# SomeUserName1/UNet-bSSFP

Measured on AMD Instinct MI355X. Metric: train-step volumes/sec (128^3 bSSFP->6ch DTI), higher is better.
Workload: dtype bf16; 1 GPU; gan_step: full GAN training step (G fwd x2, G bwd, D fwd x3, D bwd x3, 2x AdamW); volume=1x24x128^3 -> 6ch per GPU, global_batch=1, perceptual_term=absent (needs remote weights), parallelism=dp1, input_feed=one batch resident in HBM

## Files before the change

### include/mi355_unet.h

```cpp
#ifndef MI355_UNET_H
#define MI355_UNET_H

#include <stddef.h>
#include <stdint.h>

#ifdef __cplusplus
extern "C" {
#endif

#define MI355_DT_F32 0
#define MI355_DT_BF16 1
#define MI355_DT_F64 2
#define MI355_DT_FP8 3

#define MI355_OK 0
#define MI355_ERR_ARG (-1)
#define MI355_ERR_UNSUPPORTED (-2)
#define MI355_ERR_HIP (-3)

int mi355_version(void);
const char* mi355_last_error(void);

int mi355_pack_ncdhw(const float* src, void* dst, int32_t n, int32_t c, int64_t v,
                     int32_t ld, int32_t coff, int32_t zero_to, int32_t dtype, void* stream);
int mi355_unpack_ncdhw(const void* src, float* dst, int32_t n, int32_t c, int64_t v,
                       int32_t ld, int32_t coff, int32_t dtype, void* stream);
int mi355_pack_ncdhw_s2d(const float* src, void* dst, int32_t n, int32_t c, int32_t d, int32_t h, int32_t w,
                         int32_t cblk, int32_t ld, int32_t coff, int32_t zero_to, int32_t dtype, void* stream);
int mi355_pack2_ncdhw(const float* src0, int32_t c0, const float* src1, int32_t c1, void* dst, int32_t n, int64_t v,
                      int32_t ld, int32_t coff, int32_t zero_to, int32_t dtype, void* stream);
int mi355_pack2_ncdhw_s2d(const float* src0, int32_t c0, const float* src1, int32_t c1, void* dst, int32_t n, int32_t d,
                          int32_t h, int32_t w, int32_t cblk, int32_t ld, int32_t coff, int32_t zero_to, int32_t dtype,
                          void* stream);
int mi355_unpack_ncdhw_s2d(const void* src, float* dst, int32_t n, int32_t c, int32_t d, int32_t h, int32_t w,
                           int32_t cblk, int32_t ld, int32_t coff, int32_t dtype, void* stream);

typedef struct mi355_wpack_desc {
  const float* src;
  void* dst;
  int32_t cout, cin;
  int32_t coutp, cinp;
  int32_t ks;
  int64_t s_co, s_ci;
  int64_t s_k[3];
  int32_t tbase[3], tstep[3];
  int32_t dtype;
  int32_t s2d_mode, s2d_cp;
  const float* q_amax;
} mi355_wpack_desc;
int mi355_weight_pack(const mi355_wpack_desc* d, void* stream);
int mi355_weight_pack_multi(const mi355_wpack_desc* descs, int32_t n, void* stream);

typedef struct mi355_conv_desc {
  const void* x0; int32_t c0; int32_t ld0;
  const void* x1; int32_t c1; int32_t ld1;
  int32_t n, di, hi, wi;
  int32_t do_, ho, wo;
  int32_t ks, stride;
  int32_t pad[3];
  const void* wp;
  int32_t coutp;
  const float* bias;
  void* y; int32_t ldy; int32_t cstore;
  int32_t dy, hy, wy;
  int32_t os; int32_t ooff[3];
  float* stats_part;
  int32_t dtype;
  void* workspace; int64_t workspace_bytes;
  int32_t cls_cout;
  int32_t nbias;
  const float* q_amax_x; const float* q_amax_w;
  const float* addend; int32_t ld_add; int32_t y_f32;
  int32_t add_n;
  int32_t d2s; const float* delta; int32_t add_bf16;
} mi355_conv_desc;
int mi355_conv_fwd(const mi355_conv_desc* d, void* stream);
int64_t mi355_conv_workspace_bytes(const mi355_conv_desc* d);
int mi355_conv_plan_id(const mi355_conv_desc* d);
int mi355_conv_num_tiles(const mi355_conv_desc* d, int32_t* tiles, int32_t* tiles_per_sample);

int mi355_upcat_compose(const float* wd, const float* wc, const float* bd, const float* bc, int32_t cl, int32_t cu, int32_t ce,
                        int32_t co, float* k4, void* wp_d2s, float* biasp, float* delta, void* stream);
int mi355_upcat_chain(const float* dk4, const float* wd, const float* wc, const float* bd, const float* esum, int32_t cl, int32_t cu,
                      int32_t ce, int32_t co, float* dwd, float* dwc, float* dbd, int32_t accumulate, void* stream);
int64_t mi355_border_sums_workspace(int32_t n, int32_t d, int32_t c);
int mi355_border_sums(const void* g, int32_t ld, int32_t n, int32_t d, int32_t h, int32_t w, int32_t c, int32_t dtype, float* workspace,
                      float* e, void* stream);
int mi355_s2d_repack(const void* src, int32_t ld_src, void* dst, int32_t ld_dst, int32_t n, int32_t d, int32_t h, int32_t w,
                     int32_t c, int32_t dtype, void* stream);
int mi355_seam_grad(const float* g_ncdhw, const void* g_s2d, int32_t ld_s, int32_t cblk, void* dz, int32_t ld_dz, int32_t cpad,
                    int32_t n, int32_t c, int32_t d, int32_t h, int32_t w, int32_t dtype, void* stream);

typedef struct mi355_wgrad_desc {
  const void* x0; int32_t c0; int32_t ld0;
  const void* x1; int32_t c1; int32_t ld1;
  int32_t n, di, hi, wi;
  const void* g; int32_t cg; int32_t ldg;
  int32_t do_, ho, wo;
  int32_t gd, gh, gw;
  int32_t gs; int32_t goff[3];
  int32_t ks, stride;
  int32_t pad[3];
  float* workspace; int64_t workspace_bytes;
  float* dw; int32_t cout, cin;
  int64_t s_co, s_ci; int64_t s_k[3];
  int32_t tbase[3], tstep[3];
  int32_t accumulate;
  int32_t dtype;
  int32_t s2d_cp;
  int32_t g_cls_cout;
  int32_t xn;
} mi355_wgrad_desc;
int64_t mi355_conv_wgrad_workspace(const mi355_wgrad_desc* d);
int mi355_conv_wgrad(const mi355_wgrad_desc* d, void* stream);
int mi355_conv_wgrad_plan_kind(const mi355_wgrad_desc* d);
typedef struct mi355_wreduce_job { int64_t opaque[20]; } mi355_wreduce_job;
int mi355_conv_wgrad_partial(const mi355_wgrad_desc* d, mi355_wreduce_job* job, void* stream);
int mi355_wgrad_reduce_multi(const mi355_wreduce_job* jobs, int32_t n, void* stream);

int mi355_channel_stats(const void* x, int32_t ld, int32_t c, int64_t rows_per_group, int32_t groups,
                        float* part, int32_t blocks_per_group, int32_t dtype, void* stream);
int32_t mi355_channel_stats_blocks(int64_t rows_per_group);

int mi355_norm_finalize(const float* part, int32_t parts_per_group, int32_t groups, int32_t c,
                        int64_t count_per_group, const float* shift, int32_t n_real, float eps,
                        float* mean, float* rstd,
                        float* running_mean, float* running_var, float momentum, int64_t* batches_tracked, void* stream);

typedef struct mi355_normact_desc {
  const void* z; int32_t ldz;
  void* a; int32_t lda;
  int32_t c; int64_t rows_per_group; int32_t groups;
  const float* mean; const float* rstd;
  const float* gamma; const float* beta;
  float slope;
  float drop_p; uint64_t seed;
  int32_t dtype;
  const void* da; int32_t ldda;
  void* dz; int32_t lddz;
  float* part;
  int32_t blocks_per_group;
  const float* sums;
  int32_t batch_stats;
  int32_t s2d_a, s2d_da;
  int32_t sd, sh, sw;
  const uint64_t* seed_ptr;
  int32_t n_affine;
  void* q8; int32_t ld8; const float* q_use; float* q_next;
  const void* gz; int32_t ldgz; const float* gw; int32_t gw_ld; int32_t gk;
  void* fy; int32_t ldfy; int32_t fcp; const float* fbias; int32_t skip_a;
  const void* pool_idx; const void* pool_dy; int32_t ldpdy;
  void* pool_y; int32_t ldpy; uint8_t* pool_widx;
} mi355_normact_desc;
int mi355_normact_fwd(const mi355_normact_desc* d, void* stream);
int mi355_normact_bwd_reduce(const mi355_normact_desc* d, void* stream);
int mi355_normact_bwd_finalize(const float* part, int32_t blocks_per_group, int32_t groups, int32_t c,
                               float* sums, float* dgamma, float* dbeta, void* stream);
int mi355_normact_bwd_finalize_into(const float* part, int32_t blocks_per_group, int32_t groups, int32_t c,
                                    float* sums, float* dgamma, float* dbeta, int32_t n_affine, int32_t accumulate,
                                    void* stream);
int mi355_normact_bwd_apply(const mi355_normact_desc* d, void* stream);

typedef struct mi355_normact_small_desc {
  mi355_normact_desc base;
  float eps, momentum;
  float* mean_out; float* rstd_out;
  float* running_mean; float* running_var; int64_t* batches_tracked; int32_t n_real;
  float* dgamma; float* dbeta; int32_t accumulate;
} mi355_normact_small_desc;
int mi355_normact_small_fwd(const mi355_normact_small_desc* d, void* stream);
int mi355_normact_small_bwd(const mi355_normact_small_desc* d, void* stream);

int mi355_colsum_finalize(const float* part, int32_t parts, int32_t c, float* out, void* stream);
int mi355_colsum_finalize_into(const float* part, int32_t parts, int32_t c, float* out, int32_t n_out, int32_t accumulate,
                               void* stream);
int mi355_colsum_finalize_from(const float* part, int32_t parts, int32_t c, int32_t offset, float* out, int32_t n_out,
                               int32_t accumulate, void* stream);

int mi355_maxpool2_fwd(const void* x, int32_t ldx, void* y, int32_t ldy, int32_t n, int32_t c,
                       int32_t d, int32_t h, int32_t w, int32_t dtype, void* stream);
int mi355_maxpool2_fwd_idx(const void* x, int32_t ldx, void* y, int32_t ldy, uint8_t* idx, int32_t n, int32_t c,
                           int32_t d, int32_t h, int32_t w, int32_t dtype, void* stream);
int mi355_maxpool2_bwd(const void* x, int32_t ldx, const void* y, int32_t ldy,
                       const void* dy, int32_t lddy, void* dx, int32_t lddx,
                       int32_t n, int32_t c, int32_t d, int32_t h, int32_t w,
                       int32_t dtype, void* stream);
int mi355_maxpool2_bwd_add(const void* x, int32_t ldx, const void* y, int32_t ldy, const void* dy, int32_t lddy,
                           void* dx, int32_t lddx, const void* add, int32_t ldadd,
                           int32_t n, int32_t c, int32_t d, int32_t h, int32_t w,
                           int32_t dtype, void* stream);

int32_t mi355_l1_blocks(int64_t count);
int mi355_l1_fwd(const float* a, const float* b, int64_t count, float* partials, float* out, void* stream);
int mi355_l1_bwd(const float* a, const float* b, int64_t count, const float* gscale, float* da, void* stream);
int mi355_l1_partials(const float* a, const float* b, int64_t count, float* partials, void* stream);

int mi355_gan_gen_loss_fwd(const float* logits, int32_t n, const float* l1_partials, int32_t n_partials, int64_t count,
                           float recon_divisor, float recon_factor, float* out4, void* stream);
int mi355_gan_gen_loss_bwd(const float* logits, int32_t n, const float* upstream, float recon_divisor, float recon_factor,
                           float* dlogits, float* l1_gscale, void* stream);
int mi355_gan_discr_loss_fwd(const float* logits_fake, int32_t n_fake, const float* logits_real, int32_t n_real, float* out1,
                             void* stream);
int mi355_gan_discr_loss_bwd(const float* logits_fake, int32_t n_fake, const float* logits_real, int32_t n_real,
                             const float* upstream, float* dfake, float* dreal, void* stream);

int mi355_adamw_multi(const void* const* ptrs, const int64_t* sizes, int32_t ntensors,
                      float lr, float beta1, float beta2, float eps, float weight_decay,
                      const int64_t* step_dev, int64_t step, void* stream);

int mi355_dti_scalar_maps(const void* tensor, int32_t dtype, int64_t nvox, int64_t comp_stride,
                          int64_t vox_stride, double scale, double offset, void* fa, void* md, void* ad,
                          void* rd, void* azimuth, void* inclination, void* rgb, void* stream);

int64_t mi355_dti_errors_workspace_bytes(int64_t nvox, int32_t nroi);
int mi355_dti_errors(const void* pred, const void* target, int32_t dtype, int64_t comp_stride, int64_t vox_stride,
                     const uint8_t* mask, const void* probseg, int32_t probseg_dtype, int64_t roi_stride,
                     int64_t probseg_vox_stride, int64_t nvox, int32_t nroi, double scale, double offset,
                     void* workspace, int64_t workspace_bytes, double* table_out, void* const* maps, void* stream);

#define MI355_MAX_PATCHES 48
#define MI355_AGG_CROP 0
#define MI355_AGG_AVERAGE 1
int mi355_patch_gather(const float* vol, int32_t c, int32_t d, int32_t h, int32_t w, const int32_t* origins,
                       int32_t npatches, int32_t pd, int32_t ph, int32_t pw, float* out, void* stream);
int mi355_patch_aggregate(const float* patches, const int32_t* locs9, int32_t npatches, int32_t pd, int32_t ph,
                          int32_t pw, int32_t mode, float* vol, float* count, int32_t c, int32_t d, int32_t h,
                          int32_t w, void* stream);
int mi355_patch_average_finalize(float* vol, const float* count, int32_t c, int64_t voxels, void* stream);

int32_t mi355_err_blocks(int64_t per_item);
int mi355_err_sums(const float* a, const float* b, int64_t per_item, int32_t items, double* partials,
                   double* out, void* stream);
int64_t mi355_ssim3d_workspace_bytes(int32_t items, int32_t c, int32_t d, int32_t h, int32_t w, int32_t win);
int mi355_ssim3d(const float* x, const float* y, int32_t items, int32_t c, int32_t d, int32_t h, int32_t w,
                 int32_t win, const float* window, float c1, float c2, void* workspace,
                 int64_t workspace_bytes, double* out, void* stream);

int mi355_aug_bias_field(const float* x, float* out, int32_t c, int32_t d, int32_t h, int32_t w,
                         const float* coefficients, int32_t order, void* stream);
int mi355_aug_gamma(const float* x, float* out, int64_t count, float gamma, void* stream);
int mi355_aug_noise(const float* x, float* out, int64_t count, float mean, float std, uint64_t seed, void* stream);

#define MI355_QUEUE_MAX_LOADS 4
#define MI355_QUEUE_MAX_IMAGES 4
#define MI355_QUEUE_MAX_STAGES 3
#define MI355_STAGE_BIAS_FIELD 1
#define MI355_STAGE_NOISE 2
#define MI355_STAGE_GAMMA 3

typedef struct mi355_queue_load {
  int32_t nstages;
  int32_t stage[MI355_QUEUE_MAX_STAGES];
  int32_t bias_order;
  float bias_coef[35];
  float noise_mean, noise_std;
  uint64_t noise_seed;
  float gamma;
} mi355_queue_load;

typedef struct mi355_queue_source {
  const float* src;
  int32_t d, h, w;
} mi355_queue_source;

int mi355_patch_queue_gather(const mi355_queue_load* loads, int32_t nloads, const mi355_queue_source* sources,
                             const int32_t* channels, const int32_t* augmented, float* const* outs, int32_t nimages,
                             const int32_t* patches, int32_t npatches, int32_t td, int32_t th, int32_t tw,
                             int32_t pd, int32_t ph, int32_t pw, float padding_value, void* stream);

#define MI355_AXIS_MAX_N 128
#define MI355_KSPACE_SUM_BLOCKS 128
int mi355_axis_apply(const float* x, const float* m, float* out, int32_t c, int32_t d, int32_t h, int32_t w,
                     int32_t axis, void* stream);
int mi355_axis_apply_complex(const float* xr, const float* xi, const float* mr, const float* mi, float* outr, float* outi,
                             int32_t c, int32_t d, int32_t h, int32_t w, int32_t axis, void* stream);
int64_t mi355_kspace_workspace_bytes(int32_t c, int32_t d, int32_t h, int32_t w);
int mi355_axis_apply_complex_max(const float* xr, const float* xi, const float* mr, const float* mi, int32_t c, int32_t d,
                                 int32_t h, int32_t w, void* workspace, int64_t workspace_bytes, double* out, void* stream);
int mi355_channel_sum_min(const float* x, int32_t c, int64_t vol, void* workspace, int64_t workspace_bytes, double* out,
                          void* stream);
int mi355_aug_spike_add(const float* x, float* out, int32_t c, int32_t d, int32_t h, int32_t w, int32_t f0, int32_t f1,
                        int32_t f2, const double* m, int32_t dc, float intensity, void* stream);

int mi355_mfma_selftest(float* out_f32_1024, float* out_bf16_1024, void* stream);

int mi355_amax_f32(const float* x, int64_t n, float* amax, void* stream);
int mi355_amax_act(const void* x, int32_t ld, int32_t c, int64_t rows, int32_t dtype, float* amax, void* stream);
int mi355_cast_fp8(const void* src, int32_t ld_src, int32_t c, int64_t rows, int32_t src_dtype, const float* amax,
                   void* dst, int32_t ld_dst, void* stream);
int mi355_cast_fp8_delayed(const void* src, int32_t ld_src, int32_t c, int64_t rows, int32_t src_dtype, const float* amax,
                           float* amax_next, void* dst, int32_t ld_dst, void* stream);
int mi355_fp8_scale_roll(float* table, int32_t n, int32_t* sat, void* stream);
int mi355_fp8_selftest(float* out_1024, void* stream);

#ifdef __cplusplus
}
#endif
#endif
```

### unet_bssfp_amd/_lib.py

```python
from __future__ import annotations

import ctypes as C
import os
import threading

_HERE = os.path.dirname(os.path.abspath(__file__))
LIB_PATH = os.path.join(_HERE, "libmi355_unet.so")

DT_F32 = 0
DT_BF16 = 1
DT_FP8 = 3

_i32, _i64, _f32, _u64, _vp = C.c_int32, C.c_int64, C.c_float, C.c_uint64, C.c_void_p


class WpackDesc(C.Structure):
    _fields_ = [("src", _vp), ("dst", _vp), ("cout", _i32), ("cin", _i32), ("coutp", _i32), ("cinp", _i32),
                ("ks", _i32), ("s_co", _i64), ("s_ci", _i64), ("s_k", _i64 * 3),
                ("tbase", _i32 * 3), ("tstep", _i32 * 3), ("dtype", _i32), ("s2d_mode", _i32), ("s2d_cp", _i32),
                ("q_amax", _vp)]


class ConvDesc(C.Structure):
    _fields_ = [("x0", _vp), ("c0", _i32), ("ld0", _i32), ("x1", _vp), ("c1", _i32), ("ld1", _i32),
                ("n", _i32), ("di", _i32), ("hi", _i32), ("wi", _i32),
                ("do_", _i32), ("ho", _i32), ("wo", _i32), ("ks", _i32), ("stride", _i32),
                ("pad", _i32 * 3), ("wp", _vp), ("coutp", _i32), ("bias", _vp),
                ("y", _vp), ("ldy", _i32), ("cstore", _i32), ("dy", _i32), ("hy", _i32), ("wy", _i32),
                ("os", _i32), ("ooff", _i32 * 3), ("stats_part", _vp), ("dtype", _i32),
                ("workspace", _vp), ("workspace_bytes", _i64), ("cls_cout", _i32), ("nbias", _i32),
                ("q_amax_x", _vp), ("q_amax_w", _vp), ("addend", _vp), ("ld_add", _i32), ("y_f32", _i32), ("add_n", _i32),
                ("d2s", _i32), ("delta", _vp), ("add_bf16", _i32)]


class WgradDesc(C.Structure):
    _fields_ = [("x0", _vp), ("c0", _i32), ("ld0", _i32), ("x1", _vp), ("c1", _i32), ("ld1", _i32),
                ("n", _i32), ("di", _i32), ("hi", _i32), ("wi", _i32),
                ("g", _vp), ("cg", _i32), ("ldg", _i32),
                ("do_", _i32), ("ho", _i32), ("wo", _i32), ("gd", _i32), ("gh", _i32), ("gw", _i32),
                ("gs", _i32), ("goff", _i32 * 3), ("ks", _i32), ("stride", _i32), ("pad", _i32 * 3),
                ("workspace", _vp), ("workspace_bytes", _i64),
                ("dw", _vp), ("cout", _i32), ("cin", _i32), ("s_co", _i64), ("s_ci", _i64), ("s_k", _i64 * 3),
                ("tbase", _i32 * 3), ("tstep", _i32 * 3), ("accumulate", _i32), ("dtype", _i32), ("s2d_cp", _i32),
                ("g_cls_cout", _i32), ("xn", _i32)]


class WreduceJob(C.Structure):
    _fields_ = [("opaque", _i64 * 20)]


class NormActDesc(C.Structure):
    _fields_ = [("z", _vp), ("ldz", _i32), ("a", _vp), ("lda", _i32), ("c", _i32),
                ("rows_per_group", _i64), ("groups", _i32),
                ("mean", _vp), ("rstd", _vp), ("gamma", _vp), ("beta", _vp),
                ("slope", _f32), ("drop_p", _f32), ("seed", _u64), ("dtype", _i32),
                ("da", _vp), ("ldda", _i32), ("dz", _vp), ("lddz", _i32),
                ("part", _vp), ("blocks_per_group", _i32), ("sums", _vp), ("batch_stats", _i32),
                ("s2d_a", _i32), ("s2d_da", _i32), ("sd", _i32), ("sh", _i32), ("sw", _i32), ("seed_ptr", _vp),
                ("n_affine", _i32), ("q8", _vp), ("ld8", _i32), ("q_use", _vp), ("q_next", _vp),
                ("gz", _vp), ("ldgz", _i32), ("gw", _vp), ("gw_ld", _i32), ("gk", _i32),
                ("fy", _vp), ("ldfy", _i32), ("fcp", _i32), ("fbias", _vp), ("skip_a", _i32),
                ("pool_idx", _vp), ("pool_dy", _vp), ("ldpdy", _i32),
                ("pool_y", _vp), ("ldpy", _i32), ("pool_widx", _vp)]


class QueueLoad(C.Structure):
    _fields_ = [("nstages", _i32), ("stage", _i32 * 3), ("bias_order", _i32), ("bias_coef", _f32 * 35),
                ("noise_mean", _f32), ("noise_std", _f32), ("noise_seed", _u64), ("gamma", _f32)]


class QueueSource(C.Structure):
    _fields_ = [("src", _vp), ("d", _i32), ("h", _i32), ("w", _i32)]


class NormSmallDesc(C.Structure):
    _fields_ = [("base", NormActDesc), ("eps", _f32), ("momentum", _f32), ("mean_out", _vp), ("rstd_out", _vp),
                ("running_mean", _vp), ("running_var", _vp), ("batches_tracked", _vp), ("n_real", _i32),
                ("dgamma", _vp), ("dbeta", _vp), ("accumulate", _i32)]


_SIGNATURES = {
    "mi355_version": (C.c_int, []),
    "mi355_last_error": (C.c_char_p, []),
    "mi355_pack_ncdhw": (C.c_int, [_vp, _vp, _i32, _i32, _i64, _i32, _i32, _i32, _i32, _vp]),
    "mi355_unpack_ncdhw": (C.c_int, [_vp, _vp, _i32, _i32, _i64, _i32, _i32, _i32, _vp]),
    "mi355_pack_ncdhw_s2d": (C.c_int, [_vp, _vp, _i32, _i32, _i32, _i32, _i32, _i32, _i32, _i32, _i32, _i32, _vp]),
    "mi355_unpack_ncdhw_s2d": (C.c_int, [_vp, _vp, _i32, _i32, _i32, _i32, _i32, _i32, _i32, _i32, _i32, _vp]),
    "mi355_pack2_ncdhw": (C.c_int, [_vp, _i32, _vp, _i32, _vp, _i32, _i64, _i32, _i32, _i32, _i32, _vp]),
    "mi355_pack2_ncdhw_s2d": (C.c_int, [_vp, _i32, _vp, _i32, _vp, _i32, _i32, _i32, _i32, _i32, _i32, _i32, _i32, _i32, _vp]),
    "mi355_upcat_compose": (C.c_int, [_vp, _vp, _vp, _vp, _i32, _i32, _i32, _i32, _vp, _vp, _vp, _vp, _vp]),
    "mi355_upcat_chain": (C.c_int, [_vp, _vp, _vp, _vp, _vp, _i32, _i32, _i32, _i32, _vp, _vp, _vp, _i32, _vp]),
    "mi355_border_sums_workspace": (_i64, [_i32, _i32, _i32]),
    "mi355_border_sums": (C.c_int, [_vp, _i32, _i32, _i32, _i32, _i32, _i32, _i32, _vp, _vp, _vp]),
    "mi355_s2d_repack": (C.c_int, [_vp, _i32, _vp, _i32, _i32, _i32, _i32, _i32, _i32, _i32, _vp]),
    "mi355_seam_grad": (C.c_int, [_vp, _vp, _i32, _i32, _vp, _i32, _i32, _i32, _i32, _i32, _i32, _i32, _i32, _vp]),
    "mi355_weight_pack": (C.c_int, [C.POINTER(WpackDesc), _vp]),
    "mi355_weight_pack_multi": (C.c_int, [C.POINTER(WpackDesc), _i32, _vp]),
    "mi355_conv_fwd": (C.c_int, [C.POINTER(ConvDesc), _vp]),
    "mi355_conv_workspace_bytes": (_i64, [C.POINTER(ConvDesc)]),
    "mi355_conv_plan_id": (C.c_int, [C.POINTER(ConvDesc)]),
    "mi355_conv_num_tiles": (C.c_int, [C.POINTER(ConvDesc), C.POINTER(_i32), C.POINTER(_i32)]),
    "mi355_conv_wgrad_workspace": (_i64, [C.POINTER(WgradDesc)]),
    "mi355_conv_wgrad_plan_kind": (C.c_int, [C.POINTER(WgradDesc)]),
    "mi355_conv_wgrad": (C.c_int, [C.POINTER(WgradDesc), _vp]),
    "mi355_conv_wgrad_partial": (C.c_int, [C.POINTER(WgradDesc), C.POINTER(WreduceJob), _vp]),
    "mi355_wgrad_reduce_multi": (C.c_int, [C.POINTER(WreduceJob), _i32, _vp]),
    "mi355_channel_stats": (C.c_int, [_vp, _i32, _i32, _i64, _i32, _vp, _i32, _i32, _vp]),
    "mi355_channel_stats_blocks": (_i32, [_i64]),
    "mi355_norm_finalize": (C.c_int, [_vp, _i32, _i32, _i32, _i64, _vp, _i32, _f32, _vp, _vp, _vp, _vp, _f32, _vp, _vp]),
    "mi355_normact_fwd": (C.c_int, [C.POINTER(NormActDesc), _vp]),
    "mi355_normact_bwd_reduce": (C.c_int, [C.POINTER(NormActDesc), _vp]),
    "mi355_normact_bwd_finalize": (C.c_int, [_vp, _i32, _i32, _i32, _vp, _vp, _vp, _vp]),
    "mi355_normact_bwd_finalize_into": (C.c_int, [_vp, _i32, _i32, _i32, _vp, _vp, _vp, _i32, _i32, _vp]),
    "mi355_normact_bwd_apply": (C.c_int, [C.POINTER(NormActDesc), _vp]),
    "mi355_normact_small_fwd": (C.c_int, [C.POINTER(NormSmallDesc), _vp]),
    "mi355_normact_small_bwd": (C.c_int, [C.POINTER(NormSmallDesc), _vp]),
    "mi355_colsum_finalize": (C.c_int, [_vp, _i32, _i32, _vp, _vp]),
    "mi355_colsum_finalize_into": (C.c_int, [_vp, _i32, _i32, _vp, _i32, _i32, _vp]),
    "mi355_colsum_finalize_from": (C.c_int, [_vp, _i32, _i32, _i32, _vp, _i32, _i32, _vp]),
    "mi355_maxpool2_fwd": (C.c_int, [_vp, _i32, _vp, _i32, _i32, _i32, _i32, _i32, _i32, _i32, _vp]),
    "mi355_maxpool2_fwd_idx": (C.c_int, [_vp, _i32, _vp, _i32, _vp, _i32, _i32, _i32, _i32, _i32, _i32, _vp]),
    "mi355_maxpool2_bwd": (C.c_int, [_vp, _i32, _vp, _i32, _vp, _i32, _vp, _i32, _i32, _i32, _i32, _i32, _i32, _i32, _vp]),
    "mi355_maxpool2_bwd_add": (C.c_int, [_vp, _i32, _vp, _i32, _vp, _i32, _vp, _i32, _vp, _i32, _i32, _i32, _i32, _i32, _i32, _i32, _vp]),
    "mi355_l1_blocks": (_i32, [_i64]),
    "mi355_l1_fwd": (C.c_int, [_vp, _vp, _i64, _vp, _vp, _vp]),
    "mi355_l1_bwd": (C.c_int, [_vp, _vp, _i64, _vp, _vp, _vp]),
    "mi355_l1_partials": (C.c_int, [_vp, _vp, _i64, _vp, _vp]),
    "mi355_gan_gen_loss_fwd": (C.c_int, [_vp, _i32, _vp, _i32, _i64, _f32, _f32, _vp, _vp]),
    "mi355_gan_gen_loss_bwd": (C.c_int, [_vp, _i32, _vp, _f32, _f32, _vp, _vp, _vp]),
    "mi355_gan_discr_loss_fwd": (C.c_int, [_vp, _i32, _vp, _i32, _vp, _vp]),
    "mi355_gan_discr_loss_bwd": (C.c_int, [_vp, _i32, _vp, _i32, _vp, _vp, _vp, _vp]),
    "mi355_adamw_multi": (C.c_int, [_vp, _vp, _i32, _f32, _f32, _f32, _f32, _f32, _vp, _i64, _vp]),
    "mi355_dti_scalar_maps": (C.c_int, [_vp, _i32, _i64, _i64, _i64, C.c_double, C.c_double,
                                        _vp, _vp, _vp, _vp, _vp, _vp, _vp, _vp]),
    "mi355_dti_errors_workspace_bytes": (_i64, [_i64, _i32]),
    "mi355_dti_errors": (C.c_int, [_vp, _vp, _i32, _i64, _i64, _vp, _vp, _i32, _i64, _i64, _i64, _i32,
                                   C.c_double, C.c_double, _vp, _i64, _vp, _vp, _vp]),
    "mi355_patch_gather": (C.c_int, [_vp, _i32, _i32, _i32, _i32, _vp, _i32, _i32, _i32, _i32, _vp, _vp]),
    "mi355_patch_aggregate": (C.c_int, [_vp, _vp, _i32, _i32, _i32, _i32, _i32, _vp, _vp, _i32, _i32, _i32, _i32, _vp]),
    "mi355_patch_average_finalize": (C.c_int, [_vp, _vp, _i32, _i64, _vp]),
    "mi355_err_blocks": (_i32, [_i64]),
    "mi355_err_sums": (C.c_int, [_vp, _vp, _i64, _i32, _vp, _vp, _vp]),
    "mi355_ssim3d_workspace_bytes": (_i64, [_i32, _i32, _i32, _i32, _i32, _i32]),
    "mi355_ssim3d": (C.c_int, [_vp, _vp, _i32, _i32, _i32, _i32, _i32, _i32, _vp, _f32, _f32, _vp, _i64, _vp, _vp]),
    "mi355_aug_bias_field": (C.c_int, [_vp, _vp, _i32, _i32, _i32, _i32, _vp, _i32, _vp]),
    "mi355_aug_gamma": (C.c_int, [_vp, _vp, _i64, _f32, _vp]),
    "mi355_aug_noise": (C.c_int, [_vp, _vp, _i64, _f32, _f32, C.c_uint64, _vp]),
    "mi355_patch_queue_gather": (C.c_int, [C.POINTER(QueueLoad), _i32, C.POINTER(QueueSource), _vp, _vp, _vp, _i32,
                                           _vp, _i32, _i32, _i32, _i32, _i32, _i32, _i32, _f32, _vp]),
    "mi355_axis_apply": (C.c_int, [_vp, _vp, _vp, _i32, _i32, _i32, _i32, _i32, _vp]),
    "mi355_axis_apply_complex": (C.c_int, [_vp, _vp, _vp, _vp, _vp, _vp, _i32, _i32, _i32, _i32, _i32, _vp]),
    "mi355_kspace_workspace_bytes": (_i64, [_i32, _i32, _i32, _i32]),
    "mi355_axis_apply_complex_max": (C.c_int, [_vp, _vp, _vp, _vp, _i32, _i32, _i32, _i32, _vp, _i64, _vp, _vp]),
    "mi355_channel_sum_min": (C.c_int, [_vp, _i32, _i64, _vp, _i64, _vp, _vp]),
    "mi355_aug_spike_add": (C.c_int, [_vp, _vp, _i32, _i32, _i32, _i32, _i32, _i32, _i32, _vp, _i32, _f32, _vp]),
    "mi355_mfma_selftest": (C.c_int, [_vp, _vp, _vp]),
    "mi355_amax_f32": (C.c_int, [_vp, _i64, _vp, _vp]),
    "mi355_amax_act": (C.c_int, [_vp, _i32, _i32, _i64, _i32, _vp, _vp]),
    "mi355_cast_fp8": (C.c_int, [_vp, _i32, _i32, _i64, _i32, _vp, _vp, _i32, _vp]),
    "mi355_cast_fp8_delayed": (C.c_int, [_vp, _i32, _i32, _i64, _i32, _vp, _vp, _vp, _i32, _vp]),
    "mi355_fp8_scale_roll": (C.c_int, [_vp, _i32, _vp, _vp]),
    "mi355_fp8_selftest": (C.c_int, [_vp, _vp]),
}

EXPORTED_SYMBOLS = tuple(_SIGNATURES)

_lock = threading.Lock()
_lib = None


class Mi355Error(RuntimeError):
    pass


def load():
    global _lib
    if _lib is not None:
        return _lib
    with _lock:
        if _lib is None:
            if not os.path.exists(LIB_PATH):
                raise Mi355Error(
                    f"{LIB_PATH} not found: build it with `python -c 'import __graft_entry__ as g; g.build()'` "
                    "(hipcc --offload-arch=gfx950).  There is no CPU fallback.")
            lib = C.CDLL(LIB_PATH)
            for name, (res, args) in _SIGNATURES.items():
                fn = getattr(lib, name)
                fn.restype = res
                fn.argtypes = args
            _lib = lib
    return _lib


def check(rc: int, what: str = ""):
    if rc != 0:
        msg = load().mi355_last_error().decode("utf-8", "replace")
        raise Mi355Error(f"{what or 'mi355 call'} failed ({rc}): {msg}")
```

### unet_bssfp_amd/csrc/elementwise.hip

```cpp
#include <stdlib.h>
#include "common.h"

namespace {

constexpr int kRowsPerStatBlock = 2048;

struct S2D { int d, h, w, cblk; };
__device__ __forceinline__ void s2d_cell(const S2D& q, long long row , long long& srow, int& blk, int& border) {
  const int w = (int)(row % q.w); long long t = row / q.w;
  const int h = (int)(t % q.h); t /= q.h;
  const int d = (int)(t % q.d); const long long n = t / q.d;
  srow = ((n * (q.d / 2 + 1) + ((d + 1) >> 1)) * (q.h / 2 + 1) + ((h + 1) >> 1)) * (q.w / 2 + 1) + ((w + 1) >> 1);
  blk = ((d + 1) & 1) * 4 + ((h + 1) & 1) * 2 + ((w + 1) & 1);
  border = ((d == 0 || d == q.d - 1) ? 4 : 0) | ((h == 0 || h == q.h - 1) ? 2 : 0) | ((w == 0 || w == q.w - 1) ? 1 : 0);
}
__device__ __forceinline__ long long s2d_offset(const S2D& q, long long row, int ld) {
  long long srow; int blk, border;
  s2d_cell(q, row, srow, blk, border);
  return srow * ld + (long long)blk * q.cblk;
}
template <typename T>
__device__ __forceinline__ void s2d_zero_siblings(T* base, const S2D& q, long long srow, int blk, int border, int ld, int e0) {
  if (!border) return;
  Vec16<T> z;
// ... 222 lines not shown
                                                             long long rows_per_group, float* __restrict__ part,
                                                             int blocks_per_group) {
  const int g = blockIdx.y, b = blockIdx.x;
  const long long rb = (rows_per_group + blocks_per_group - 1) / blocks_per_group;
  const long long r0 = (long long)b * rb;
  long long r1 = r0 + rb;
  if (r1 > rows_per_group) r1 = rows_per_group;
  const T* base = x + (long long)g * rows_per_group * ld;
  float* out = part + ((long long)g * blocks_per_group + b) * 2 * c;
  block_channel_sums<T>(c, r0, r1,
      [&](long long row, int ch0, float* s0, float* s1) {
        Vec16<T> v;
        v.load(base + row * ld + ch0);
#pragma unroll
        for (int j = 0; j < Vec16<T>::N; ++j) { s0[j] += v.f[j]; s1[j] += v.f[j] * v.f[j]; }
      },
      out, out + c);
}

__device__ __forceinline__ void block_sum_parts(const float* __restrict__ part, int nparts, int c, int ch0,
                                                double& t0, double& t1) {
  __shared__ double red[16][8][2];
  const int cl = threadIdx.x & 7, pl = threadIdx.x >> 3;
  const int ch = ch0 + cl;
  double s0 = 0.0, s1 = 0.0;
  if (ch < c) {
    int k = pl;
    for (; k + 384 < nparts; k += 512) {
      const float a0 = part[(long long)k * 2 * c + ch], b0 = part[(long long)k * 2 * c + c + ch];
      const float a1 = part[(long long)(k + 128) * 2 * c + ch], b1 = part[(long long)(k + 128) * 2 * c + c + ch];
      const float a2 = part[(long long)(k + 256) * 2 * c + ch], b2 = part[(long long)(k + 256) * 2 * c + c + ch];
      const float a3 = part[(long long)(k + 384) * 2 * c + ch], b3 = part[(long long)(k + 384) * 2 * c + c + ch];
      s0 += ((double)a0 + (double)a1) + ((double)a2 + (double)a3);
      s1 += ((double)b0 + (double)b1) + ((double)b2 + (double)b3);
    }
    for (; k < nparts; k += 128) {
      s0 += (double)part[(long long)k * 2 * c + ch];
      s1 += (double)part[(long long)k * 2 * c + c + ch];
    }
  }
#pragma unroll
  for (int o = 8; o < 64; o <<= 1) {
    s0 += __shfl_xor(s0, o, 64);
    s1 += __shfl_xor(s1, o, 64);
  }
  const int wave = threadIdx.x >> 6;
  if ((threadIdx.x & 63) < 8) { red[wave][cl][0] = s0; red[wave][cl][1] = s1; }
  __syncthreads();
  double a0 = 0.0, a1 = 0.0;
#pragma unroll
  for (int w = 0; w < 16; ++w) { a0 += red[w][cl][0]; a1 += red[w][cl][1]; }
  t0 = a0;
  t1 = a1;
  __syncthreads();
}

__global__ __launch_bounds__(1024) void norm_finalize_kernel(const float* __restrict__ part, int ppg, int c,
                                                             long long count, const float* __restrict__ shift,
                                                             int n_real, float eps, float* __restrict__ mean,
                                                             float* __restrict__ rstd, float* running_mean,
                                                             float* running_var, float momentum,
                                                             long long* batches_tracked, int groups_here) {
  const int ch0 = blockIdx.x * 8;
  if (batches_tracked && blockIdx.x == 0 && blockIdx.y == 0 && threadIdx.x == 0) batches_tracked[0] += groups_here;
  for (int gi = 0; gi < groups_here; ++gi) {
    const int g = groups_here > 1 ? gi : blockIdx.y;
    double s1, s2;
    block_sum_parts(part + (long long)g * ppg * 2 * c, ppg, c, ch0, s1, s2);
    const int ch = ch0 + (int)threadIdx.x;
    if (threadIdx.x >= 8 || ch >= c) continue;
    const double m = s1 / (double)count;
    double var = s2 / (double)count - m * m;
    if (var < 0.0) var = 0.0;
    const double mu = m + ((shift && ch < n_real) ? (double)shift[ch] : 0.0);
    mean[(long long)g * c + ch] = (float)mu;
    rstd[(long long)g * c + ch] = (float)(1.0 / sqrt(var + (double)eps));
    if (running_mean && ch < n_real) {
      const double unb = count > 1 ? var * (double)count / (double)(count - 1) : var;
      running_mean[ch] = (float)((1.0 - momentum) * running_mean[ch] + momentum * mu);
      running_var[ch] = (float)((1.0 - momentum) * running_var[ch] + momentum * unb);
    }
  }
}

__global__ __launch_bounds__(1024) void colsum_finalize_kernel(const float* __restrict__ part, int parts, int c, int offset,
                                                               float* __restrict__ out, int n_out, int accumulate) {
  const int ch0 = offset + blockIdx.x * 8;
  double s0, s1;
  block_sum_parts(part, parts, c, ch0, s0, s1);
  const int j = blockIdx.x * 8 + (int)threadIdx.x;
  if (threadIdx.x < 8 && j < n_out) out[j] = accumulate ? out[j] + (float)s0 : (float)s0;
}

__device__ __forceinline__ unsigned long long eff_seed(unsigned long long salt, const unsigned long long* p) {
  return p ? p[0] * 0x9E3779B97F4A7C15ull + salt * 0xD1B54A32D192ED03ull + 1ull : salt;
}
__device__ __forceinline__ unsigned long long drop_group_bits(unsigned long long seed, unsigned long long group) {
  unsigned long long x = group * 0x9E3779B97F4A7C15ull + seed;
  x ^= x >> 32; x *= 0xD6E8FEB86659FD93ull; x ^= x >> 32;
  return x;
}
template <int EPV>
__device__ __forceinline__ unsigned drop_keep_mask(unsigned long long seed, unsigned long long e0, unsigned thr16) {
  unsigned m = 0;
#pragma unroll
  for (int g4 = 0; g4 < EPV / 4; ++g4) {
    const unsigned long long x = drop_group_bits(seed, (e0 >> 2) + g4);
#pragma unroll
    for (int k = 0; k < 4; ++k) m |= ((((unsigned)(x >> (16 * k))) & 0xffffu) >= thr16 ? 1u : 0u) << (4 * g4 + k);
  }
  return m;
}

__device__ __forceinline__ void amax_commit(float m, float* out) {
  __shared__ float red[4];
#pragma unroll
  for (int o = 32; o > 0; o >>= 1) m = fmaxf(m, __shfl_xor(m, o, 64));
  if ((threadIdx.x & 63) == 0) red[threadIdx.x >> 6] = m;
  __syncthreads();
  if (threadIdx.x == 0) {
    m = fmaxf(fmaxf(red[0], red[1]), fmaxf(red[2], red[3]));
    const unsigned cur = __hip_atomic_load(reinterpret_cast<unsigned int*>(out), __ATOMIC_RELAXED, __HIP_MEMORY_SCOPE_AGENT);
    if (__float_as_uint(m) > cur) atomicMax(reinterpret_cast<unsigned int*>(out), __float_as_uint(m));
  }
}
__device__ __forceinline__ float e4m3_piece(const float (&f)[8], float sc, uint8_t* dst) {
  float m = 0.f, r[8];
#pragma unroll
  for (int j = 0; j < 8; ++j) {
    const float b = __uint_as_float((uint32_t)f32_to_bf16_bits(f[j]) << 16);
    m = fmaxf(m, fabsf(b));
    r[j] = b * sc;
  }
  uint32_t w0 = cvt_pk_fp8(r[0], r[1], 0u, false), w1 = cvt_pk_fp8(r[4], r[5], 0u, false);
  w0 = cvt_pk_fp8(r[2], r[3], w0, true);
  w1 = cvt_pk_fp8(r[6], r[7], w1, true);
  *reinterpret_cast<uint2*>(dst) = make_uint2(w0, w1);
  return m;
}

struct NormActArgs {
  const char* z; int ldz; char* a; int lda;
  int c; long long rows_per_group; int groups;
  const float* mean; const float* rstd; const float* gamma; const float* beta;
  float slope; float drop_scale; unsigned thr16; unsigned long long seed; const unsigned long long* seed_ptr;
  const char* da; int ldda; char* dz; int lddz;
  float* part; int blocks_per_group; const float* sums; int batch_stats;
  int n_affine;
  S2D s2d_a;
  S2D s2d_da;
  uint8_t* q8; int ld8; const float* q_use; float* q_next;
  const char* gz; int ldgz; const float* gw; int gw_ld; int gk;
  char* fy; int ldfy; int fcp; const float* fbias; int skip_a;
  const uint8_t* pool_idx; const char* pool_dy; int ldpdy; int pd, ph, pw;
  char* pool_y; int ldpy; uint8_t* pool_widx;
};

#ifndef MI355_DIAG_NO_NT
#define FP8_NT_A 1
#endif
__device__ __forceinline__ void st_nt_b128(void* p, const uint4 v) {
  typedef unsigned u4 __attribute__((ext_vector_type(4)));
  const u4 x = {v.x, v.y, v.z, v.w};
  __builtin_nontemporal_store(x, reinterpret_cast<u4*>(p));
}
__device__ __forceinline__ void store16_nt(const Vec16<float>& v, void* p) {
  st_nt_b128(p, make_uint4(__float_as_uint(v.f[0]), __float_as_uint(v.f[1]), __float_as_uint(v.f[2]), __float_as_uint(v.f[3])));
}
__device__ __forceinline__ void store16_nt(const Vec16<bf16_t>& v, void* p) {
  uint32_t w[4];
#pragma unroll
  for (int i = 0; i < 4; ++i) w[i] = (uint32_t)f32_to_bf16_bits(v.f[2 * i]) | ((uint32_t)f32_to_bf16_bits(v.f[2 * i + 1]) << 16);
  st_nt_b128(p, make_uint4(w[0], w[1], w[2], w[3]));
}

template <typename T, bool DROP>
__global__ __launch_bounds__(256) void normact_fwd_kernel(const NormActArgs q) {
  constexpr int EPV = Elem<T>::kPer16B;
  const int g = blockIdx.y;
  const int lpr = q.c / EPV, rpp = 256 / lpr;
  const int piece = threadIdx.x % lpr, rsub = threadIdx.x / lpr;
  if (rsub >= rpp) return;
  const int ch0 = piece * EPV;
  const unsigned long long seed = DROP ? eff_seed(q.seed, q.seed_ptr) : 0ull;
  float sc[EPV], sh[EPV];
#pragma unroll
  for (int j = 0; j < EPV; ++j) {
    const int ch = ch0 + j;
    const float ga = q.gamma ? (ch < q.n_affine ? q.gamma[ch] : 0.f) : 1.f, be = (q.beta && ch < q.n_affine) ? q.beta[ch] : 0.f;
    if (q.mean) {
      const float rs = q.rstd[(long long)g * q.c + ch], mu = q.mean[(long long)g * q.c + ch];
      sc[j] = ga * rs;
      sh[j] = be - mu * ga * rs;
    } else { sc[j] = ga; sh[j] = be; }
  }
  const T* zb = reinterpret_cast<const T*>(q.z) + (long long)g * q.rows_per_group * q.ldz;
  T* ab = reinterpret_cast<T*>(q.a) + (long long)g * q.rows_per_group * q.lda;
  const long long stride = (long long)gridDim.x * rpp;
  const float sc8 = q.q8 ? fp8_scale_of(q.q_use) : 1.f;
  float m8 = 0.f;
  for (long long row = (long long)blockIdx.x * rpp + rsub; row < q.rows_per_group; row += stride) {
    Vec16<T> v;
#ifdef NORM_NT_FWD
    v.load_nt(zb + row * q.ldz + ch0);
#else
    v.load(zb + row * q.ldz + ch0);
#endif
    const unsigned long long e0 = ((unsigned long long)g * q.rows_per_group + row) * q.c + ch0;
    unsigned keep = 0;
    if constexpr (DROP) keep = drop_keep_mask<EPV>(seed, e0, q.thr16);
#pragma unroll
    for (int j = 0; j < EPV; ++j) {
      float t = v.f[j] * sc[j] + sh[j];
      if constexpr (DROP) t = (keep >> j) & 1u ? t * q.drop_scale : 0.f;
      v.f[j] = t > 0.f ? t : t * q.slope;
    }
    if (q.s2d_a.d) {
      long long srow; int blk, border;
      s2d_cell(q.s2d_a, (long long)g * q.rows_per_group + row, srow, blk, border);
      v.store(reinterpret_cast<T*>(q.a) + srow * q.lda + (long long)blk * q.s2d_a.cblk + ch0);
      s2d_zero_siblings<T>(reinterpret_cast<T*>(q.a), q.s2d_a, srow, blk, border, q.lda, ch0);
    }
#ifdef FP8_NT_A
    else if (q.q8) store16_nt(v, ab + row * q.lda + ch0);
#endif
    else v.store(ab + row * q.lda + ch0);
    if constexpr (sizeof(T) == 2) {
      if (q.q8) m8 = fmaxf(m8, e4m3_piece(v.f, sc8, q.q8 + ((long long)g * q.rows_per_group + row) * q.ld8 + ch0));
    }
  }
  if constexpr (sizeof(T) == 2) {
    if (q.q8) amax_commit(m8, q.q_next);
  }
}

template <typename T, bool DROP>
__global__ __launch_bounds__(256) void normact_pool_fwd_kernel(const NormActArgs q) {
  constexpr int EPV = Elem<T>::kPer16B;
  const int lpr = q.c / EPV, vpp = 256 / lpr;
  const int piece = threadIdx.x % lpr, vsub = threadIdx.x / lpr;
  if (vsub >= vpp) return;
  const int ch0 = piece * EPV;
  const int n_ = blockIdx.y;
  const long long dhw = (long long)q.pd * q.ph * q.pw;
  const int g = (int)(((long long)n_ * dhw) / q.rows_per_group);
  const unsigned long long seed = DROP ? eff_seed(q.seed, q.seed_ptr) : 0ull;
  float sc[EPV], sh[EPV];
#pragma unroll
  for (int j = 0; j < EPV; ++j) {
    const int ch = ch0 + j;
    const float ga = q.gamma ? (ch < q.n_affine ? q.gamma[ch] : 0.f) : 1.f, be = (q.beta && ch < q.n_affine) ? q.beta[ch] : 0.f;
    if (q.mean) {
      const float rs = q.rstd[(long long)g * q.c + ch], mu = q.mean[(long long)g * q.c + ch];
      sc[j] = ga * rs;
      sh[j] = be - mu * ga * rs;
    } else { sc[j] = ga; sh[j] = be; }
  }
  const int od_ = q.pd / 2, oh_ = q.ph / 2, ow_ = q.pw / 2;
  const int pooled = od_ * oh_ * ow_;
  const T* zb = reinterpret_cast<const T*>(q.z);
  T* ab = reinterpret_cast<T*>(q.a);
  for (int o = blockIdx.x * vpp + vsub; o < pooled; o += gridDim.x * vpp) {
    const int ow = o % ow_, t = o / ow_, oh = t % oh_, od = t / oh_;
    Vec16<T> m;
    unsigned long long where = 0;
    unsigned nan_seen = 0;
#pragma unroll
    for (int kd = 0; kd < 2; ++kd)
#pragma unroll
      for (int kh = 0; kh < 2; ++kh)
#pragma unroll
        for (int kw = 0; kw < 2; ++kw) {
          const long long vox = (((long long)n_ * q.pd + 2 * od + kd) * q.ph + 2 * oh + kh) * q.pw + 2 * ow + kw;
          const unsigned long long kk = (unsigned long long)(kd * 4 + kh * 2 + kw);
          Vec16<T> v;
#ifdef NORM_NT_FWD
          v.load_nt(zb + vox * q.ldz + ch0);
#else
          v.load(zb + vox * q.ldz + ch0);
#endif
          unsigned keep = 0;
          if constexpr (DROP) keep = drop_keep_mask<EPV>(seed, (unsigned long long)vox * q.c + ch0, q.thr16);
#pragma unroll
          for (int j = 0; j < EPV; ++j) {
            float t2 = v.f[j] * sc[j] + sh[j];
            if constexpr (DROP) t2 = (keep >> j) & 1u ? t2 * q.drop_scale : 0.f;
            t2 = t2 > 0.f ? t2 : t2 * q.slope;
            if constexpr (sizeof(T) == 2) t2 = bf16_bits_to_f32(f32_to_bf16_bits(t2));
            v.f[j] = t2;
          }
          v.store(ab + vox * q.lda + ch0);
          if (kk == 0) {
            m = v;
#pragma unroll
            for (int j = 0; j < EPV; ++j) nan_seen |= (v.f[j] != v.f[j] ? 1u : 0u) << j;
          } else {
#pragma unroll
            for (int j = 0; j < EPV; ++j) {
              const bool isnan_ = v.f[j] != v.f[j];
              const bool take = v.f[j] > m.f[j] || isnan_;
              m.f[j] = take ? v.f[j] : m.f[j];
              const bool mark = ((nan_seen >> j) & 1u) ? false : take;
              where = mark ? ((where & ~(0xffull << (8 * j))) | (kk << (8 * j))) : where;
              nan_seen |= (isnan_ ? 1u : 0u) << j;
            }
          }
        }
    const long long orow = (long long)n_ * pooled + o;
    m.store(reinterpret_cast<T*>(q.pool_y) + orow * q.ldpy + ch0);
    if constexpr (EPV == 8) *reinterpret_cast<unsigned long long*>(q.pool_widx + orow * q.c + ch0) = where;
    else *reinterpret_cast<unsigned*>(q.pool_widx + orow * q.c + ch0) = (unsigned)where;
  }
}

typedef float f32x4v __attribute__((ext_vector_type(4)));
template <bool DROP>
__global__ __launch_bounds__(256) void normact_fwd_final32_kernel(const NormActArgs q) {
  const int lane = threadIdx.x & 63, wave = threadIdx.x >> 6, n = lane & 15, p = lane >> 4;
  const int g = blockIdx.y, ch0 = 8 * p;
  const unsigned long long seed = DROP ? eff_seed(q.seed, q.seed_ptr) : 0ull;
  float sc[8], sh[8];
#pragma unroll
  for (int j = 0; j < 8; ++j) {
    const int ch = ch0 + j;
    const float ga = q.gamma ? (ch < q.n_affine ? q.gamma[ch] : 0.f) : 1.f, be = (q.beta && ch < q.n_affine) ? q.beta[ch] : 0.f;
    if (q.mean) {
      const float rs = q.rstd[(long long)g * 32 + ch], mu = q.mean[(long long)g * 32 + ch];
      sc[j] = ga * rs;
      sh[j] = be - mu * ga * rs;
    } else { sc[j] = ga; sh[j] = be; }
  }
  uint4 wf;
  {
    unsigned w[4];
#pragma unroll
    for (int i = 0; i < 4; ++i) {
      const int ch = ch0 + 2 * i;
      const float lo = (n < q.gk && ch < q.gw_ld) ? q.gw[(long long)n * q.gw_ld + ch] : 0.f;
      const float hi = (n < q.gk && ch + 1 < q.gw_ld) ? q.gw[(long long)n * q.gw_ld + ch + 1] : 0.f;
      w[i] = (unsigned)f32_to_bf16_bits(lo) | ((unsigned)f32_to_bf16_bits(hi) << 16);
    }
    wf = make_uint4(w[0], w[1], w[2], w[3]);
  }
  float fb[4];
#pragma unroll
  for (int j = 0; j < 4; ++j) fb[j] = (q.fbias && 4 * p + j < q.gk) ? q.fbias[4 * p + j] : 0.f;
  const bf16_t* zb = reinterpret_cast<const bf16_t*>(q.z) + (long long)g * q.rows_per_group * q.ldz;
  bf16_t* ab = reinterpret_cast<bf16_t*>(q.a) + (long long)g * q.rows_per_group * q.lda;
  bf16_t* yb = reinterpret_cast<bf16_t*>(q.fy) + (long long)g * q.rows_per_group * q.ldfy;
  const long long stride = (long long)gridDim.x * 64;
  const long long first = (long long)blockIdx.x * 64 + wave * 16;
  uint4 zn = make_uint4(0u, 0u, 0u, 0u);
  if (first < q.rows_per_group) {
    const long long rc = first + n < q.rows_per_group ? first + n : q.rows_per_group - 1;
    zn = *reinterpret_cast<const uint4*>(zb + rc * q.ldz + ch0);
  }
  for (long long row0 = first; row0 < q.rows_per_group; row0 += stride) {
    const long long row = row0 + n;
    const bool ok = row < q.rows_per_group;
    const long long rowc = ok ? row : q.rows_per_group - 1;
    const uint4 zc = zn;
    if (row0 + stride < q.rows_per_group) {
      const long long rc = row + stride < q.rows_per_group ? row + stride : q.rows_per_group - 1;
      zn = *reinterpret_cast<const uint4*>(zb + rc * q.ldz + ch0);
    }
    Vec16<bf16_t> v;
    v.from_bits(zc);
    unsigned keep = 0;
    if constexpr (DROP) keep = drop_keep_mask<8>(seed, ((unsigned long long)g * q.rows_per_group + rowc) * 32 + ch0, q.thr16);
#pragma unroll
    for (int j = 0; j < 8; ++j) {
      float x = v.f[j] * sc[j] + sh[j];
      if constexpr (DROP) x = (keep >> j) & 1u ? x * q.drop_scale : 0.f;
      v.f[j] = x > 0.f ? x : x * q.slope;
    }
    unsigned w[4];
#pragma unroll
    for (int i = 0; i < 4; ++i) w[i] = (unsigned)f32_to_bf16_bits(v.f[2 * i]) | ((unsigned)f32_to_bf16_bits(v.f[2 * i + 1]) << 16);
    const uint4 aw = make_uint4(w[0], w[1], w[2], w[3]);
    if (ok && !q.skip_a) *reinterpret_cast<uint4*>(ab + row * q.lda + ch0) = aw;
    f32x4v acc = {0.f, 0.f, 0.f, 0.f};
    acc = __builtin_amdgcn_mfma_f32_16x16x32_bf16(__builtin_bit_cast(bf16x8, wf), __builtin_bit_cast(bf16x8, aw), acc, 0, 0, 0);
    if (ok && 4 * p < q.fcp) {
      const uint2 yv = make_uint2((uint32_t)f32_to_bf16_bits(acc[0] + fb[0]) | ((uint32_t)f32_to_bf16_bits(acc[1] + fb[1]) << 16),
                                  (uint32_t)f32_to_bf16_bits(acc[2] + fb[2]) | ((uint32_t)f32_to_bf16_bits(acc[3] + fb[3]) << 16));
      *reinterpret_cast<uint2*>(yb + row * q.ldfy + 4 * p) = yv;
    }
  }
}

template <int EPV> struct BwdConst { float mu[EPV], rs[EPV], ga[EPV], be[EPV]; };
template <int EPV>
__device__ __forceinline__ void load_bwd_const(const NormActArgs& q, int g, int ch0, BwdConst<EPV>& k) {
#pragma unroll
  for (int j = 0; j < EPV; ++j) {
    const int ch = ch0 + j;
    k.mu[j] = q.mean ? q.mean[(long long)g * q.c + ch] : 0.f;
    k.rs[j] = q.mean ? q.rstd[(long long)g * q.c + ch] : 1.f;
    k.ga[j] = q.gamma ? (ch < q.n_affine ? q.gamma[ch] : 0.f) : 1.f;
    k.be[j] = (q.beta && ch < q.n_affine) ? q.beta[ch] : 0.f;
  }
}
constexpr int kImplicitMaxC = 64;
__device__ __forceinline__ void fill_implicit_w(const NormActArgs& q, uint4* wtab) {
  const int ch = threadIdx.x;
  if (ch < q.c && ch < kImplicitMaxC) {
    unsigned w[4];
#pragma unroll
    for (int i = 0; i < 4; ++i) {
      const bool okc = ch < q.gw_ld;
      const float lo = (okc && 2 * i < q.gk) ? q.gw[(long long)(2 * i) * q.gw_ld + ch] : 0.f;
      const float hi = (okc && 2 * i + 1 < q.gk) ? q.gw[(long long)(2 * i + 1) * q.gw_ld + ch] : 0.f;
      w[i] = (unsigned)f32_to_bf16_bits(lo) | ((unsigned)f32_to_bf16_bits(hi) << 16);
    }
    wtab[ch] = make_uint4(w[0], w[1], w[2], w[3]);
  }
  __syncthreads();
}
template <typename T, int EPV>
__device__ __forceinline__ void implicit_da(const NormActArgs& q, long long grow, const uint4* wtab, int ch0, Vec16<T>& dv) {
  if constexpr (sizeof(T) == 2) {
    typedef __bf16 bf16x2 __attribute__((ext_vector_type(2)));
    const uint4 gv = *reinterpret_cast<const uint4*>(reinterpret_cast<const T*>(q.gz) + grow * q.ldgz);
    asm volatile("" : "+v"(ch0));
#pragma unroll
    for (int j = 0; j < EPV; ++j) {
      const uint4 wv = wtab[ch0 + j];
      float t = __builtin_amdgcn_fdot2_f32_bf16(__builtin_bit_cast(bf16x2, gv.x), __builtin_bit_cast(bf16x2, wv.x), 0.f, false);
      t = __builtin_amdgcn_fdot2_f32_bf16(__builtin_bit_cast(bf16x2, gv.y), __builtin_bit_cast(bf16x2, wv.y), t, false);
      t = __builtin_amdgcn_fdot2_f32_bf16(__builtin_bit_cast(bf16x2, gv.z), __builtin_bit_cast(bf16x2, wv.z), t, false);
      t = __builtin_amdgcn_fdot2_f32_bf16(__builtin_bit_cast(bf16x2, gv.w), __builtin_bit_cast(bf16x2, wv.w), t, false);
      dv.f[j] = bf16_bits_to_f32(f32_to_bf16_bits(t));
    }
  }
}
template <typename T, int EPV>
__device__ __forceinline__ void pooled_da(const NormActArgs& q, long long grow, int ch0, Vec16<T>& dv) {
  const unsigned v = (unsigned)grow, W = (unsigned)q.pw, H = (unsigned)q.ph, D = (unsigned)q.pd;
  const unsigned w_ = v % W, t1 = v / W, h_ = t1 % H, t2 = t1 / H, d_ = t2 % D, n_ = t2 / D;
  const long long o = (((long long)n_ * (D >> 1) + (d_ >> 1)) * (H >> 1) + (h_ >> 1)) * (W >> 1) + (w_ >> 1);
  const unsigned k = ((d_ & 1u) << 2) | ((h_ & 1u) << 1) | (w_ & 1u);
  Vec16<T> gy;
  gy.load(reinterpret_cast<const T*>(q.pool_dy) + o * q.ldpdy + ch0);
  unsigned long long ib;
  if constexpr (EPV == 8) ib = *reinterpret_cast<const unsigned long long*>(q.pool_idx + o * q.c + ch0);
  else ib = *reinterpret_cast<const unsigned*>(q.pool_idx + o * q.c + ch0);
  if (q.da) dv.load(reinterpret_cast<const T*>(q.da) + grow * q.ldda + ch0);
#pragma unroll
  for (int j = 0; j < EPV; ++j) {
    float t = ((unsigned)(ib >> (8 * j)) & 0xffu) == k ? gy.f[j] : 0.f;
    if (q.da) t += dv.f[j];
    if constexpr (sizeof(T) == 2) t = bf16_bits_to_f32(f32_to_bf16_bits(t));
    dv.f[j] = t;
  }
}
template <bool DROP>
__device__ __forceinline__ void bwd_elem(const NormActArgs& q, bool keep, float mu, float rs, float ga,
                                         float be, float zv, float dav, float& gout, float& xhat) {
  xhat = (zv - mu) * rs;
  float pre = xhat * ga + be;
  float gv = dav;
  if constexpr (DROP) {
    pre = keep ? pre : 0.f;
    gv = keep ? gv * q.drop_scale : 0.f;
  }
  gout = pre > 0.f ? gv : gv * q.slope;
}

template <typename T, bool DROP, int IMPL = 0>
__global__ __launch_bounds__(256) void normact_bwd_reduce_kernel(const NormActArgs q) {
  constexpr int EPV = Elem<T>::kPer16B;
  const int g = blockIdx.y, b = blockIdx.x;
  const long long rb = (q.rows_per_group + q.blocks_per_group - 1) / q.blocks_per_group;
  const long long r0 = (long long)b * rb;
  long long r1 = r0 + rb;
  if (r1 > q.rows_per_group) r1 = q.rows_per_group;
  const T* zb = reinterpret_cast<const T*>(q.z) + (long long)g * q.rows_per_group * q.ldz;
  const T* db = reinterpret_cast<const T*>(q.da) + (long long)g * q.rows_per_group * q.ldda;
  float* out = q.part + ((long long)g * q.blocks_per_group + b) * 2 * q.c;
  BwdConst<EPV> k;
  load_bwd_const<EPV>(q, g, (int)(threadIdx.x % (q.c / EPV)) * EPV, k);
  const unsigned long long seed = DROP ? eff_seed(q.seed, q.seed_ptr) : 0ull;
  __shared__ uint4 wtab[IMPL == 1 ? kImplicitMaxC : 1];
  if constexpr (IMPL == 1) fill_implicit_w(q, wtab);
  block_channel_sums<T>(q.c, r0, r1,
      [&](long long row, int ch0, float* s0, float* s1) {
        Vec16<T> zv, dv;
        zv.load(zb + row * q.ldz + ch0);
        if constexpr (IMPL == 1) implicit_da<T, EPV>(q, (long long)g * q.rows_per_group + row, wtab, ch0, dv);
        else if constexpr (IMPL == 2) pooled_da<T, EPV>(q, (long long)g * q.rows_per_group + row, ch0, dv);
        else if (q.s2d_da.d) dv.load(reinterpret_cast<const T*>(q.da) + s2d_offset(q.s2d_da, (long long)g * q.rows_per_group + row, q.ldda) + ch0);
        else dv.load(db + row * q.ldda + ch0);
        unsigned keep = 0;
        if constexpr (DROP) keep = drop_keep_mask<EPV>(seed, ((unsigned long long)g * q.rows_per_group + row) * q.c + ch0, q.thr16);
#pragma unroll
        for (int j = 0; j < EPV; ++j) {
          float gv, xh;
          bwd_elem<DROP>(q, (keep >> j) & 1u, k.mu[j], k.rs[j], k.ga[j], k.be[j], zv.f[j], dv.f[j], gv, xh);
          s0[j] += gv;
          s1[j] += gv * xh;
        }
      },
      out, out + q.c);
}

__global__ __launch_bounds__(1024) void normact_bwd_finalize_kernel(const float* __restrict__ part, int bpg,
                                                                    int groups, int c, float* __restrict__ sums,
                                                                    float* dgamma, float* dbeta, int n_affine, int accumulate) {
  const int ch0 = blockIdx.x * 8;
  const int ch = ch0 + (int)threadIdx.x;
  const bool owner = threadIdx.x < 8 && ch < c;
  double tg = 0.0, tb = 0.0;
  for (int g = 0; g < groups; ++g) {
    double s0, s1;
    block_sum_parts(part + (long long)g * bpg * 2 * c, bpg, c, ch0, s0, s1);
    if (owner) {
      sums[((long long)g * 2 + 0) * c + ch] = (float)s0;
      sums[((long long)g * 2 + 1) * c + ch] = (float)s1;
      tb += s0;
      tg += s1;
    }
  }
  if (owner && ch < n_affine) {
    if (dgamma) dgamma[ch] = accumulate ? dgamma[ch] + (float)tg : (float)tg;
    if (dbeta) dbeta[ch] = accumulate ? dbeta[ch] + (float)tb : (float)tb;
  }
}

template <typename T, bool DROP, int IMPL = 0>
__global__ __launch_bounds__(256, IMPL == 1 ? 5 : 1) void normact_bwd_apply_kernel(const NormActArgs q) {
  constexpr int EPV = Elem<T>::kPer16B;
  __shared__ uint4 wtab[IMPL == 1 ? kImplicitMaxC : 1];
  if constexpr (IMPL == 1) fill_implicit_w(q, wtab);
  const int g = blockIdx.y;
  const int lpr = q.c / EPV, rpp = 256 / lpr;
  const int piece = threadIdx.x % lpr, rsub = threadIdx.x / lpr;
  if (rsub >= rpp) return;
  const int ch0 = piece * EPV;
  const float inv = 1.f / (float)q.rows_per_group;
// ... 1070 lines not shown
                "weight_pack: bad extents");
  MI355_REQUIRE(d->s2d_mode >= 0 && d->s2d_mode <= 2 && (d->s2d_mode == 0 || (d->s2d_cp > 0 && d->s2d_cp % 8 == 0)),
                "weight_pack: bad space-to-depth mode");
  a->src = d->src; a->dst = d->dst; a->cout = d->cout; a->cin = d->cin; a->coutp = d->coutp; a->cinp = d->cinp; a->ks = d->ks;
  a->s_co = d->s_co; a->s_ci = d->s_ci; a->s_k0 = d->s_k[0]; a->s_k1 = d->s_k[1]; a->s_k2 = d->s_k[2];
  a->tb0 = d->tbase[0]; a->tb1 = d->tbase[1]; a->tb2 = d->tbase[2];
  a->ts0 = d->tstep[0]; a->ts1 = d->tstep[1]; a->ts2 = d->tstep[2];
  a->s2d_mode = d->s2d_mode; a->s2d_cp = d->s2d_cp;
  a->q_amax = d->q_amax;
  return MI355_OK;
}

int mi355_weight_pack_multi(const mi355_wpack_desc* descs, int32_t n, void* stream) {
  MI355_REQUIRE(descs && n > 0, "weight_pack_multi: bad argument");
  const int dtype = descs[0].dtype;
  MI355_REQUIRE(dtype == MI355_DT_F32 || dtype == MI355_DT_BF16 || dtype == MI355_DT_FP8, "weight_pack_multi: bad dtype");
  for (int pass = 0; pass < 3; ++pass) {
    const bool want_dense = pass == 0, want_s2d = pass == 1;
    int i0 = 0;
    while (i0 < n) {
      WpackMulti m;
      int cnt = 0;
      long long mx = 0, patches = 0;
      const mi355_wpack_desc* firstd = nullptr;
      for (; i0 < n && cnt < kWpackChunk; ++i0) {
        const mi355_wpack_desc* d = &descs[i0];
        MI355_REQUIRE(d->dtype == dtype, "weight_pack_multi: mixed dtypes");
        const int klass = wpack_is_dense3(d) ? 0 : (wpack_is_s2d_dense(d) ? 1 : 2);
        if (klass != pass) continue;
        int rc = fill_wpack(d, &m.a[cnt]);
        if (rc) return rc;
        if (!firstd) firstd = d;
        const long long total = (long long)d->cinp * d->ks * d->ks * d->ks * d->coutp;
        const long long np = want_s2d ? (d->s2d_mode == 1 ? (long long)(d->coutp / 8) * (d->s2d_cp / 16) : (long long)(d->cinp / 16) * (d->s2d_cp / 8))
                                      : (long long)(d->cinp / 16) * (d->coutp / 16);
        if (total > mx) mx = total;
        if (np > patches) patches = np;
        ++cnt;
      }
      if (cnt == 0) break;
      for (int i = cnt; i < kWpackChunk; ++i) m.a[i] = m.a[0];
      if (want_dense) {
        MI355_REQUIRE(patches < (1ll << 31), "weight_pack_multi: too many patches");
        dim3 grid((unsigned)patches, cnt);
        if (dtype == MI355_DT_F32) wpack_dense3_multi_kernel<float><<<grid, dim3(256), 0, (hipStream_t)stream>>>(m);
        else if (dtype == MI355_DT_FP8) wpack_dense3_multi_kernel<fp8_t><<<grid, dim3(256), 0, (hipStream_t)stream>>>(m);
        else wpack_dense3_multi_kernel<bf16_t><<<grid, dim3(256), 0, (hipStream_t)stream>>>(m);
      } else if (want_s2d) {
        MI355_REQUIRE(patches < (1ll << 31), "weight_pack_multi: too many patches");
        dim3 grid((unsigned)patches, cnt);
        MI355_REQUIRE(dtype != MI355_DT_FP8, "weight_pack_multi: no fp8 space-to-depth packing");
        if (dtype == MI355_DT_F32) wpack_s2d_multi_kernel<float><<<grid, dim3(256), 0, (hipStream_t)stream>>>(m);
        else wpack_s2d_multi_kernel<bf16_t><<<grid, dim3(256), 0, (hipStream_t)stream>>>(m);
      } else {
        long long nb = (mx + 256 * 8 - 1) / (256 * 8);
        if (nb > 512) nb = 512;
        dim3 grid((unsigned)nb, cnt);
        if (dtype == MI355_DT_F32) hipLaunchKernelGGL(wpack_multi_kernel<float>, grid, dim3(256), 0, (hipStream_t)stream, m);
        else if (dtype == MI355_DT_FP8) hipLaunchKernelGGL(wpack_multi_kernel<fp8_t>, grid, dim3(256), 0, (hipStream_t)stream, m);
        else hipLaunchKernelGGL(wpack_multi_kernel<bf16_t>, grid, dim3(256), 0, (hipStream_t)stream, m);
      }
    }
  }
  return mi355_check_launch("weight_pack_multi");
}

int32_t mi355_channel_stats_blocks(int64_t rows_per_group) {
  long long b = rows_per_group / 128;
  if (b > 1024) b = (rows_per_group + kRowsPerStatBlock - 1) / kRowsPerStatBlock;
  if (b < 1024 && rows_per_group / 128 > 1024) b = 1024;
  const long long fine = rows_per_group / 16 < 256 ? rows_per_group / 16 : 256;
  if (b < fine) b = fine;
  if (b < 1) b = 1;
  if (b > 2048) b = 2048;
  return (int32_t)b;
}

int mi355_channel_stats(const void* x, int32_t ld, int32_t c, int64_t rows_per_group, int32_t groups, float* part,
                        int32_t blocks_per_group, int32_t dtype, void* stream) {
  MI355_REQUIRE(x && part && rows_per_group > 0 && groups > 0 && blocks_per_group > 0, "channel_stats: bad argument");
  int rc = check_rows(c, ld, dtype, "channel_stats");
  if (rc) return rc;
  dim3 grid(blocks_per_group, groups);
  if (dtype == MI355_DT_F32)
    hipLaunchKernelGGL(channel_stats_kernel<float>, grid, dim3(256), 0, (hipStream_t)stream, (const float*)x, ld, c, (long long)rows_per_group, part, blocks_per_group);
  else
    hipLaunchKernelGGL(channel_stats_kernel<bf16_t>, grid, dim3(256), 0, (hipStream_t)stream, (const bf16_t*)x, ld, c, (long long)rows_per_group, part, blocks_per_group);
  return mi355_check_launch("channel_stats");
}

int mi355_norm_finalize(const float* part, int32_t parts_per_group, int32_t groups, int32_t c, int64_t count_per_group,
                        const float* shift, int32_t n_real, float eps, float* mean, float* rstd, float* running_mean,
                        float* running_var, float momentum, int64_t* batches_tracked, void* stream) {
  MI355_REQUIRE(part && mean && rstd && parts_per_group > 0 && groups > 0 && c > 0 && count_per_group > 0, "norm_finalize: bad argument");
  MI355_REQUIRE(!running_mean || running_var, "norm_finalize: running_mean without running_var");
  const bool serial = running_mean && groups > 1;
  hipLaunchKernelGGL(norm_finalize_kernel, dim3((c + 7) / 8, serial ? 1 : groups), dim3(1024), 0, (hipStream_t)stream, part,
                     parts_per_group, c, (long long)count_per_group, shift, n_real > 0 ? n_real : c, eps, mean, rstd, running_mean, running_var, momentum,
                     (long long*)batches_tracked, serial ? groups : 1);
  return mi355_check_launch("norm_finalize");
}

int mi355_colsum_finalize(const float* part, int32_t parts, int32_t c, float* out, void* stream) {
  return mi355_colsum_finalize_into(part, parts, c, out, c, 0, stream);
}

int mi355_colsum_finalize_into(const float* part, int32_t parts, int32_t c, float* out, int32_t n_out, int32_t accumulate,
                               void* stream) {
  return mi355_colsum_finalize_from(part, parts, c, 0, out, n_out, accumulate, stream);
}

int mi355_colsum_finalize_from(const float* part, int32_t parts, int32_t c, int32_t offset, float* out, int32_t n_out,
                               int32_t accumulate, void* stream) {
  MI355_REQUIRE(part && out && parts > 0 && c > 0 && n_out > 0 && offset >= 0 && offset + n_out <= c, "colsum_finalize: bad argument");
  hipLaunchKernelGGL(colsum_finalize_kernel, dim3((n_out + 7) / 8), dim3(1024), 0, (hipStream_t)stream, part, parts, c, offset, out, n_out,
                     accumulate);
  return mi355_check_launch("colsum_finalize");
}

static int fill_normact(const mi355_normact_desc* d, NormActArgs* q, const char* who) {
  MI355_REQUIRE(d && d->z, "%s: null pointer", who);
  int rc = check_rows(d->c, d->ldz, d->dtype, who);
  if (rc) return rc;
  MI355_REQUIRE(d->rows_per_group > 0 && d->groups > 0, "%s: empty", who);
  MI355_REQUIRE(!d->mean || d->rstd, "%s: mean without rstd", who);
  MI355_REQUIRE(d->drop_p >= 0.f && d->drop_p < 1.f, "%s: dropout p out of range", who);
  q->z = (const char*)d->z; q->ldz = d->ldz; q->a = (char*)d->a; q->lda = d->lda;
  q->c = d->c; q->rows_per_group = d->rows_per_group; q->groups = d->groups;
  q->mean = d->mean; q->rstd = d->rstd; q->gamma = d->gamma; q->beta = d->beta;
  q->slope = d->slope;
  q->thr16 = d->drop_p > 0.f ? (unsigned)(d->drop_p * 65536.f + 0.5f) : 0u;
  q->drop_scale = d->drop_p > 0.f ? 1.f / (1.f - d->drop_p) : 1.f;
  q->seed = d->seed;
  q->seed_ptr = (const unsigned long long*)d->seed_ptr;
  q->n_affine = d->n_affine > 0 ? d->n_affine : d->c;
  q->da = (const char*)d->da; q->ldda = d->ldda; q->dz = (char*)d->dz; q->lddz = d->lddz;
  q->part = d->part; q->blocks_per_group = d->blocks_per_group; q->sums = d->sums; q->batch_stats = d->batch_stats;
  q->s2d_a = S2D{0, 0, 0, 0};
  q->s2d_da = S2D{0, 0, 0, 0};
  MI355_REQUIRE(!d->q8 || (d->dtype == MI355_DT_BF16 && d->c == 32 && d->ld8 >= d->c && d->ld8 % 8 == 0 && d->q_use && d->q_next &&
                           !d->s2d_a && !d->s2d_da),
                "%s: the e4m3 copy is written for plain bf16 tensors of 32 channels (q8, q_use, q_next)", who);
  q->q8 = (uint8_t*)d->q8; q->ld8 = d->ld8; q->q_use = d->q_use; q->q_next = d->q_next;
  MI355_REQUIRE(!d->gz || (d->dtype == MI355_DT_BF16 && !d->da && !d->s2d_da && d->gw && d->gk > 0 && d->gk <= 8 && d->ldgz >= 8 &&
                           d->ldgz % 8 == 0 && d->gw_ld > 0 && d->c <= kImplicitMaxC),
                "%s: the implicit 1x1x1 data gradient needs bf16, gz rows of >= 8 channels, gk <= 8 and no da", who);
  q->gz = (const char*)d->gz; q->ldgz = d->ldgz; q->gw = d->gw; q->gw_ld = d->gw_ld; q->gk = d->gk;
  MI355_REQUIRE(!d->fy || (d->dtype == MI355_DT_BF16 && d->gw && d->gk > 0 && d->gk <= 8 && d->gw_ld > 0 && d->c == 32 &&
                           d->fcp >= 8 && d->fcp % 8 == 0 && d->fcp <= d->c && d->ldfy >= d->fcp && d->ldfy % 8 == 0 && !d->s2d_a &&
                           !d->q8 && d->ldz % 8 == 0 && (d->skip_a || d->lda % 8 == 0)),
                "%s: the fused 1x1x1 convolution needs bf16, 32 channels, gk <= 8 outputs in rows of fcp (8 .. 32) channels", who);
  MI355_REQUIRE(!d->skip_a || d->fy, "%s: skip_a without the fused convolution", who);
  q->fy = (char*)d->fy; q->ldfy = d->ldfy; q->fcp = d->fcp; q->fbias = d->fbias; q->skip_a = d->skip_a;
  MI355_REQUIRE(!d->pool_idx || (d->pool_dy && !d->gz && !d->s2d_da && !d->s2d_a && d->sd >= 2 && d->sh >= 2 && d->sw >= 2 &&
                                 !((d->sd | d->sh | d->sw) & 1) && d->ldpdy >= d->c && d->ldpdy % (d->dtype == MI355_DT_F32 ? 4 : 8) == 0 &&
                                 ((long long)d->rows_per_group * d->groups) % ((long long)d->sd * d->sh * d->sw) == 0 &&
                                 (long long)d->rows_per_group * d->groups < (1ll << 31) && (!d->da || d->ldda >= d->c)),
                "%s: the implicit max-pool gradient needs pool_dy, even extents sd/sh/sw that divide the row count, and plain layouts", who);
  q->pool_idx = (const uint8_t*)d->pool_idx; q->pool_dy = (const char*)d->pool_dy; q->ldpdy = d->ldpdy;
  q->pd = d->sd; q->ph = d->sh; q->pw = d->sw;
  MI355_REQUIRE(!d->pool_y || (d->pool_widx && !d->pool_idx && !d->s2d_a && !d->s2d_da && !d->q8 && !d->fy && d->a && d->sd >= 2 &&
                               d->sh >= 2 && d->sw >= 2 && !((d->sd | d->sh | d->sw) & 1) && d->ldpy >= d->c &&
                               d->ldpy % (d->dtype == MI355_DT_F32 ? 4 : 8) == 0 &&
                               d->rows_per_group % ((long long)d->sd * d->sh * d->sw) == 0),
                "%s: the fused max-pool needs pool_widx, even extents sd/sh/sw that divide the row count, and plain layouts", who);
  q->pool_y = (char*)d->pool_y; q->ldpy = d->ldpy; q->pool_widx = (uint8_t*)d->pool_widx;
  if (d->s2d_a || d->s2d_da) {
    MI355_REQUIRE((long long)d->sd * d->sh * d->sw * (d->groups == 1 ? 1 : 1) > 0 &&
                  ((long long)d->rows_per_group * d->groups) % ((long long)d->sd * d->sh * d->sw) == 0,
                  "%s: space-to-depth extents do not match the row count", who);
    if (d->s2d_a) { int rc2 = check_s2d(d->sd, d->sh, d->sw, d->c, d->lda, who); if (rc2) return rc2; q->s2d_a = S2D{d->sd, d->sh, d->sw, d->c}; }
    if (d->s2d_da) { int rc2 = check_s2d(d->sd, d->sh, d->sw, d->c, d->ldda, who); if (rc2) return rc2; q->s2d_da = S2D{d->sd, d->sh, d->sw, d->c}; }
  }
  return MI355_OK;
}

static unsigned stream_blocks(long long rows, int c, int dtype) {
  const int epv = dtype == MI355_DT_F32 ? 4 : 8;
  const int rpp = 256 / (c / epv);
  long long b = (rows + (long long)rpp * 8 - 1) / ((long long)rpp * 8);
  if (b < 1) b = 1;
  if (b > 1024) b = 1024;
  return (unsigned)b;
}

int mi355_normact_fwd(const mi355_normact_desc* d, void* stream) {
  NormActArgs q;
  int rc = fill_normact(d, &q, "normact_fwd");
  if (rc) return rc;
  MI355_REQUIRE((d->a && d->lda >= d->c) || d->skip_a, "normact_fwd: bad output");
  dim3 grid(stream_blocks(d->rows_per_group, d->c, d->dtype), d->groups);
  if (q.pool_y) {
    const long long dhw = (long long)d->sd * d->sh * d->sw, samples = (long long)d->rows_per_group * d->groups / dhw;
    const int epv = d->dtype == MI355_DT_F32 ? 4 : 8, vpp = 256 / (d->c / epv);
    long long b = (dhw / 8 + vpp - 1) / vpp;
    const long long cap = std::max(1ll, 2048 / samples);
    if (b > cap) b = cap;
    const dim3 gridp((unsigned)b, (unsigned)samples);
    if (d->dtype == MI355_DT_F32) {
      if (q.thr16) normact_pool_fwd_kernel<float, true><<<gridp, dim3(256), 0, (hipStream_t)stream>>>(q);
      else normact_pool_fwd_kernel<float, false><<<gridp, dim3(256), 0, (hipStream_t)stream>>>(q);
    } else {
      if (q.thr16) normact_pool_fwd_kernel<bf16_t, true><<<gridp, dim3(256), 0, (hipStream_t)stream>>>(q);
      else normact_pool_fwd_kernel<bf16_t, false><<<gridp, dim3(256), 0, (hipStream_t)stream>>>(q);
    }
    return mi355_check_launch("normact_pool_fwd");
  }
  if (d->dtype == MI355_DT_F32) {
    if (q.thr16) normact_fwd_kernel<float, true><<<grid, dim3(256), 0, (hipStream_t)stream>>>(q);
    else normact_fwd_kernel<float, false><<<grid, dim3(256), 0, (hipStream_t)stream>>>(q);
  } else if (q.fy) {
    MI355_REQUIRE(d->fcp == 16, "normact_fwd: the fused convolution writes 16-channel rows");
    long long b = (d->rows_per_group + 64 * 8 - 1) / (64 * 8);
    const dim3 grid32((unsigned)(b < 1 ? 1 : (b > 2048 ? 2048 : b)), d->groups);
    if (q.thr16) normact_fwd_final32_kernel<true><<<grid32, dim3(256), 0, (hipStream_t)stream>>>(q);
    else normact_fwd_final32_kernel<false><<<grid32, dim3(256), 0, (hipStream_t)stream>>>(q);
  } else {
    if (q.thr16) normact_fwd_kernel<bf16_t, true><<<grid, dim3(256), 0, (hipStream_t)stream>>>(q);
    else normact_fwd_kernel<bf16_t, false><<<grid, dim3(256), 0, (hipStream_t)stream>>>(q);
  }
  return mi355_check_launch("normact_fwd");
}

int mi355_normact_bwd_reduce(const mi355_normact_desc* d, void* stream) {
  NormActArgs q;
  int rc = fill_normact(d, &q, "normact_bwd_reduce");
  if (rc) return rc;
  MI355_REQUIRE((d->gz || d->pool_idx || (d->da && d->ldda >= d->c)) && d->part && d->blocks_per_group > 0, "normact_bwd_reduce: bad argument");
  dim3 grid(d->blocks_per_group, d->groups);
  if (q.pool_idx) {
    if (d->dtype == MI355_DT_F32) {
      if (q.thr16) normact_bwd_reduce_kernel<float, true, 2><<<grid, dim3(256), 0, (hipStream_t)stream>>>(q);
      else normact_bwd_reduce_kernel<float, false, 2><<<grid, dim3(256), 0, (hipStream_t)stream>>>(q);
    } else {
      if (q.thr16) normact_bwd_reduce_kernel<bf16_t, true, 2><<<grid, dim3(256), 0, (hipStream_t)stream>>>(q);
      else normact_bwd_reduce_kernel<bf16_t, false, 2><<<grid, dim3(256), 0, (hipStream_t)stream>>>(q);
    }
  } else if (d->dtype == MI355_DT_F32) {
    if (q.thr16) normact_bwd_reduce_kernel<float, true><<<grid, dim3(256), 0, (hipStream_t)stream>>>(q);
    else normact_bwd_reduce_kernel<float, false><<<grid, dim3(256), 0, (hipStream_t)stream>>>(q);
  } else if (q.gz) {
    if (q.thr16) normact_bwd_reduce_kernel<bf16_t, true, 1><<<grid, dim3(256), 0, (hipStream_t)stream>>>(q);
    else normact_bwd_reduce_kernel<bf16_t, false, 1><<<grid, dim3(256), 0, (hipStream_t)stream>>>(q);
  } else {
    if (q.thr16) normact_bwd_reduce_kernel<bf16_t, true><<<grid, dim3(256), 0, (hipStream_t)stream>>>(q);
    else normact_bwd_reduce_kernel<bf16_t, false><<<grid, dim3(256), 0, (hipStream_t)stream>>>(q);
  }
  return mi355_check_launch("normact_bwd_reduce");
}

int mi355_normact_bwd_finalize(const float* part, int32_t blocks_per_group, int32_t groups, int32_t c, float* sums,
                               float* dgamma, float* dbeta, void* stream) {
  return mi355_normact_bwd_finalize_into(part, blocks_per_group, groups, c, sums, dgamma, dbeta, c, 0, stream);
}

int mi355_normact_bwd_finalize_into(const float* part, int32_t blocks_per_group, int32_t groups, int32_t c, float* sums,
                                    float* dgamma, float* dbeta, int32_t n_affine, int32_t accumulate, void* stream) {
  MI355_REQUIRE(part && sums && blocks_per_group > 0 && groups > 0 && c > 0 && n_affine > 0 && n_affine <= c,
                "normact_bwd_finalize: bad argument");
  hipLaunchKernelGGL(normact_bwd_finalize_kernel, dim3((c + 7) / 8), dim3(1024), 0, (hipStream_t)stream, part,
                     blocks_per_group, groups, c, sums, dgamma, dbeta, n_affine, accumulate);
  return mi355_check_launch("normact_bwd_finalize");
}

int mi355_normact_bwd_apply(const mi355_normact_desc* d, void* stream) {
  NormActArgs q;
  int rc = fill_normact(d, &q, "normact_bwd_apply");
  if (rc) return rc;
  MI355_REQUIRE((d->gz || d->pool_idx || (d->da && d->ldda >= d->c)) && d->dz && d->lddz >= d->c, "normact_bwd_apply: bad argument");
  MI355_REQUIRE(!(d->mean && d->batch_stats) || d->sums, "normact_bwd_apply: sums required");
  dim3 grid(stream_blocks(d->rows_per_group, d->c, d->dtype), d->groups);
  if (q.pool_idx) {
    if (d->dtype == MI355_DT_F32) {
      if (q.thr16) normact_bwd_apply_kernel<float, true, 2><<<grid, dim3(256), 0, (hipStream_t)stream>>>(q);
      else normact_bwd_apply_kernel<float, false, 2><<<grid, dim3(256), 0, (hipStream_t)stream>>>(q);
    } else {
      if (q.thr16) normact_bwd_apply_kernel<bf16_t, true, 2><<<grid, dim3(256), 0, (hipStream_t)stream>>>(q);
      else normact_bwd_apply_kernel<bf16_t, false, 2><<<grid, dim3(256), 0, (hipStream_t)stream>>>(q);
    }
  } else if (d->dtype == MI355_DT_F32) {
    if (q.thr16) normact_bwd_apply_kernel<float, true><<<grid, dim3(256), 0, (hipStream_t)stream>>>(q);
    else normact_bwd_apply_kernel<float, false><<<grid, dim3(256), 0, (hipStream_t)stream>>>(q);
  } else if (q.gz) {
    if (q.thr16) normact_bwd_apply_kernel<bf16_t, true, 1><<<grid, dim3(256), 0, (hipStream_t)stream>>>(q);
    else normact_bwd_apply_kernel<bf16_t, false, 1><<<grid, dim3(256), 0, (hipStream_t)stream>>>(q);
  } else {
    if (q.thr16) normact_bwd_apply_kernel<bf16_t, true><<<grid, dim3(256), 0, (hipStream_t)stream>>>(q);
    else normact_bwd_apply_kernel<bf16_t, false><<<grid, dim3(256), 0, (hipStream_t)stream>>>(q);
  }
  return mi355_check_launch("normact_bwd_apply");
}

int mi355_normact_small_fwd(const mi355_normact_small_desc* d, void* stream) {
  NormSmallArgs p;
  MI355_REQUIRE(d, "normact_small_fwd: null pointer");
  int rc = fill_normact(&d->base, &p.q, "normact_small_fwd");
  if (rc) return rc;
  MI355_REQUIRE(d->base.a && d->base.lda >= d->base.c && d->mean_out && d->rstd_out, "normact_small_fwd: bad output");
  MI355_REQUIRE(!d->running_mean || d->running_var, "normact_small_fwd: running_mean without running_var");
  p.eps = d->eps; p.momentum = d->momentum; p.mean_out = d->mean_out; p.rstd_out = d->rstd_out;
  p.running_mean = d->running_mean; p.running_var = d->running_var; p.batches_tracked = (long long*)d->batches_tracked;
  p.n_real = d->n_real > 0 ? d->n_real : d->base.c;
  p.dgamma = p.dbeta = nullptr; p.accumulate = 0;
  const int epv = d->base.dtype == MI355_DT_F32 ? 4 : 8;
  dim3 grid(d->base.c / epv);
  if (p.q.rows_per_group <= 8ll * kSmallThreads && p.q.groups <= kSmallResMaxGroups) {
    const int s_slots = p.q.rows_per_group <= kSmallThreads ? 1 : 8, chunk = p.q.groups % 2 == 0 ? 2 : 1;
    if (!p.running_mean) grid.y = (unsigned)(p.q.groups / chunk);
    if (d->base.dtype == MI355_DT_F32) {
      if (p.q.thr16) MI355_SMALL_RES_LAUNCH(normact_small_res_fwd_kernel, float, true, 2);
      else MI355_SMALL_RES_LAUNCH(normact_small_res_fwd_kernel, float, false, 2);
    } else {
      if (p.q.thr16) MI355_SMALL_RES_LAUNCH(normact_small_res_fwd_kernel, bf16_t, true, 2);
      else MI355_SMALL_RES_LAUNCH(normact_small_res_fwd_kernel, bf16_t, false, 2);
    }
    return mi355_check_launch("normact_small_fwd");
  }
  if (d->base.dtype == MI355_DT_F32) {
    if (p.q.thr16) normact_small_fwd_kernel<float, true><<<grid, dim3(kSmallThreads), 0, (hipStream_t)stream>>>(p);
    else normact_small_fwd_kernel<float, false><<<grid, dim3(kSmallThreads), 0, (hipStream_t)stream>>>(p);
  } else {
    if (p.q.thr16) normact_small_fwd_kernel<bf16_t, true><<<grid, dim3(kSmallThreads), 0, (hipStream_t)stream>>>(p);
    else normact_small_fwd_kernel<bf16_t, false><<<grid, dim3(kSmallThreads), 0, (hipStream_t)stream>>>(p);
  }
  return mi355_check_launch("normact_small_fwd");
}

int mi355_normact_small_bwd(const mi355_normact_small_desc* d, void* stream) {
  NormSmallArgs p;
  MI355_REQUIRE(d, "normact_small_bwd: null pointer");
  int rc = fill_normact(&d->base, &p.q, "normact_small_bwd");
  if (rc) return rc;
  MI355_REQUIRE(d->base.da && d->base.dz && d->base.mean, "normact_small_bwd: null pointer");
  p.eps = d->eps; p.momentum = 0.f; p.mean_out = p.rstd_out = nullptr;
  p.running_mean = p.running_var = nullptr; p.batches_tracked = nullptr; p.n_real = 0;
  p.dgamma = d->dgamma; p.dbeta = d->dbeta; p.accumulate = d->accumulate;
  const int epv = d->base.dtype == MI355_DT_F32 ? 4 : 8;
  dim3 grid(d->base.c / epv);
  if (p.q.rows_per_group <= 8ll * kSmallThreads && p.q.groups <= kSmallResMaxGroups) {
    const int s_slots = p.q.rows_per_group <= kSmallThreads ? 1 : 8, chunk = p.q.groups % 2 == 0 ? 2 : 1;
    const bool split = d->base.part != nullptr && p.q.groups / chunk > 1;
    if (split) grid.y = (unsigned)(p.q.groups / chunk); else p.q.part = nullptr;
    if (d->base.dtype == MI355_DT_F32) {
      if (p.q.thr16) MI355_SMALL_RES_LAUNCH(normact_small_res_bwd_kernel, float, true, 1);
      else MI355_SMALL_RES_LAUNCH(normact_small_res_bwd_kernel, float, false, 1);
    } else {
      if (p.q.thr16) MI355_SMALL_RES_LAUNCH(normact_small_res_bwd_kernel, bf16_t, true, 1);
      else MI355_SMALL_RES_LAUNCH(normact_small_res_bwd_kernel, bf16_t, false, 1);
    }
    if (split && (p.dgamma || p.dbeta) && p.q.n_affine > 0)
      normact_small_affine_kernel<<<dim3((p.q.n_affine + 255) / 256), dim3(256), 0, (hipStream_t)stream>>>(
          reinterpret_cast<const double*>(d->base.part), p.q.groups, p.q.c, p.q.n_affine, p.dgamma, p.dbeta, p.accumulate);
    return mi355_check_launch("normact_small_bwd");
  }
  if (d->base.dtype == MI355_DT_F32) {
    if (p.q.thr16) normact_small_bwd_kernel<float, true><<<grid, dim3(kSmallThreads), 0, (hipStream_t)stream>>>(p);
    else normact_small_bwd_kernel<float, false><<<grid, dim3(kSmallThreads), 0, (hipStream_t)stream>>>(p);
  } else {
    if (p.q.thr16) normact_small_bwd_kernel<bf16_t, true><<<grid, dim3(kSmallThreads), 0, (hipStream_t)stream>>>(p);
    else normact_small_bwd_kernel<bf16_t, false><<<grid, dim3(kSmallThreads), 0, (hipStream_t)stream>>>(p);
  }
  return mi355_check_launch("normact_small_bwd");
}

int mi355_maxpool2_fwd(const void* x, int32_t ldx, void* y, int32_t ldy, int32_t n, int32_t c, int32_t d, int32_t h,
                       int32_t w, int32_t dtype, void* stream) {
  return mi355_maxpool2_fwd_idx(x, ldx, y, ldy, nullptr, n, c, d, h, w, dtype, stream);
}

// ... 295 lines not shown
```

### unet_bssfp_amd/functional.py

```python
from __future__ import annotations

import os
import weakref
from typing import Optional

import torch
from torch.autograd import Function
from torch.autograd.function import once_differentiable

from . import ops
from .gradsink import sink_grad, sink_of
from .ops import round_up

CLASSES8 = [(a, b, c) for a in (0, 1) for b in (0, 1) for c in (0, 1)]

_WEIGHT_EPOCH = 0


def bump_weight_epoch():
    global _WEIGHT_EPOCH
    _WEIGHT_EPOCH += 1


class LayerCache:
# ... 214 lines not shown
        s = cls.Slot(table[len(slots)], sat[len(slots): len(slots) + 1])
        slots.append(s)
        return s

    @classmethod
    def advance(cls, device):
        for table, slots, sat in cls._chunks.get(device, ()):
            if any(s.touched for s in slots):
                ops.fp8_scale_roll(table, len(slots), sat)
                for s in slots:
                    s.primed, s.touched = s.primed or s.touched, False
        Fp8Side.clear()

    @classmethod
    def primed_slots(cls, device) -> set:
        return {id(s) for _, slots, _ in cls._chunks.get(device, ()) for s in slots if s.primed or s.touched}

    @classmethod
    def check_capture(cls, device, primed_before: set):
        bad = sum(1 for _, slots, _ in cls._chunks.get(device, ()) for s in slots if s.touched and id(s) not in primed_before)
        if bad:
            raise RuntimeError(f"fp8 delayed scaling: {bad} operand slot(s) were used for the first time inside a hipGraph capture; "
                               "run the step eagerly (at least twice) before capturing it")

    @classmethod
    def saturated_steps(cls, device=None) -> int:
        total = 0
        for dev, chunks in cls._chunks.items():
            if device is None or torch.device(dev) == torch.device(device):
                total += sum(int(sat[: len(slots)].sum()) for _, slots, sat in chunks)
        return total


class Fp8Side:
    _by_ptr = {}

    @classmethod
    def put(cls, t: torch.Tensor, t8: torch.Tensor):
        if len(cls._by_ptr) >= 32:
            cls._by_ptr.clear()
        cls._by_ptr[t.data_ptr()] = (t8, tuple(t.shape), t)

    @classmethod
    def take(cls, t: torch.Tensor, keep: bool = False) -> Optional[torch.Tensor]:
        hit = cls._by_ptr.get(t.data_ptr()) if keep else cls._by_ptr.pop(t.data_ptr(), None)
        return hit[0] if hit is not None and hit[1] == tuple(t.shape) else None

    @classmethod
    def clear(cls):
        cls._by_ptr.clear()


class ColSumSide:
    _by_ptr = {}
    enabled = True

    @classmethod
    def put(cls, t: torch.Tensor, part: torch.Tensor, offset: int):
        if len(cls._by_ptr) >= 32:
            cls._by_ptr.clear()
        cls._by_ptr[t.data_ptr()] = (part, offset, tuple(t.shape), t)

    @classmethod
    def take(cls, t: torch.Tensor):
        hit = cls._by_ptr.pop(t.data_ptr(), None)
        return (hit[0], hit[1]) if hit is not None and hit[2] == tuple(t.shape) else None

    @classmethod
    def clear(cls):
        cls._by_ptr.clear()


class LazyDx:
    _by_ptr = {}
    enabled = True

    @classmethod
    def put(cls, placeholder: torch.Tensor, gz: torch.Tensor, gw: torch.Tensor):
        if len(cls._by_ptr) >= 8:
            cls._by_ptr.clear()
        cls._by_ptr[placeholder.data_ptr()] = (gz, gw, tuple(placeholder.shape), placeholder)

    @classmethod
    def take(cls, t: torch.Tensor):
        hit = cls._by_ptr.pop(t.data_ptr(), None)
        return (hit[0], hit[1]) if hit is not None and hit[2] == tuple(t.shape) else None

    @classmethod
    def clear(cls):
        cls._by_ptr.clear()


class LazyPool:
    _by_ptr = {}
    enabled = True

    @classmethod
    def put(cls, placeholder, x, y, idx, d_pool, d_skip):
        if len(cls._by_ptr) >= 8:
            cls._by_ptr.clear()
        cls._by_ptr[placeholder.data_ptr()] = (x, y, idx, d_pool, d_skip, tuple(placeholder.shape), placeholder)

    @classmethod
    def take(cls, t):
        hit = cls._by_ptr.pop(t.data_ptr(), None)
        return hit[:5] if hit is not None and hit[5] == tuple(t.shape) else None

    @classmethod
    def clear(cls):
        cls._by_ptr.clear()


class PoolSide:
    _by_ptr = {}
    enabled = True

    @classmethod
    def put(cls, a, y, idx):
        if len(cls._by_ptr) >= 8:
            cls._by_ptr.clear()
        cls._by_ptr[a.data_ptr()] = (y, idx, tuple(a.shape), a)

    @classmethod
    def take(cls, a):
        hit = cls._by_ptr.pop(a.data_ptr(), None)
        return (hit[0], hit[1]) if hit is not None and hit[2] == tuple(a.shape) else None

    @classmethod
    def clear(cls):
        cls._by_ptr.clear()


class FusedFinal:
    _by_ptr = {}

    @classmethod
    def put(cls, a: torch.Tensor, y: torch.Tensor, w: torch.Tensor):
        if len(cls._by_ptr) >= 8:
            cls._by_ptr.clear()
        cls._by_ptr[a.data_ptr()] = (y, w, w._version, tuple(a.shape), a)

    @classmethod
    def take(cls, a: torch.Tensor, w: torch.Tensor):
        hit = cls._by_ptr.pop(a.data_ptr(), None)
        if hit is None:
            return None
        if hit[3] != tuple(a.shape) or hit[1].data_ptr() != w.data_ptr() or hit[2] != w._version:
            raise RuntimeError("FusedFinal: the convolution that takes the precomputed output is not the one it was computed for")
        return hit[0]

    @classmethod
    def clear(cls):
        cls._by_ptr.clear()


def fp8_operand(x: torch.Tensor, slot: "Fp8Scales.Slot", constant: bool = False) -> torch.Tensor:
    x8 = Fp8Side.take(x, keep=constant)
    if x8 is not None:
        return x8
    if slot.primed:
        x8 = ops.cast_fp8(x, slot.use, slot.next)
    else:
        ops.amax_act(x, out=slot.use)
        torch.maximum(slot.next, slot.use, out=slot.next)
        x8 = ops.cast_fp8(x, slot.use)
    slot.touched = True
    if constant:
        Fp8Side.put(x, x8)
    return x8


class PackMemo:
    _store = {}

    @classmethod
    def get(cls, x, cp, dtype):
        e = cls._store.get((id(x), cp, dtype))
        if e is not None and e[0]() is x and e[1] == x._version:
            return e[2]
        return None

    @classmethod
    def put(cls, x, cp, dtype, act):
        if len(cls._store) >= 8:
            cls._store.clear()
        cls._store[(id(x), cp, dtype)] = (weakref.ref(x), x._version, act)

    @classmethod
    def holds(cls, act) -> bool:
        return any(e[2].data_ptr() == act.data_ptr() for e in cls._store.values())

    @classmethod
    def clear(cls):
        cls._store.clear()


class PackFn(Function):

    @staticmethod
    def forward(ctx, cp, dtype, *srcs):
        s2d = cp < 0
        cp = abs(cp)
        ctx.s2d = s2d
        n, _, d, h, w = srcs[0].shape
        ctx.dims = (d, h, w)
        epv = 4 if dtype == torch.float32 else 8
        ctx.split = None
        if len(srcs) > 1 and any(s.shape[1] % epv for s in srcs[:-1]):
            ctx.split = [s.shape[1] for s in srcs]
            srcs = (torch.cat([s.detach().to(torch.float32) for s in srcs], dim=1),)
        if s2d:
            out = _new_s2d(ops.s2d_shape(n, d, h, w, cp), dtype, srcs[0].device)
        else:
            out = ops.new_act(n, d, h, w, cp, dtype, srcs[0].device)
        offs, off = [], 0
        if len(srcs) == 2:
            s0, s1 = (t.detach().to(torch.float32).contiguous() for t in srcs)
            ops.pack2(s0, s1, out, 0, cp, s2d_cblk=cp if s2d else 0)
            ctx.offs = [(0, s0.shape[1]), (s0.shape[1], s1.shape[1])]
            return out
        for i, s in enumerate(srcs):
            c = s.shape[1]
            last = i == len(srcs) - 1
            s32 = s.detach().to(torch.float32).contiguous()
            if s2d:
                ops.pack_ncdhw_s2d(s32, out, cp, off, cp if last else off + c)
            else:
                ops.pack_ncdhw(s32, out, off, cp if last else off + c)
            offs.append((off, c))
            off += c
        ctx.offs = offs
        return out

    @staticmethod
    @once_differentiable
    def backward(ctx, g):
        g = ops.as_act(g)
        grads = []
        if ctx.s2d:
            cp = g.shape[4] // 8
            if ctx.split is not None:
                full = ops.unpack_ncdhw_s2d(g, sum(ctx.split), ctx.dims, cp, 0)
                pieces = torch.split(full, ctx.split, dim=1)
                return (None, None, *[pc.contiguous() if ctx.needs_input_grad[2 + i] else None for i, pc in enumerate(pieces)])
            for i, (off, c) in enumerate(ctx.offs):
                grads.append(ops.unpack_ncdhw_s2d(g, c, ctx.dims, cp, off) if ctx.needs_input_grad[2 + i] else None)
            return (None, None, *grads)
        if ctx.split is not None:
            full = ops.unpack_ncdhw(g, sum(ctx.split), 0)
            pieces = torch.split(full, ctx.split, dim=1)
            grads = [pc.contiguous() if ctx.needs_input_grad[2 + i] else None for i, pc in enumerate(pieces)]
            return (None, None, *grads)
        for i, (off, c) in enumerate(ctx.offs):
            grads.append(ops.unpack_ncdhw(g, c, off) if ctx.needs_input_grad[2 + i] else None)
        return (None, None, *grads)


class UnpackFn(Function):

    @staticmethod
    def forward(ctx, act, c):
        ctx.meta = (act.shape[4], act.dtype)
        return ops.unpack_ncdhw(act, c, 0)

    @staticmethod
    @once_differentiable
    def backward(ctx, g):
        cp, dtype = ctx.meta
        n, c, d, h, w = g.shape
        out = ops.new_act(n, d, h, w, cp, dtype, g.device)
        ops.pack_ncdhw(g.to(torch.float32).contiguous(), out, 0, cp)
        return out, None


class GenOutFn(Function):

    @staticmethod
    def forward(ctx, act, c, cblk):
        act = ops.as_act(act)
        ctx.meta = (tuple(act.shape), act.dtype, c)
        ctx.set_materialize_grads(False)
        return ops.unpack_ncdhw(act, c, 0), ops.s2d_repack(act, cblk)

    @staticmethod
    @once_differentiable
    def backward(ctx, gy, gs):
        shape, dtype, c = ctx.meta
        if gy is None and gs is None:
            return None, None, None
        out = torch.empty(shape, dtype=dtype, device=(gy if gy is not None else gs).device)
        ops.seam_grad(gy.to(torch.float32).contiguous() if gy is not None else None, ops.as_act(gs) if gs is not None else None, out, c, shape[1:4])
        return out, None, None


class ConvSpec:

    def __init__(self, kind, cin, cout, ks, stride, pad):
        assert kind in ("conv", "deconv2")
        self.kind, self.cin, self.cout, self.ks, self.stride, self.pad = kind, cin, cout, ks, stride, pad
        self.cache = LayerCache()

    def w_fwd(self, w, dtype, cinp):
        k = self.ks
        return self.cache.get(("fwd", dtype, cinp), w, lambda r: ops.weight_pack(
            w.detach(), self.cout, self.cin, k, self.cin * k ** 3, k ** 3, (k * k, k, 1), (0, 0, 0), (1, 1, 1),
            dtype, cinp, reuse=r))

    def w_dgrad_s1(self, w, dtype, cinp, coutp_min):
        k = self.ks
        return self.cache.get(("dgrad", dtype, cinp), w, lambda r: ops.weight_pack(
            w.detach(), self.cin, self.cout, k, k ** 3, self.cin * k ** 3, (k * k, k, 1), (k - 1,) * 3, (-1,) * 3,
            dtype, cinp, reuse=r))

    def fp8_slot(self, role: str, device) -> "Fp8Scales.Slot":
        slots = self.__dict__.setdefault("_fp8_slots", {})
        key = (role, device)
        if key not in slots:
            slots[key] = Fp8Scales.slot(device)
        return slots[key]

    def _fp8(self, key, w, builder):
        def build(reuse):
            amax = ops.amax_f32(w.detach(), out=self._amax.get(key))
            self._amax[key] = amax
            packed, coutp, cinp = builder(reuse, amax)
            return packed, coutp, cinp, amax
        if not hasattr(self, "_amax"):
            self._amax = {}
        return self.cache.get(key, w, build)

    def w_fwd8(self, w, cinp):
        k = self.ks
        return self._fp8(("fwd8", cinp), w, lambda r, amax: ops.weight_pack(
            w.detach(), self.cout, self.cin, k, self.cin * k ** 3, k ** 3, (k * k, k, 1), (0, 0, 0), (1, 1, 1),
            ops.FP8, cinp, reuse=r, q_amax=amax))

    def w_dgrad8(self, w, cinp):
        k = self.ks
        return self._fp8(("dgrad8", cinp), w, lambda r, amax: ops.weight_pack(
            w.detach(), self.cin, self.cout, k, k ** 3, self.cin * k ** 3, (k * k, k, 1), (k - 1,) * 3, (-1,) * 3,
            ops.FP8, cinp, reuse=r, q_amax=amax))

    def w_dgrad_s2(self, w, dtype, cinp, cls):
        k = self.ks
        tb = tuple(3 if p == 0 else 2 for p in cls)
        return self.cache.get(("dgrad2", dtype, cinp, cls), w, lambda r: ops.weight_pack(
            w.detach(), self.cin, self.cout, 2, k ** 3, self.cin * k ** 3, (k * k, k, 1), tb, (-2,) * 3, dtype, cinp, reuse=r))

    def w_deconv_fwd(self, w, dtype, cinp, cls):
        return self.cache.get(("dfwd", dtype, cinp, cls), w, lambda r: ops.weight_pack(
            w.detach(), self.cout, self.cin, 1, 8, self.cout * 8, (4, 2, 1), cls, (0, 0, 0), dtype, cinp, reuse=r))

    def w_deconv_fwd_all(self, w, dtype, cinp):
        return self.cache.get(("dfwd_all", dtype, cinp), w, lambda r: ops.weight_pack(
            w.detach(), self.cout, self.cin, 1, 8, self.cout * 8, (4, 2, 1), (0, 0, 0), (0, 0, 0), dtype, cinp,
            coutp=8 * self.cout, s2d_mode=2, s2d_cp=self.cout, reuse=r))

    def w_deconv_dgrad(self, w, dtype, cinp):
        return self.cache.get(("ddgrad", dtype, cinp), w, lambda r: ops.weight_pack(
            w.detach(), self.cin, self.cout, 2, self.cout * 8, 8, (4, 2, 1), (0, 0, 0), (1, 1, 1), dtype, cinp, reuse=r))

    def w_fwd_s2d(self, w, dtype, cp):
        k = self.ks
        return self.cache.get(("fwd_s2d", dtype, cp), w, lambda r: ops.weight_pack(
            w.detach(), self.cout, self.cin, 2, self.cin * k ** 3, k ** 3, (k * k, k, 1), (0, 0, 0), (2, 2, 2),
            dtype, cinp=8 * cp, s2d_mode=1, s2d_cp=cp, reuse=r))

    def w_dgrad_s2d(self, w, dtype, cinp, cp):
        k = self.ks
        return self.cache.get(("dgrad_s2d", dtype, cinp, cp), w, lambda r: ops.weight_pack(
            w.detach(), self.cin, self.cout, 2, k ** 3, self.cin * k ** 3, (k * k, k, 1), (2, 2, 2), (-2, -2, -2),
            dtype, cinp=cinp, coutp=8 * cp, s2d_mode=2, s2d_cp=cp, reuse=r))

    def w_fwd_part(self, w, dtype, cinp, c_off, c_n):
        k = self.ks
        return self.cache.get(("fwd_part", dtype, cinp, c_off, c_n), w, lambda r: ops.weight_pack(
            w.detach(), self.cout, c_n, k, self.cin * k ** 3, k ** 3, (k * k, k, 1), (0, 0, 0), (1, 1, 1),
            dtype, cinp, reuse=r, src_offset=c_off * k ** 3))

    def w_dgrad_s1_part(self, w, dtype, cinp, c_off, c_n):
        k = self.ks
        return self.cache.get(("dgrad_part", dtype, cinp, c_off, c_n), w, lambda r: ops.weight_pack(
            w.detach(), c_n, self.cout, k, k ** 3, self.cin * k ** 3, (k * k, k, 1), (k - 1,) * 3, (-1,) * 3,
            dtype, cinp, reuse=r, src_offset=c_off * k ** 3))

    def w_fwd_s2d_part(self, w, dtype, cp, c_off, c_n):
        k = self.ks
        return self.cache.get(("fwd_s2d_part", dtype, cp, c_off, c_n), w, lambda r: ops.weight_pack(
            w.detach(), self.cout, c_n, 2, self.cin * k ** 3, k ** 3, (k * k, k, 1), (0, 0, 0), (2, 2, 2),
            dtype, cinp=8 * cp, s2d_mode=1, s2d_cp=cp, reuse=r, src_offset=c_off * k ** 3))

    def w_dgrad_s2d_part(self, w, dtype, cinp, cp, c_off, c_n):
        k = self.ks
        return self.cache.get(("dgrad_s2d_part", dtype, cinp, cp, c_off, c_n), w, lambda r: ops.weight_pack(
            w.detach(), c_n, self.cout, 2, k ** 3, self.cin * k ** 3, (k * k, k, 1), (2, 2, 2), (-2, -2, -2),
            dtype, cinp=cinp, coutp=8 * cp, s2d_mode=2, s2d_cp=cp, reuse=r, src_offset=c_off * k ** 3))

    def out_extent(self, e):
        if self.kind == "deconv2":
            return 2 * e
        return (e + 2 * self.pad - self.ks) // self.stride + 1


class ConvFn(Function):
    wgrad_first = False

    @staticmethod
    def forward(ctx, x0, x1, weight, bias, spec: ConvSpec, want_stats: bool, zero_bias_grad: bool = False,
                s2d_cp: int = 0, fp8: bool = False, lazy_dx: bool = False):
        x0 = ops.as_act(x0)
        x1 = ops.as_act(x1) if x1 is not None else None
        n, di, hi, wi, c0 = x0.shape
        c1 = x1.shape[4] if x1 is not None else 0
        dtype, dev = x0.dtype, x0.device
        cp = round_up(spec.cout, 16)
        ctx.s2d_cp = s2d_cp
        if s2d_cp:
            assert spec.kind == "conv" and spec.ks == 4 and spec.stride == 2 and spec.pad == 1 and x1 is None
            assert c0 == 8 * s2d_cp
            do_, ho, wo = di - 1, hi - 1, wi - 1
        else:
            do_, ho, wo = (spec.out_extent(e) for e in (di, hi, wi))
        out = ops.new_act(n, do_, ho, wo, cp, dtype, dev)
        part = None
        if s2d_cp:
            wp, coutp, _ = spec.w_fwd_s2d(weight, dtype, s2d_cp)
            bp = bias.detach() if bias is not None else None
            if want_stats:
                tiles, _ = ops.conv_num_tiles(x0, None, wp, coutp, 2, 1, (0, 0, 0), out, (do_, ho, wo))
                part = torch.empty((tiles, 2, coutp), dtype=torch.float32, device=dev)
            ops.conv_fwd(x0, None, wp, coutp, bp, 2, 1, (0, 0, 0), out, (do_, ho, wo), stats=part,
                         real=(spec.cin, spec.cout))
        elif (fp8 and spec.kind == "conv" and spec.ks == 3 and spec.stride == 1 and spec.pad == 1 and x1 is None
              and dtype == torch.bfloat16 and ops.conv_fp8_supported(x0, round_up(spec.cout, 32), out, (do_, ho, wo))):
# ... 288 lines not shown
        return None, dsy, dw, db, None, None, None, None


class UpCatTables:

    def __init__(self):
        self.tag = None
        self.bufs = None
        self.wpk = None

    def stale(self, wd, bd, wc, bc) -> bool:
        return self.tag != tuple(LayerCache._tag(t) for t in (wd, wc, bd, bc) if t is not None)

    def get(self, wd, bd, wc, bc, ce, dtype):
        tag = tuple(LayerCache._tag(t) for t in (wd, wc, bd, bc) if t is not None)
        if tag != self.tag:
            self.bufs = ops.upcat_compose(wd.detach(), wc.detach(), bd.detach(), bc.detach() if bc is not None else None, ce, out=self.bufs)
            k4 = self.bufs[0]
            cl, co = k4.shape[:2]
            self.wpk = ops.weight_pack(k4, cl, co, 2, co * 64, 64, (16, 4, 1), (0, 0, 0), (2, 2, 2), dtype, cinp=8 * co, s2d_mode=1,
                                       s2d_cp=co, reuse=self.wpk[0] if self.wpk is not None else None)
            self.tag = tag
            self.args = (wd, bd, wc, bc, ce, dtype)
        return self.bufs, self.wpk

    def refresh(self):
        if self.tag is not None:
            self.get(*self.args)


class UpCatConvFn(Function):

    @staticmethod
    def forward(ctx, x_e, x_low, wd, bd, wc, bc, spec_c: ConvSpec, tables: UpCatTables, want_stats: bool):
        x_e, x_low = ops.as_act(x_e), ops.as_act(x_low)
        n, D, H, W, ce = x_e.shape
        cl = x_low.shape[4]
        co = spec_c.cout
        assert tuple(x_low.shape[1:4]) == (D // 2, H // 2, W // 2) and wc.shape[1] == ce + wd.shape[1] and co % 32 == 0
        dtype, dev = x_e.dtype, x_e.device
        (k4, wp, biasp, delta), _ = tables.get(wd, bd, wc, bc, ce, dtype)
        wps, coutp, _ = spec_c.w_fwd_part(wc, dtype, ce, 0, ce)
        p_skip = ops.new_act(n, D, H, W, co, dtype, dev)
        ops.conv_fwd(x_e, None, wps, coutp, None, 3, 1, (1, 1, 1), p_skip, (D, H, W), real=(ce, co))
        out = ops.new_act(n, D, H, W, co, dtype, dev)
        grid = (D // 2, H // 2, W // 2)
        part = None
        if want_stats:
            tiles, _ = ops.conv_num_tiles(x_low, None, wp, 8 * co, 2, 1, (0, 0, 0), out, grid, addend=p_skip, d2s=True)
            part = torch.empty((tiles, 2, co), dtype=torch.float32, device=dev)
        ops.conv_fwd(x_low, None, wp, 8 * co, biasp, 2, 1, (0, 0, 0), out, grid, stats=part, addend=p_skip, d2s=True, delta=delta,
                     real=(cl, 8 * co))
        ctx.save_for_backward(x_e, x_low, wd, wc, bd)
        ctx.spec_c, ctx.tables = spec_c, tables
        ctx.params = (wd, bd, wc, bc)
        if part is None:
            part = torch.empty((0,), dtype=torch.float32, device=dev)
        ctx.mark_non_differentiable(part)
        ctx.set_materialize_grads(False)
        return out, part

    @staticmethod
    @once_differentiable
    def backward(ctx, dz, _dpart):
        if dz is None:
            return (None,) * 9
        x_e, x_low, wd, wc, bd = ctx.saved_tensors
        spec_c: ConvSpec = ctx.spec_c
        dz = ops.as_act(dz)
        n, D, H, W, ce = x_e.shape
        cl, co = x_low.shape[4], spec_c.cout
        cu = wd.shape[1]
        dtype, dev = x_e.dtype, x_e.device
        grid = (D // 2, H // 2, W // 2)
        (k4, _, _, _), wpk = ctx.tables.get(wd, bd, wc, ctx.params[3], ce, dtype)
        dx_e = dx_low = dwd = dbd = dwc = dbc = None
        if ctx.needs_input_grad[0]:
            wp, coutp, _ = spec_c.w_dgrad_s1_part(wc, dtype, dz.shape[4], 0, ce)
            dx_e = ops.new_act(n, D, H, W, ce, dtype, dev)
            ops.conv_fwd(dz, None, wp, coutp, None, 3, 1, (1, 1, 1), dx_e, (D, H, W), real=(co, ce))
        need_w = ctx.needs_input_grad[2] or ctx.needs_input_grad[4] or ctx.needs_input_grad[3]
        sg = ops.s2d_repack(dz) if (ctx.needs_input_grad[1] or need_w) else None
        if ctx.needs_input_grad[1]:
            dx_low = ops.new_act(n, *grid, cl, dtype, dev)
            ops.conv_fwd(sg, None, wpk[0], wpk[1], None, 2, 1, (0, 0, 0), dx_low, grid, real=(co, cl))
        if need_w:
            wd_p, bd_p, wc_p, bc_p = ctx.params

            def target(p):
                sink = sink_of(p)
                if sink is not None:
                    return sink, sink_grad(p), not sink.fresh(p)
                return None, torch.empty_like(p, dtype=torch.float32), False
            sk_c, dwc_t, acc_c = target(wc_p)
            sk_d, dwd_t, acc_d = target(wd_p)
            sk_b, dbd_t, acc_b = target(bd_p)
            assert acc_c == acc_d == acc_b, "the UpCat block's parameters are used together"
            ops.conv_wgrad(x_e, None, dz, (D, H, W), 1, (0, 0, 0), 3, 1, (1, 1, 1), dwc_t, co, ce, (ce + cu) * 27, 27, (9, 3, 1),
                           (0, 0, 0), (1, 1, 1), accumulate=acc_c)
            dk4 = torch.empty_like(k4)
            ops.conv_wgrad(sg, None, x_low, grid, 1, (0, 0, 0), 2, 1, (0, 0, 0), dk4, cl, co, co * 64, 64, (16, 4, 1), (0, 0, 0), (2, 2, 2),
                           s2d_cp=co)
            esum = ops.border_sums(dz, co)
            ops.upcat_chain(dk4, wd.detach(), wc.detach(), bd.detach(), esum, ce, dwd_t, dwc_t, dbd_t, acc_c)
            for sk, p in ((sk_c, wc_p), (sk_d, wd_p), (sk_b, bd_p)):
                if sk is not None:
                    sk.written(p)
            dwc = None if sk_c is not None else dwc_t
            dwd = None if sk_d is not None else dwd_t
            dbd = None if sk_b is not None else dbd_t
            if bc_p is not None and ctx.needs_input_grad[5]:
                bsink = sink_of(bc_p)
                if bsink is not None:
                    bsink.written(bc_p)
                else:
                    dbc = _cached_zeros(co, dev)
        return dx_e, dx_low, dwd, dbd, dwc, dbc, None, None, None


class NormCfg:
    def __init__(self, kind, channels, eps=1e-5, momentum=0.1, slope=1.0, p=0.0):
        assert kind in ("instance", "batch", "none")
        self.kind, self.channels, self.eps, self.momentum, self.slope, self.p = kind, channels, eps, momentum, slope, p


class DropoutState:
    _base = {}
    _salt = 0

    @classmethod
    def base(cls, device) -> torch.Tensor:
        t = cls._base.get(device)
        if t is None:
            t = torch.randint(0, 2 ** 40, (1,), dtype=torch.int64).to(device)
            cls._base[device] = t
        return t

    @classmethod
    def next_salt(cls) -> int:
        cls._salt += 1
        return cls._salt

    @classmethod
    def advance(cls, device):
        cls.base(device).add_(1)
        cls._salt = 0
        PackMemo.clear()
        StepMemo.clear()
        ColSumSide.clear()
        LazyDx.clear()
        LazyPool.clear()
        PoolSide.clear()
        FusedFinal.clear()
        Fp8Scales.advance(device)

    @classmethod
    def reset(cls):
        cls._base.clear()
        cls._salt = 0


class NormActFn(Function):

    @staticmethod
    def forward(ctx, z, part, gamma, beta, conv_bias, cfg: NormCfg, training, running_mean, running_var,
                s2d_out: bool = False, batches_tracked=None, small: bool = False, bn_groups: int = 1,
                emit8=None, emit8_bwd=None, final=None, pool_after: bool = False):
        z = ops.as_act(z)
        n, d, h, w, c = z.shape
        rows = n * d * h * w
        use_batch = cfg.kind == "instance" or (cfg.kind == "batch" and (training or running_mean is None))
        groups = n if cfg.kind == "instance" else (bn_groups if (cfg.kind == "batch" and use_batch) else 1)
        assert n % groups == 0
        mean = rstd = None
        batch_stats = False
        ctx.small = False
        ctx.emit8_bwd = emit8_bwd if (emit8_bwd is not None and emit8_bwd.primed and not small and not s2d_out) else None
        if emit8 is not None and not (emit8.primed and not small and not s2d_out and z.dtype == torch.bfloat16 and c == 32):
            emit8 = None
        if small and cfg.kind != "none" and use_batch:
            if rows // groups <= 1:
                raise ValueError(f"Expected more than 1 value per channel when training, got input size {tuple(z.shape)}")
            gp = gamma.detach() if gamma is not None else None
            bp = beta.detach() if beta is not None else None
            p = cfg.p if training else 0.0
            seed = DropoutState.next_salt() if p > 0.0 else 0
            seed_t = DropoutState.base(z.device) if p > 0.0 else None
            upd = cfg.kind == "batch" and training and running_mean is not None
            out = _new_s2d(ops.s2d_shape(n, d, h, w, c), z.dtype, z.device) if s2d_out else None
            a, mean, rstd = ops.normact_small_fwd(z, groups, gp, bp, cfg.eps, cfg.slope, p, seed, seed_t,
                                                  running_mean if upd else None, running_var if upd else None, cfg.momentum,
                                                  batches_tracked if upd else None, out=out, s2d=s2d_out)
            ctx.small = True
            ctx.s2d_out = s2d_out
            ctx.seed_t = seed_t
            ctx.affine_params = (gamma, beta)
            ctx.save_for_backward(z, mean, rstd, gp, bp)
            ctx.meta = (groups, cfg.slope, p, seed, True, gamma.numel() if gamma is not None else 0)
            return a
        if cfg.kind != "none":
            if use_batch:
                if rows // groups <= 1:
                    raise ValueError(f"Expected more than 1 value per channel when training, got input size {tuple(z.shape)}")
                if part is not None and part.numel() > 0:
                    assert part.shape[2] == c, "fused statistics need coutp == padded channels"
                    ppg = part.shape[0] // groups
                    shift = conv_bias.detach() if conv_bias is not None else None
                else:
                    part, ppg = ops.channel_stats(z, groups)
                    shift = None
                upd = cfg.kind == "batch" and training and running_mean is not None
                n_real = running_mean.numel() if upd else (shift.numel() if shift is not None else 0)
                mean, rstd = ops.norm_finalize(part, ppg, groups, c, rows // groups, shift, cfg.eps,
                                               running_mean if upd else None, running_var if upd else None,
                                               cfg.momentum, n_real=n_real,
                                               batches_tracked=batches_tracked if upd else None)
                batch_stats = True
            else:
                mean = _padded(running_mean, c).reshape(1, c)
                rstd = torch.rsqrt(_padded(running_var, c, 1.0) + cfg.eps).reshape(1, c)
        gp = gamma.detach() if gamma is not None else None
        bp = beta.detach() if beta is not None else None
        p = cfg.p if training else 0.0
        seed = DropoutState.next_salt() if p > 0.0 else 0
        seed_t = DropoutState.base(z.device) if p > 0.0 else None
        if s2d_out:
            out = _new_s2d(ops.s2d_shape(n, d, h, w, c), z.dtype, z.device)
            a = ops.normact_fwd(z, groups, mean, rstd, gp, bp, cfg.slope, p, seed, out=out, s2d=True, seed_t=seed_t)
        elif emit8 is not None:
            a8 = torch.empty(z.shape, dtype=torch.uint8, device=z.device)
            a = ops.normact_fwd(z, groups, mean, rstd, gp, bp, cfg.slope, p, seed, seed_t=seed_t, q8=(a8, emit8.use, emit8.next))
            emit8.touched = True
            Fp8Side.put(a, a8)
        elif final is not None and z.dtype == torch.bfloat16 and c == 32:
            fw, fb, skip_a = final
            y = ops.new_act(n, d, h, w, round_up(fw.shape[0], 16), z.dtype, z.device)
            a = ops.normact_fwd(z, groups, mean, rstd, gp, bp, cfg.slope, p, seed, seed_t=seed_t,
                                final=(fw.detach(), fb.detach() if fb is not None else None, y), skip_a=skip_a)
            FusedFinal.put(a, y, fw)
        elif (pool_after and PoolSide.enabled and not s2d_out and emit8 is None and d % 2 == 0 and h % 2 == 0 and w % 2 == 0
              and (rows // groups) % (d * h * w) == 0):
            a, py, pidx = ops.normact_fwd(z, groups, mean, rstd, gp, bp, cfg.slope, p, seed, seed_t=seed_t, pool=True)
            PoolSide.put(a, py, pidx)
        else:
            a = ops.normact_fwd(z, groups, mean, rstd, gp, bp, cfg.slope, p, seed, seed_t=seed_t)
        ctx.s2d_out = s2d_out
        ctx.seed_t = seed_t
        ctx.affine_params = (gamma, beta)
        ctx.save_for_backward(z, mean, rstd, gp, bp)
        ctx.meta = (groups, cfg.slope, p, seed, batch_stats, gamma.numel() if gamma is not None else 0)
        return a

    @staticmethod
    @once_differentiable
    def backward(ctx, da):
        z, mean, rstd, gp, bp = ctx.saved_tensors
        groups, slope, p, seed, batch_stats, nch = ctx.meta
        da = ops.as_act(da)
        lazy = LazyDx.take(da)
        if lazy is not None:
            if ctx.small or ctx.s2d_out:
                raise RuntimeError("LazyDx placeholder reached a norm node that cannot form the gradient itself")
            da = None
        pool = None
        lp = LazyPool.take(da) if da is not None else None
        if lp is not None:
            if ctx.small or ctx.s2d_out:
                da = ops.maxpool2_bwd(lp[0], lp[1], lp[3], lp[4])
            else:
                pool, da = (lp[2], lp[3]), lp[4]
        want_affine = ctx.needs_input_grad[2] or ctx.needs_input_grad[3]
        gamma_p, beta_p = ctx.affine_params
        sink = sink_of(gamma_p) if (ctx.needs_input_grad[2] and ctx.needs_input_grad[3] and mean is not None) else None
        slot8 = ctx.emit8_bwd if (not ctx.small and z.dtype == torch.bfloat16 and z.shape[4] == 32) else None
        q8 = (torch.empty(z.shape, dtype=torch.uint8, device=z.device), slot8.use, slot8.next) if slot8 is not None else None

        def done(dz):
            if q8 is not None:
                slot8.touched = True
                Fp8Side.put(dz, q8[0])
            return dz
        if ctx.small:
            none11 = (None,) * 16
            if sink is not None and sink_of(beta_p) is sink:
                dz, _, _ = ops.normact_small_bwd(z, da, groups, mean, rstd, gp, bp, slope, p, seed, batch_stats, s2d=ctx.s2d_out,
                                                 seed_t=ctx.seed_t, affine_into=(sink_grad(gamma_p), sink_grad(beta_p)),
                                                 accumulate=not sink.fresh(gamma_p))
                sink.written(gamma_p)
                sink.written(beta_p)
                return (dz,) + none11
            dz, dgamma, dbeta = ops.normact_small_bwd(z, da, groups, mean, rstd, gp, bp, slope, p, seed, batch_stats,
                                                      s2d=ctx.s2d_out, seed_t=ctx.seed_t, want_affine=want_affine)
            dg = dgamma[:nch].contiguous() if (dgamma is not None and ctx.needs_input_grad[2]) else None
            dbt = dbeta[:nch].contiguous() if (dbeta is not None and ctx.needs_input_grad[3]) else None
            return (dz, None, dg, dbt) + (None,) * 13
        if sink is not None and sink_of(beta_p) is sink:
            dz, _, _ = ops.normact_bwd(z, da, groups, mean, rstd, gp, bp, slope, p, seed, batch_stats, True,
                                       s2d=ctx.s2d_out, seed_t=ctx.seed_t, affine_into=(sink_grad(gamma_p), sink_grad(beta_p)),
                                       accumulate=not sink.fresh(gamma_p), q8=q8, implicit=lazy, pool=pool)
            sink.written(gamma_p)
            sink.written(beta_p)
            return (done(dz),) + (None,) * 16
        dz, dgamma, dbeta = ops.normact_bwd(z, da, groups, mean, rstd, gp, bp, slope, p, seed, batch_stats,
                                            want_affine and mean is not None, s2d=ctx.s2d_out, seed_t=ctx.seed_t, q8=q8,
                                            implicit=lazy, pool=pool)
        dg = dgamma[:nch].contiguous() if (dgamma is not None and ctx.needs_input_grad[2]) else None
        dbt = dbeta[:nch].contiguous() if (dbeta is not None and ctx.needs_input_grad[3]) else None
        return (done(dz), None, dg, dbt) + (None,) * 13


class MaxPoolFn(Function):
    @staticmethod
    def forward(ctx, x):
        x = ops.as_act(x)
        y = ops.maxpool2_fwd(x)
        ctx.save_for_backward(x, y)
        return y

    @staticmethod
    @once_differentiable
    def backward(ctx, dy):
        x, y = ctx.saved_tensors
        return ops.maxpool2_bwd(x, y, ops.as_act(dy))


class SkipPoolFn(Function):

    @staticmethod
    def forward(ctx, x, lazy=False):
        x = ops.as_act(x)
        n, d, h, w, c = x.shape
        ctx.lazy = bool(lazy and LazyPool.enabled and d % 2 == 0 and h % 2 == 0 and w % 2 == 0)
        side = PoolSide.take(x)
        if side is not None:
            y, idx = side
            ctx.save_for_backward(*((x, y, idx) if ctx.lazy else (x, y)))
        elif ctx.lazy:
            y, idx = ops.maxpool2_fwd(x, want_idx=True)
            ctx.save_for_backward(x, y, idx)
        else:
            y = ops.maxpool2_fwd(x)
            ctx.save_for_backward(x, y)
        ctx.set_materialize_grads(False)
        return x.view_as(x), y

    @staticmethod
    @once_differentiable
    def backward(ctx, d_skip, d_pool):
        if d_pool is None:
            return d_skip, None
        x, y = ctx.saved_tensors[:2]
        add = None
        if d_skip is not None:
            add = d_skip if d_skip.stride(4) == 1 and d_skip.dtype == x.dtype else ops.as_act(d_skip)
        if ctx.lazy:
            ph = torch.empty(x.shape, dtype=x.dtype, device=x.device)
            LazyPool.put(ph, x, y, ctx.saved_tensors[2], ops.as_act(d_pool), add)
            return ph, None
        return ops.maxpool2_bwd(x, y, ops.as_act(d_pool), add), None

    @classmethod
    def apply_to(cls, x):
        fnode = x.grad_fn
        return cls.apply(x, fnode is not None and type(fnode).__name__ == "NormActFnBackward")


class L1LossFn(Function):

    @staticmethod
    def forward(ctx, a, b):
        a = a.contiguous()
        b = b.contiguous()
        ctx.save_for_backward(a, b)
        return ops.l1_fwd(a, b)

    @staticmethod
    @once_differentiable
    def backward(ctx, g):
        a, b = ctx.saved_tensors
        da = ops.l1_bwd(a, b, g)
        return (da if ctx.needs_input_grad[0] else None, (-da) if ctx.needs_input_grad[1] else None)


def l1_loss(a: torch.Tensor, b: torch.Tensor) -> torch.Tensor:
    return L1LossFn.apply(a, b)


class GanGenLossFn(Function):

    @staticmethod
    def forward(ctx, logits, y_hat, y, divisor: float, factor: float):
        logits, y_hat, y = logits.contiguous(), y_hat.contiguous(), y.contiguous()
# ... 45 lines not shown
```

### unet_bssfp_amd/gan.py

```python
from __future__ import annotations

from collections import OrderedDict
from typing import Callable, Dict, Optional

import torch
import torch.nn as nn
import torch.nn.functional as F

DATA = "data"


def dist_world(group=None) -> int:
    import torch.distributed as dist
    return dist.get_world_size(group) if dist.is_available() and dist.is_initialized() else 1

LOG_KEYS = ("train_gen_loss_adversarial", "train_gen_loss_recon_L1", "train_gen_loss_recon", "train_gen_loss",
            "train_discr_loss")


class bSSFPToDWITensorModel(nn.Module):
    def __init__(self, input_modality, lr=1e-3, batch_size=8, perceptual_factor=1e3, recon_factor=1e2,
                 gen: Optional[nn.Module] = None, discr: Optional[nn.Module] = None,
                 l1_fn: Optional[Callable] = None, optimizer_class=None,
                 extra_recon_terms: Optional[Dict[str, Callable]] = None, recon_divisor: Optional[int] = None,
                 reference_quirks: bool = False):
        super().__init__()
        self.input_modality = input_modality
        if gen is None or discr is None:
            from .nn import Discriminator, Generator
            gen = Generator(input_modality) if gen is None else gen
            discr = Discriminator(input_modality) if discr is None else discr
        self.gen, self.discr = gen, discr
        self.recon_factor, self.lr, self.batch_size = recon_factor, lr, batch_size
        self.perceptual_factor = perceptual_factor
        self.l1_fn = l1_fn
        self.extra_recon_terms = extra_recon_terms or {}
        self.optimizer_class = optimizer_class
        self.recon_divisor = recon_divisor
        self.reference_quirks = reference_quirks
        self.grad_sync_gen = None
        self.grad_sync_discr = None
        self.sinks_gen = None
        self.sinks_discr = None
        self.use_grad_sinks = True
        self._stage = None
        self._optimizers = None
        self.last_logs: Dict[str, torch.Tensor] = {}

    def forward(self, x):
        return self.gen(x)

    def configure_optimizers(self):
        cls = self.optimizer_class
        if cls is None:
            from .optim import FusedAdamW
            cls = FusedAdamW if next(self.gen.parameters()).is_cuda else torch.optim.AdamW
        return cls(self.gen.parameters(), lr=self.lr), cls(self.discr.parameters(), lr=self.lr)

    def optimizers(self):
        if self._optimizers is None:
            self._optimizers = self.configure_optimizers()
        return self._optimizers

    def unpack_batch(self, batch, test=False):
        x = batch[self.input_modality][DATA]
        y = batch["dwi-tensor" if test else "dwi-tensor_orig"][DATA]
        return x, y

    def _l1(self, a, b):
        if self.l1_fn is not None:
            return self.l1_fn(a, b)
        if a.is_cuda:
            from .functional import l1_loss
            return l1_loss(a, b)
        return F.l1_loss(a, b)

    def compute_recon_loss(self, y_hat, y, logs, prefix):
        terms = OrderedDict(L1=self._l1(y_hat, y))
        for name, fn in self.extra_recon_terms.items():
            terms[name] = fn(y_hat, y)
        total = None
        for name, t in terms.items():
            logs[f"{prefix}_loss_recon_{name}"] = t.detach()
            total = t if total is None else total + t
        total = total / (self.recon_divisor or len(terms)) * self.recon_factor
        logs[f"{prefix}_loss_recon"] = total.detach()
        return total

    fused_loss_heads = True

    def _fused_losses(self, *tensors) -> bool:
        return (self.fused_loss_heads and self.l1_fn is None and not self.extra_recon_terms
                and all(t.is_cuda and t.dtype == torch.float32 for t in tensors))

    def _gen_for_discr(self, x):
        if hasattr(self.gen, "emit_s2d") and next(self.gen.parameters()).is_cuda:
            self.gen.emit_s2d = True
            try:
                return self.gen(x)
            finally:
                self.gen.emit_s2d = False
        return self.gen(x)

    @staticmethod
    def _detach(y):
        out = y.detach()
        s = getattr(y, "_mi355_s2d", None)
        if s is not None:
            out._mi355_s2d = s.detach()
        return out

    def _gen_step(self, x, y, logs, step_name="train"):
        y_hat = self._gen_for_discr(x)
        logits = self.discr(x, y_hat)
        if self._fused_losses(logits, y_hat, y):
            from .functional import GanGenLossFn
            total, parts = GanGenLossFn.apply(logits, y_hat, y, float(self.recon_divisor or 1), float(self.recon_factor))
            logs[f"{step_name}_gen_loss_recon_L1"] = parts[0]
            logs[f"{step_name}_gen_loss_recon"] = parts[1]
            logs[f"{step_name}_gen_loss_adversarial"] = parts[2]
            return total, y_hat
        adv = F.binary_cross_entropy_with_logits(logits, torch.ones_like(logits))
        recon = self.compute_recon_loss(y_hat, y, logs, step_name + "_gen")
        logs[f"{step_name}_gen_loss_adversarial"] = adv.detach()
        return adv + recon, y_hat

    pair_discriminator_calls = True

    def _discr_pair(self) -> bool:
        return self.pair_discriminator_calls and hasattr(self.discr, "forward_pair") and next(self.discr.parameters()).is_cuda

    def _discr_uses(self, x, y) -> int:
        if self._discr_pair() and self.discr.pair_single_pass(x, x.new_empty(0), y):
            return 1
        return 2

    def _discr_step(self, x, y):
        y_hat = self._detach(self._gen_for_discr(x))
        if self._discr_pair():
            both = self.discr.forward_pair(x, y_hat, y, stacked=self._fused_losses(x, y))
            if isinstance(both, torch.Tensor):
                from .functional import GanDiscrLossFn
                return GanDiscrLossFn.apply(both, None)
            logits_hat, logits = both
        else:
            logits_hat = self.discr(x, y_hat)
            logits = self.discr(x, y)
        if self._fused_losses(logits_hat, logits):
            from .functional import GanDiscrLossFn
            return GanDiscrLossFn.apply(logits_hat, logits)
        loss_hat = F.binary_cross_entropy_with_logits(logits_hat, torch.zeros_like(logits_hat))
        loss = F.binary_cross_entropy_with_logits(logits, torch.ones_like(logits))
        return (loss + loss_hat) / 2

    @staticmethod
    def _repack(module: nn.Module):
        if next(module.parameters()).is_cuda:
            from .functional import repack_weights
            repack_weights(module)

    @staticmethod
    def _toggle(module: nn.Module, flag: bool):
        for p in module.parameters():
            p.requires_grad_(flag)

    def enable_grad_sinks(self, group=None, distributed: bool = False, force_collectives: bool = False) -> bool:
        if self.sinks_gen is not None:
            want = distributed and (dist_world(group) > 1 or force_collectives)
            if not want or self.sinks_gen.exchange:
                return True
            self.sinks_gen.detach()
            self.sinks_discr.detach()
            self.sinks_gen = self.sinks_discr = None
        if not self.use_grad_sinks:
            return False
        from .nn import Discriminator, Generator, backward_stages
        if not (isinstance(self.gen, Generator) and isinstance(self.discr, Discriminator) and next(self.gen.parameters()).is_cuda):
            return False
        from .gradsink import GradBuckets
        self.sinks_gen = GradBuckets(backward_stages(self.gen, self.input_modality), group, uses_per_phase=1,
                                     distributed=distributed, force_collectives=force_collectives)
        self.sinks_discr = GradBuckets(backward_stages(self.discr, self.input_modality), group, uses_per_phase=2,
                                       distributed=distributed, force_collectives=force_collectives)
        return True

    def _finish_grads(self, which: str):
        sinks = self.sinks_gen if which == "gen" else self.sinks_discr
        sync = self.grad_sync_gen if which == "gen" else self.grad_sync_discr
        if sinks is not None:
            sinks.finish()
        elif sync is not None:
            sync.finish()

    def _backward(self, loss, staged: bool):
        if not staged:
            with self._side_scope():
                loss.backward()
            return
        from .functional import StageBoundary
        boundary = StageBoundary.end()
        sinks = self._stage_sinks
        late = [p for p in sinks.params[0] if p.requires_grad]
        with self._side_scope():
            grads = torch.autograd.grad([loss], boundary + late, retain_graph=True, allow_unused=True)
        assert all(g is None for g in grads[len(boundary):]), "staged backward needs gradient sinks"
        self._stage = (boundary, list(grads[: len(boundary)]), [p for p in sinks.params[1] if p.requires_grad])

    def _side_scope(self):
        import contextlib
        import sys
        fn = sys.modules.get(__package__ + ".functional")
        if fn is None or self.sinks_gen is None:
            return contextlib.nullcontext()
        stack = contextlib.ExitStack()
        stack.enter_context(fn.SideStream.scope())
        stack.enter_context(fn.DeferredReduce.scope())
        return stack

    @staticmethod
    def _close_stage_boundary():
        import sys
        fn = sys.modules.get(__package__ + ".functional")
        if fn is not None and fn.StageBoundary.active():
            fn.StageBoundary.end()

    def _backward_early(self):
        boundary, grads, early = self._stage
        self._stage = None
        with self._side_scope():
            torch.autograd.backward(boundary, grads, inputs=early)

    def _phase_gen(self, batch, logs, staged=False):
        x, y = self.unpack_batch(batch)
        if x.is_cuda:
            from .functional import DropoutState, StageBoundary
            DropoutState.advance(x.device)
            if self.enable_grad_sinks():
                self.sinks_gen.begin_phase(1)
            if staged:
                self._stage_sinks = self.sinks_gen
                StageBoundary.begin()
        self._toggle(self.discr, False)
        try:
            loss, _ = self._gen_step(x, y, logs)
            logs["train_gen_loss"] = loss.detach()
            self._backward(loss, staged)
        finally:
            self._close_stage_boundary()

    def _update_gen(self):
        gen_opt, _ = self.optimizers()
        gen_opt.step()
        if self.sinks_gen is None:
            gen_opt.zero_grad()
        self._repack(self.gen)
        self._toggle(self.discr, True)

    def _phase_discr(self, batch, logs, staged=False):
        x, y = self.unpack_batch(batch)
        self._toggle(self.gen, False)
        if self.sinks_discr is not None:
            self.sinks_discr.begin_phase(self._discr_uses(x, y))
        if staged:
            from .functional import StageBoundary
            self._stage_sinks = self.sinks_discr
            StageBoundary.begin()
        try:
            loss = self._discr_step(x, y)
            logs["train_discr_loss"] = loss.detach()
            self._backward(loss, staged)
        finally:
            self._close_stage_boundary()

    def _phase_gen_update_discr(self, batch, logs):
        self._update_gen()
        self._phase_discr(batch, logs)

    def _phase_discr_update(self):
        _, discr_opt = self.optimizers()
        discr_opt.step()
        if self.sinks_discr is None:
            discr_opt.zero_grad()
        self._repack(self.discr)
        self._toggle(self.gen, True)

    def training_step(self, batch, batch_idx=0):
        logs: Dict[str, torch.Tensor] = {}
        self._phase_gen(batch, logs)
        self._finish_grads("gen")
        self._phase_gen_update_discr(batch, logs)
        self._finish_grads("discr")
# ... 240 lines not shown
```

### unet_bssfp_amd/nn.py

```python
from __future__ import annotations

import math
from typing import Optional, Sequence

import torch
import torch.nn as nn

from . import functional as Fn
from . import ops
from .ops import round_up

_DEFAULT_DTYPE = torch.float32


def set_default_compute_dtype(dtype: torch.dtype):
    global _DEFAULT_DTYPE
    assert dtype in (torch.float32, torch.bfloat16)
    _DEFAULT_DTYPE = dtype


FP8 = "fp8"


def compute_dtype_from_name(name):
# ... 28 lines not shown
        ops.require_cuda(x)
        act = getattr(x, "_mi355_act", None)
        if act is not None and act.dtype == self.compute_dtype and (cp is None or act.shape[4] == cp):
            return act
        if x.dim() != 5:
            raise ValueError(f"expected a 5-D (N,C,D,H,W) tensor, got {tuple(x.shape)}")
        cp = round_up(x.shape[1], 16) if cp is None else cp
        if x.requires_grad or torch.is_grad_enabled() and x.grad_fn is not None:
            return Fn.PackFn.apply(cp, self.compute_dtype, x)
        hit = Fn.PackMemo.get(x, cp, self.compute_dtype)
        if hit is None:
            hit = Fn.PackFn.apply(cp, self.compute_dtype, x)
            Fn.PackMemo.put(x, cp, self.compute_dtype, hit)
        return hit

    @staticmethod
    def _from_act(act: torch.Tensor, c: int) -> torch.Tensor:
        v = act.permute(0, 4, 1, 2, 3)
        if c != act.shape[4]:
            v = v[:, :c]
        v._mi355_act = act
        return v


class Conv3d(_Mi355Module):

    def __init__(self, in_channels, out_channels, kernel_size, stride=1, padding=0, bias=True):
        super().__init__()
        k = kernel_size if isinstance(kernel_size, int) else kernel_size[0]
        s = stride if isinstance(stride, int) else stride[0]
        p = padding if isinstance(padding, int) else padding[0]
        self.in_channels, self.out_channels = in_channels, out_channels
        self.kernel_size, self.stride, self.padding = (k,) * 3, (s,) * 3, (p,) * 3
        self.weight = nn.Parameter(torch.empty(out_channels, in_channels, k, k, k))
        self.bias = nn.Parameter(torch.empty(out_channels)) if bias else None
        self.spec = Fn.ConvSpec("conv", in_channels, out_channels, k, s, p)
        self.fp8 = False
        self.reset_parameters()

    def reset_parameters(self):
        nn.init.kaiming_uniform_(self.weight, a=math.sqrt(5))
        if self.bias is not None:
            fan_in, _ = nn.init._calculate_fan_in_and_fan_out(self.weight)
            bound = 1 / math.sqrt(fan_in) if fan_in > 0 else 0
            nn.init.uniform_(self.bias, -bound, bound)

    def forward_act(self, x0, x1=None, want_stats=False, zero_bias_grad=False, s2d_cp=0, lazy_dx=False):
        return Fn.ConvFn.apply(x0, x1, self.weight, self.bias, self.spec, want_stats, zero_bias_grad, s2d_cp, self.fp8, lazy_dx)

    def forward(self, x):
        z, _ = self.forward_act(self._to_act(x))
        return self._from_act(z, self.out_channels)


class ConvTranspose3d(_Mi355Module):

    def __init__(self, in_channels, out_channels, kernel_size=2, stride=2, bias=True):
        super().__init__()
        if kernel_size != 2 or stride != 2:
            raise NotImplementedError("only the k2 s2 transposed convolution of BasicUNet is implemented")
        self.in_channels, self.out_channels = in_channels, out_channels
        self.weight = nn.Parameter(torch.empty(in_channels, out_channels, 2, 2, 2))
        self.bias = nn.Parameter(torch.empty(out_channels)) if bias else None
        self.spec = Fn.ConvSpec("deconv2", in_channels, out_channels, 2, 2, 0)
        self.reset_parameters()

    def reset_parameters(self):
        nn.init.kaiming_uniform_(self.weight, a=math.sqrt(5))
        if self.bias is not None:
            fan_in, _ = nn.init._calculate_fan_in_and_fan_out(self.weight)
            bound = 1 / math.sqrt(fan_in) if fan_in > 0 else 0
            nn.init.uniform_(self.bias, -bound, bound)

    def forward_act(self, x):
        return Fn.ConvFn.apply(x, None, self.weight, self.bias, self.spec, False)[0]

    def forward(self, x):
        return self._from_act(self.forward_act(self._to_act(x)), self.out_channels)


class _NormParams(nn.Module):

    def __init__(self, channels, batch: bool):
        super().__init__()
        self.weight = nn.Parameter(torch.ones(channels))
        self.bias = nn.Parameter(torch.zeros(channels))
        if batch:
            self.register_buffer("running_mean", torch.zeros(channels))
            self.register_buffer("running_var", torch.ones(channels))
            self.register_buffer("num_batches_tracked", torch.tensor(0, dtype=torch.long))


class DownSampleConv(_Mi355Module):

    def __init__(self, in_channels, out_channels, kernel=4, strides=2, padding=1, activation=True, batchnorm=True):
        super().__init__()
        self.activation = activation
        self.batchnorm = batchnorm
        self.conv = Conv3d(in_channels, out_channels, kernel, strides, padding)
        if batchnorm:
            self.bn = _NormParams(out_channels, batch=True)
        self.cfg = Fn.NormCfg("batch" if batchnorm else "none", out_channels, eps=1e-5, momentum=0.1,
                              slope=0.2 if activation else 1.0)

    def forward_act(self, x0, x1=None, s2d_cp=0, s2d_out=False, bn_groups=1, split=None):
        fuse = self.batchnorm and self.training
        n, di, hi, wi = (x1 if split else x0).shape[:4]
        ext = (di - 1, hi - 1, wi - 1) if (s2d_cp or split) else tuple(self.conv.spec.out_extent(e) for e in (di, hi, wi))
        small = fuse and ops.norm_is_small(n, *ext, round_up(self.conv.out_channels, 16), bn_groups)
        if split:
            z, part = Fn.SplitS2dConvFn.apply(x0, x1, self.conv.weight, self.conv.bias, self.conv.spec, split[0], split[1],
                                              fuse and not small)
        else:
            z, part = self.conv.forward_act(x0, x1, want_stats=fuse and not small, zero_bias_grad=fuse, s2d_cp=s2d_cp)
        if not (self.batchnorm or self.activation):
            assert not s2d_out
            return z
        if self.batchnorm:
            return Fn.NormActFn.apply(z, part if (fuse and not small) else None, self.bn.weight, self.bn.bias, self.conv.bias,
                                      self.cfg, self.training, self.bn.running_mean, self.bn.running_var, s2d_out,
                                      self.bn.num_batches_tracked if self.training else None, small, bn_groups)
        return Fn.NormActFn.apply(z, None, None, None, None, self.cfg, self.training, None, None, s2d_out)

    def forward(self, x):
        return self._from_act(self.forward_act(self._to_act(x)), self.conv.out_channels)


class Discriminator(_Mi355Module):

    def __init__(self, modality):
        super().__init__()
        self.modality = modality
        d1_bssfp = DownSampleConv(30, 32, batchnorm=False)
        d1_dwi = DownSampleConv(12, 32, batchnorm=False)
        self.d1 = self.blocks = nn.ModuleDict({"dwi-tensor": d1_dwi, "pc-bssfp": d1_bssfp,
                                               "bssfp": d1_bssfp, "t1w": d1_dwi})
        self.d2 = DownSampleConv(32, 64)
        self.d3 = DownSampleConv(64, 128)
        self.d4 = DownSampleConv(128, 256)
        self.d5 = DownSampleConv(256, 512)
        self.final = Conv3d(512, 1, kernel_size=1)

    def forward(self, x, y):
        ops.require_cuda(x, y)
        cin = x.shape[1] + y.shape[1]
        cp = round_up(cin, 16)
        blocks = (self.d1[self.modality], self.d2, self.d3, self.d4, self.d5)
        if all(e % 32 == 0 for e in x.shape[2:]):
            split = self._split_first_block(x, y, x.shape[0])
            if split:
                h = self._packed_x(x, split[2])
                h1 = self._s2d_of(y, split[3])
            else:
                h = Fn.PackFn.apply(-cp, self.compute_dtype, x, y)
            for i, blk in enumerate(blocks):
                if i == 0 and split:
                    h = blk.forward_act(h, h1, s2d_out=True, split=split[:2])
                else:
                    h = blk.forward_act(h, s2d_cp=cp, s2d_out=i < 4)
                cp = round_up(blk.conv.out_channels, 16)
                if i == 1 and blk.conv.weight.requires_grad:
                    Fn.StageBoundary.mark(h)
        else:
            h = Fn.PackFn.apply(cp, self.compute_dtype, x, y)
            for i, blk in enumerate(blocks):
                h = blk.forward_act(h)
                if i == 1 and blk.conv.weight.requires_grad:
                    Fn.StageBoundary.mark(h)
        z, _ = self.final.forward_act(h)
        return Fn.UnpackFn.apply(z, 1)

    split_first_block = True

    def _split_first_block(self, x, y, n_grid):
        blk = self.d1[self.modality]
        cx, cy = x.shape[1], y.shape[1]
        if (not self.split_first_block or self.compute_dtype != torch.bfloat16 or x.requires_grad or blk.batchnorm
                or blk.conv.in_channels != cx + cy):
            return None
        cpx, cpy = round_up(cx, 16), round_up(cy, 8)
        se = tuple(e // 2 + 1 for e in x.shape[2:])
        coutp = round_up(blk.conv.out_channels, 32)
        if not (ops.conv_k2_marches(x.shape[0], se, 8 * cpx, coutp) and ops.conv_k2_marches(n_grid, se, 8 * cpy, coutp)):
            return None
        return cx, cy, cpx, cpy

    def _s2d_of(self, y, cpy):
        s = getattr(y, "_mi355_s2d", None)
        if s is not None and s.dtype == self.compute_dtype and s.shape[4] == 8 * cpy and s.shape[0] == y.shape[0]:
            return s
        return Fn.PackFn.apply(-cpy, self.compute_dtype, y)

    def _packed_x(self, x, cpx):
        hit = Fn.PackMemo.get(x, -cpx, self.compute_dtype)
        if hit is None:
            plain = Fn.PackMemo.get(x, cpx, self.compute_dtype)
            hit = ops.s2d_repack(plain) if plain is not None else Fn.PackFn.apply(-cpx, self.compute_dtype, x.detach())
            Fn.PackMemo.put(x, -cpx, self.compute_dtype, hit)
        return hit

    @staticmethod
    def pair_single_pass(x, y_a, y_b) -> bool:
        return (all(e % 32 == 0 for e in x.shape[2:])
                and not (x.requires_grad or y_a.requires_grad or y_b.requires_grad))

    def forward_pair(self, x, y_a, y_b, stacked: bool = False):
        ops.require_cuda(x, y_a, y_b)
        n = x.shape[0]
        cin = x.shape[1] + y_a.shape[1]
        cp = round_up(cin, 16)
        blocks = (self.d1[self.modality], self.d2, self.d3, self.d4, self.d5)
        if not self.pair_single_pass(x, y_a, y_b):
            return self(x, y_a), self(x, y_b)
        d, hh, w = x.shape[2:]
        split = self._split_first_block(x, y_a, 2 * n)
        if split:
            h = self._packed_x(x, split[2])
            h1 = Fn._new_s2d(ops.s2d_shape(2 * n, d, hh, w, split[3]), self.compute_dtype, x.device)
            for half, y in enumerate((y_a, y_b)):
                s = getattr(y, "_mi355_s2d", None)
                if s is not None and s.dtype == self.compute_dtype and tuple(s.shape) == tuple(h1[half * n:(half + 1) * n].shape):
                    h1[half * n:(half + 1) * n].copy_(s.detach())
                else:
                    ops.pack_ncdhw_s2d(y.detach().to(torch.float32).contiguous(), h1[half * n:(half + 1) * n], split[3], 0, split[3])
        else:
            h = Fn._new_s2d(ops.s2d_shape(2 * n, d, hh, w, cp), self.compute_dtype, x.device)
            x32 = x.detach().to(torch.float32).contiguous()
            for half, y in enumerate((y_a, y_b)):
                ops.pack2(x32, y.detach().to(torch.float32).contiguous(), h[half * n:(half + 1) * n], 0, cp, s2d_cblk=cp)
        for i, blk in enumerate(blocks):
            if i == 0 and split:
                h = blk.forward_act(h, h1, s2d_out=True, bn_groups=2, split=split[:2])
            else:
                h = blk.forward_act(h, s2d_cp=cp, s2d_out=i < 4, bn_groups=2)
            cp = round_up(blk.conv.out_channels, 16)
            if i == 1 and blk.conv.weight.requires_grad:
                Fn.StageBoundary.mark(h)
        z, _ = self.final.forward_act(h)
        logits = Fn.UnpackFn.apply(z, 1)
        return logits if stacked else (logits[:n], logits[n:])


class _ADN(nn.Module):
    def __init__(self, channels):
        super().__init__()
        self.N = _NormParams(channels, batch=False)


class Convolution(_Mi355Module):

    def __init__(self, cin, cout, dropout, slope=0.1, eps=1e-5):
        super().__init__()
        self.conv = Conv3d(cin, cout, 3, 1, 1, bias=True)
        self.adn = _ADN(cout)
        self.cfg = Fn.NormCfg("instance", cout, eps=eps, slope=slope, p=float(dropout or 0.0))

    def forward_act(self, x0, x1=None, feeds: Optional[Conv3d] = None, up_from=None, final: Optional[Conv3d] = None,
                    pool_after: bool = False):
        n, d, h, w = x0.shape[:4]
        cp = round_up(self.conv.out_channels, 16)
        small = ops.norm_is_small(n, d, h, w, cp)
        shift = self.conv.bias
        if up_from is not None:
            x_low, deconv, tables = up_from
            z, part = Fn.UpCatConvFn.apply(x0, x_low, deconv.weight, deconv.bias, self.conv.weight, self.conv.bias, self.conv.spec,
                                           tables, not small)
            shift = tables.bufs[2]
        else:
            z, part = self.conv.forward_act(x0, x1, want_stats=not small, zero_bias_grad=True)
        emit8 = emit8_bwd = None
        if cp == 32 and z.dtype == torch.bfloat16 and Fn.Fp8Scales.producer_side:
            if feeds is not None and feeds.fp8 and ops.conv_fp8_layer_ok(n, d, h, w, cp, feeds.out_channels):
                emit8 = feeds.spec.fp8_slot("x", z.device)
            cin = x0.shape[4] + (x1.shape[4] if x1 is not None else 0)
            if (self.conv.fp8 and up_from is None and torch.is_grad_enabled() and (x0.requires_grad or (x1 is not None and x1.requires_grad))
                    and ops.conv_fp8_layer_ok(n, d, h, w, cp, cin)):
                emit8_bwd = self.conv.spec.fp8_slot("g", z.device)
        fin = None
        if (final is not None and not small and z.dtype == torch.bfloat16 and cp == 32 and emit8 is None and final.out_channels <= 8
                and final.in_channels <= cp and Fn.LazyDx.enabled):
            fin = (final.weight, final.bias, not torch.is_grad_enabled())
        return Fn.NormActFn.apply(z, part if not small else None, self.adn.N.weight, self.adn.N.bias, shift, self.cfg,
                                  self.training, None, None, False, None, small, 1, emit8, emit8_bwd, fin, pool_after)


class TwoConv(_Mi355Module):
    def __init__(self, cin, cout, dropout):
        super().__init__()
        self.conv_0 = Convolution(cin, cout, dropout)
        self.conv_1 = Convolution(cout, cout, dropout)

    def forward_act(self, x0, x1=None, up_from=None, final=None, pool_after=False):
        return self.conv_1.forward_act(self.conv_0.forward_act(x0, x1, feeds=self.conv_1.conv, up_from=up_from), final=final,
                                       pool_after=pool_after)


class Down(_Mi355Module):
    def __init__(self, cin, cout, dropout):
        super().__init__()
        self.convs = TwoConv(cin, cout, dropout)

    def forward_act(self, x):
        return self.convs.forward_act(Fn.MaxPoolFn.apply(x))

    def forward_skip(self, x, pool_after=False):
        skip, pooled = Fn.SkipPoolFn.apply_to(x)
        return skip, self.convs.forward_act(pooled, pool_after=pool_after)


class _UpSample(nn.Module):
    def __init__(self, cin, cout):
        super().__init__()
        self.deconv = ConvTranspose3d(cin, cout, 2, 2, bias=True)


class UpCat(_Mi355Module):
    def __init__(self, cin, ccat, cout, dropout, halves=True):
        super().__init__()
        cup = cin // 2 if halves else cin
        self.upsample = _UpSample(cin, cup)
        self.convs = TwoConv(ccat + cup, cout, dropout)

    fuse_up_branch = True

    def _fused(self, x, x_e) -> bool:
        deconv, conv = self.upsample.deconv, self.convs.conv_0.conv
        co, cl = conv.out_channels, deconv.in_channels
        return (self.fuse_up_branch and self.compute_dtype == torch.bfloat16 and x.dtype == torch.bfloat16
                and tuple(x_e.shape[1:4]) == tuple(2 * e for e in x.shape[1:4])
                and co == 32 and cl % 32 == 0 and x.shape[4] == cl and x_e.shape[4] % 16 == 0
                and x_e.shape[4] + deconv.out_channels == conv.in_channels and deconv.bias is not None
                and x.shape[3] >= 32 and not ops.norm_is_small(x_e.shape[0], *x_e.shape[1:4], co))

    def forward_act(self, x, x_e, final=None):
        if self._fused(x, x_e):
            if not hasattr(self, "upcat_tables"):
                self.upcat_tables = Fn.UpCatTables()
            return self.convs.forward_act(x_e, None, up_from=(x, self.upsample.deconv, self.upcat_tables), final=final)
        x_0 = self.upsample.deconv.forward_act(x)
        if x_0.shape[1:4] != x_e.shape[1:4]:
            for ax in (1, 2, 3):
                if x_0.shape[ax] + 1 == x_e.shape[ax]:
                    x_0 = torch.cat([x_0, x_0.narrow(ax, x_0.shape[ax] - 1, 1)], ax)
            if x_0.shape[1:4] != x_e.shape[1:4]:
                raise ValueError(f"skip {tuple(x_e.shape[1:4])} and up-sampled map {tuple(x_0.shape[1:4])} differ by more than one")
        return self.convs.forward_act(x_e, x_0, final=final)


class BasicUNet(_Mi355Module):

    lazy_final_dx = True

    def __init__(self, spatial_dims: int = 3, in_channels: int = 1, out_channels: int = 2,
                 features: Sequence[int] = (32, 32, 64, 128, 256, 32),
                 act=("LeakyReLU", {"negative_slope": 0.1, "inplace": True}),
                 norm=("instance", {"affine": True}), bias: bool = True, dropout=0.0, upsample: str = "deconv"):
        super().__init__()
        if spatial_dims not in (2, 3):
            raise NotImplementedError("spatial_dims must be 2 or 3")
        self.spatial_dims = spatial_dims
        rng_state = torch.get_rng_state() if spatial_dims == 2 else None
        if upsample != "deconv" or not bias:
            raise NotImplementedError("only upsample='deconv', bias=True (the reference's configuration)")
        act_name = act[0] if isinstance(act, (tuple, list)) else act
        norm_name = norm[0] if isinstance(norm, (tuple, list)) else norm
        if str(act_name).lower() != "leakyrelu" or str(norm_name).lower() != "instance":
            raise NotImplementedError("only act=LeakyReLU / norm=instance (MONAI defaults used by the reference)")
        f = tuple(features)
        if len(f) != 6:
            raise ValueError("features must have 6 entries")
        self.in_channels, self.out_channels = in_channels, out_channels
        self.conv_0 = TwoConv(in_channels, f[0], dropout)
        self.down_1 = Down(f[0], f[1], dropout)
        self.down_2 = Down(f[1], f[2], dropout)
        self.down_3 = Down(f[2], f[3], dropout)
        self.down_4 = Down(f[3], f[4], dropout)
        self.upcat_4 = UpCat(f[4], f[3], f[3], dropout)
        self.upcat_3 = UpCat(f[3], f[2], f[2], dropout)
        self.upcat_2 = UpCat(f[2], f[1], f[1], dropout)
        self.upcat_1 = UpCat(f[1], f[0], f[5], dropout, halves=False)
        self.final_conv = Conv3d(f[5], out_channels, kernel_size=1)
        if spatial_dims == 2:
            self._make_2d(rng_state)

    _REPL = 16

    def _make_2d(self, rng_state):
        torch.set_rng_state(rng_state)
        for m in self.modules():
            if isinstance(m, (Conv3d, ConvTranspose3d)):
                k = m.weight.shape[-1]
                m.weight = nn.Parameter(torch.empty(*m.weight.shape[:2], k, k))
                nn.init.kaiming_uniform_(m.weight, a=math.sqrt(5))
                if m.bias is not None:
                    fan_in, _ = nn.init._calculate_fan_in_and_fan_out(m.weight)
                    bound = 1 / math.sqrt(fan_in) if fan_in > 0 else 0
                    nn.init.uniform_(m.bias, -bound, bound)

    def _embedded_parameters(self):
        deconv_w = {id(m.weight) for m in self.modules() if isinstance(m, ConvTranspose3d)}
        out = {}
        for name, p in self.named_parameters():
            if p.dim() == 4 and id(p) in deconv_w:
                out[name] = p.unsqueeze(2).expand(-1, -1, 2, -1, -1).contiguous()
            elif p.dim() == 4:
                w = p.unsqueeze(2)
                out[name] = torch.nn.functional.pad(w, (0, 0, 0, 0, 1, 1)) if p.shape[-1] == 3 else w
            else:
                out[name] = p
        return out

    def _forward_2d(self, x):
        if x.dim() != 4:
            raise ValueError(f"spatial_dims=2 expects (N, C, H, W), got {tuple(x.shape)}")
        x3 = x.unsqueeze(2).expand(-1, -1, self._REPL, -1, -1).contiguous()
        y3 = torch.func.functional_call(self, self._embedded_parameters(), (x3,), {"_embedded": True})
        return y3.mean(2)

    def forward_act(self, x):
        d, h, w = x.shape[1:4]
        if min(d, h, w) < 16 or (d >> 4) * (h >> 4) * (w >> 4) < 2:
            raise ValueError(f"four 2x poolings need extents >= 16, and InstanceNorm more than one element at the bottom "
                             f"level; got {tuple(x.shape[1:4])}")
        x0 = self.conv_0.forward_act(x, pool_after=True)
        s0, x1 = self.down_1.forward_skip(x0, pool_after=True)
        s1, x2 = self.down_2.forward_skip(x1, pool_after=True)
        if Fn.StageBoundary.active():
            s0, s1 = s0.view_as(s0), s1.view_as(s1)
            Fn.StageBoundary.mark(x2, s1, s0)
        s2, x3 = self.down_3.forward_skip(x2, pool_after=True)
        s3, x4 = self.down_4.forward_skip(x3)
        u4 = self.upcat_4.forward_act(x4, s3)
        u3 = self.upcat_3.forward_act(u4, s2)
        u2 = self.upcat_2.forward_act(u3, s1)
        lazy = self.lazy_final_dx and u2.dtype == torch.bfloat16
        u1 = self.upcat_1.forward_act(u2, s0, final=self.final_conv if lazy else None)
        z, _ = self.final_conv.forward_act(u1, lazy_dx=lazy and not ops.norm_is_small(*u1.shape))
        return z

    def forward(self, x, _embedded: bool = False):
        if self.spatial_dims == 2 and not _embedded:
            return self._forward_2d(x)
        z = self.forward_act(self._to_act(x, round_up(self.in_channels, 16)))
        return Fn.UnpackFn.apply(z, self.out_channels)


def backward_stages(net: nn.Module, modality):
    if isinstance(net, Generator):
        unet = net.blocks["unet"]
        early_mods = [net.blocks[modality], unet.conv_0, unet.down_1, unet.down_2]
        late_mods = [unet.down_3, unet.down_4, unet.upcat_4, unet.upcat_3, unet.upcat_2, unet.upcat_1, unet.final_conv]
    elif isinstance(net, Discriminator):
        early_mods = [net.d1[modality], net.d2]
        late_mods = [net.d3, net.d4, net.d5, net.final]
    else:
        raise TypeError("backward_stages: Generator or Discriminator expected")
    late = [p for m in reversed(late_mods) for p in reversed(list(m.parameters()))]
    early = [p for m in reversed(early_mods) for p in reversed(list(m.parameters()))]
    return late, early


class Generator(_Mi355Module):

    def __init__(self, input_modality, dropout=0.05, features=(32, 64, 128, 256, 512, 32)):
        super().__init__()
        self.input_modality = input_modality
        dwi_tensor_input = DownSampleConv(6, 24, kernel=1, strides=1, padding=0)
        bssfp_input = DownSampleConv(24, 24, kernel=1, strides=1, padding=0)
        unet = BasicUNet(spatial_dims=3, in_channels=24, out_channels=6, features=features, dropout=dropout)
        self.blocks = nn.ModuleDict({"dwi-tensor": dwi_tensor_input, "pc-bssfp": bssfp_input,
                                     "bssfp": bssfp_input, "t1w": dwi_tensor_input, "unet": unet})

    emit_s2d = False

    def forward(self, x):
        head = self.blocks[self.input_modality]
        a = head.forward_act(head._to_act(x))
        z = self.blocks["unet"].forward_act(a)
        if self.emit_s2d and z.dtype == torch.bfloat16 and all(e % 2 == 0 for e in z.shape[1:4]):
            y, s = Fn.GenOutFn.apply(z, 6, 8)
            y._mi355_s2d = s
            return y
        return Fn.UnpackFn.apply(z, 6)
```

### unet_bssfp_amd/ops.py

```python
from __future__ import annotations

import ctypes as C
from typing import Optional, Sequence, Tuple

import torch

from . import _lib
from ._lib import DT_BF16, DT_F32, DT_FP8

_DT = {torch.float32: DT_F32, torch.bfloat16: DT_BF16}


def round_up(v: int, m: int) -> int:
    return (v + m - 1) // m * m


def _stream() -> int:
    return torch.cuda.current_stream().cuda_stream


def _ptr(t: Optional[torch.Tensor]) -> Optional[int]:
    return None if t is None else t.data_ptr()


# ... 373 lines not shown
    n, d, h, w, c = x.shape
    out = torch.empty((n, d, h, w, c), dtype=torch.uint8, device=x.device)
    _lib.check(_lib.load().mi355_cast_fp8_delayed(x.data_ptr(), act_ld(x), c, n * d * h * w, _DT[x.dtype], amax.data_ptr(),
                                                  _ptr(amax_next), out.data_ptr(), c, _stream()), "cast_fp8")
    return out


def fp8_scale_roll(table: torch.Tensor, n: int, sat: Optional[torch.Tensor] = None):
    require_cuda(table, sat)
    assert table.dtype == torch.float32 and table.is_contiguous() and table.shape[1] == 2 and 0 < n <= table.shape[0]
    assert sat is None or (sat.dtype == torch.int32 and sat.is_contiguous() and sat.numel() >= n)
    _lib.check(_lib.load().mi355_fp8_scale_roll(table.data_ptr(), n, _ptr(sat), _stream()), "fp8_scale_roll")


def conv_fp8_layer_ok(n: int, d: int, h: int, w: int, c_in: int, c_out: int) -> bool:
    if c_in != 32:
        return False
    key = (n, d, h, w, c_in, c_out)
    hit = _FP8_OK.get(key)
    if hit is None:
        d_ = _lib.ConvDesc()
        d_.x0, d_.c0, d_.ld0 = 256, c_in, c_in
        d_.x1, d_.c1, d_.ld1 = None, 0, 0
        d_.n, d_.di, d_.hi, d_.wi = n, d, h, w
        d_.do_, d_.ho, d_.wo = d, h, w
        d_.ks, d_.stride = 3, 1
        d_.pad = (C.c_int32 * 3)(1, 1, 1)
        d_.wp, d_.coutp = 256, round_up(c_out, 32)
        co = round_up(c_out, 16)
        d_.y, d_.ldy, d_.cstore = 256, co, co
        d_.dy, d_.hy, d_.wy = d, h, w
        d_.os = 1
        d_.ooff = (C.c_int32 * 3)(0, 0, 0)
        d_.dtype = DT_FP8
        d_.q_amax_x = d_.q_amax_w = 256
        hit = _FP8_OK[key] = _lib.load().mi355_conv_plan_id(C.byref(d_)) > 0
    return hit


_FP8_OK = {}


def conv_fp8_supported(x0: torch.Tensor, coutp: int, out: torch.Tensor, grid) -> bool:
    n, di, hi, wi, c0 = x0.shape
    if c0 != 32 or not x0.is_cuda:
        return False
    d = _lib.ConvDesc()
    d.x0, d.c0, d.ld0 = x0.data_ptr(), c0, c0
    d.x1, d.c1, d.ld1 = None, 0, 0
    d.n, d.di, d.hi, d.wi = n, di, hi, wi
    d.do_, d.ho, d.wo = grid
    d.ks, d.stride = 3, 1
    d.pad = (C.c_int32 * 3)(1, 1, 1)
    d.wp, d.coutp = x0.data_ptr(), coutp
    d.y, d.ldy, d.cstore = out.data_ptr(), act_ld(out), out.shape[4]
    d.dy, d.hy, d.wy = out.shape[1:4]
    d.os = 1
    d.ooff = (C.c_int32 * 3)(0, 0, 0)
    d.dtype = DT_FP8
    d.q_amax_x = d.q_amax_w = x0.data_ptr()
    return _lib.load().mi355_conv_plan_id(C.byref(d)) > 0


def fp8_selftest(device) -> torch.Tensor:
    out = torch.zeros(1024, dtype=torch.float32, device=device)
    _lib.check(_lib.load().mi355_fp8_selftest(out.data_ptr(), _stream()), "fp8_selftest")
    return out.view(32, 32)


def channel_stats(x: torch.Tensor, groups: int) -> Tuple[torch.Tensor, int]:
    require_cuda(x)
    n, d, h, w, c = x.shape
    rows = n * d * h * w
    assert rows % groups == 0
    rpg = rows // groups
    lib = _lib.load()
    bpg = lib.mi355_channel_stats_blocks(rpg)
    part = torch.empty((groups * bpg, 2, c), dtype=torch.float32, device=x.device)
    _lib.check(lib.mi355_channel_stats(x.data_ptr(), act_ld(x), c, rpg, groups, part.data_ptr(), bpg,
                                       _DT[x.dtype], _stream()), "channel_stats")
    return part, bpg


def norm_finalize(part, parts_per_group, groups, c, count, shift, eps, running_mean=None, running_var=None,
                  momentum=0.0, n_real=0, batches_tracked=None):
    mean = torch.empty((groups, c), dtype=torch.float32, device=part.device)
    rstd = torch.empty_like(mean)
    _lib.check(_lib.load().mi355_norm_finalize(part.data_ptr(), parts_per_group, groups, c, count, _ptr(shift), n_real,
                                               eps, mean.data_ptr(), rstd.data_ptr(), _ptr(running_mean),
                                               _ptr(running_var), momentum, _ptr(batches_tracked), _stream()), "norm_finalize")
    return mean, rstd


def colsum(x: torch.Tensor) -> torch.Tensor:
    part, bpg = channel_stats(x, 1)
    c = x.shape[4]
    out = torch.empty((c,), dtype=torch.float32, device=x.device)
    _lib.check(_lib.load().mi355_colsum_finalize(part.data_ptr(), bpg, c, out.data_ptr(), _stream()), "colsum")
    return out


def colsum_into(x: torch.Tensor, out: torch.Tensor, accumulate: bool):
    require_cuda(x, out)
    assert out.dtype == torch.float32 and out.is_contiguous() and out.numel() <= x.shape[4]
    part, bpg = channel_stats(x, 1)
    _lib.check(_lib.load().mi355_colsum_finalize_into(part.data_ptr(), bpg, x.shape[4], out.data_ptr(), out.numel(),
                                                      1 if accumulate else 0, _stream()), "colsum_into")


def colsum_from_parts(part: torch.Tensor, offset: int, out: torch.Tensor, accumulate: bool = False):
    require_cuda(part, out)
    rows, two, c = part.shape
    assert two == 2 and part.is_contiguous() and part.dtype == out.dtype == torch.float32 and out.is_contiguous()
    assert 0 <= offset and offset + out.numel() <= c
    _lib.check(_lib.load().mi355_colsum_finalize_from(part.data_ptr(), rows, c, offset, out.data_ptr(), out.numel(),
                                                      1 if accumulate else 0, _stream()), "colsum_from_parts")


def _normact_desc(z, groups, mean, rstd, gamma, beta, slope, drop_p, seed, seed_t=None):
    d = _lib.NormActDesc()
    n, dd, h, w, c = z.shape
    rows = n * dd * h * w
    d.z, d.ldz, d.c = z.data_ptr(), act_ld(z), c
    d.rows_per_group, d.groups = rows // groups, groups
    for t in (mean, rstd):
        if t is not None and t.numel() != groups * c:
            raise ValueError(f"norm statistics hold {t.numel()} values for {groups} group(s) x {c} channels")
    d.mean, d.rstd, d.gamma, d.beta = _ptr(mean), _ptr(rstd), _ptr(gamma), _ptr(beta)
    d.n_affine = gamma.numel() if gamma is not None else 0
    d.slope, d.drop_p, d.seed = slope, drop_p, seed
    d.seed_ptr = _ptr(seed_t)
    d.dtype = _DT[z.dtype]
    return d


NORM_PROBE = None


def _norm_probe(kind, z, gamma):
    if NORM_PROBE is None:
        return None
    n, dd, h, w, c = z.shape
    return NORM_PROBE(kind, gamma.numel() if gamma is not None else c, n * dd * h * w, z.element_size())


def _set_q8(d, q8):
    t8, use, nxt = q8
    require_cuda(t8, use, nxt)
    assert t8.dtype == torch.uint8 and t8.is_contiguous() and use.dtype == nxt.dtype == torch.float32
    d.q8, d.ld8, d.q_use, d.q_next = t8.data_ptr(), t8.shape[-1], use.data_ptr(), nxt.data_ptr()


def normact_fwd(z, groups, mean, rstd, gamma, beta, slope, drop_p=0.0, seed=0, out=None, s2d=False, seed_t=None, q8=None,
                final=None, skip_a=False, pool=False):
    require_cuda(z, mean, rstd, gamma, beta, out)
    if out is None:
        out = torch.empty(z.shape, dtype=z.dtype, device=z.device)
    d = _normact_desc(z, groups, mean, rstd, gamma, beta, slope, drop_p, seed, seed_t)
    d.a, d.lda = out.data_ptr(), act_ld(out)
    keep_final = None
    if final is not None:
        fw, fb, fy = final
        require_cuda(fw, fb, fy)
        assert not s2d and z.dtype == fy.dtype == torch.bfloat16 and fw.dtype == torch.float32 and fw.is_contiguous()
        fw2 = fw.detach().reshape(fw.shape[0], -1)
        assert fw2.shape[0] <= 8 and fw2.shape[1] <= z.shape[4] and tuple(fy.shape[:4]) == tuple(z.shape[:4])
        assert fb is None or (fb.dtype == torch.float32 and fb.numel() == fw2.shape[0])
        d.gw, d.gw_ld, d.gk = fw2.data_ptr(), fw2.shape[1], fw2.shape[0]
        d.fy, d.ldfy, d.fcp, d.fbias = fy.data_ptr(), act_ld(fy), fy.shape[4], _ptr(fb.detach() if fb is not None else None)
        d.skip_a = 1 if skip_a else 0
        keep_final = (fw2, fb, fy)
    else:
        assert not skip_a
    if q8 is not None:
        _set_q8(d, q8)
    if s2d:
        d.s2d_a = 1
        d.sd, d.sh, d.sw = z.shape[1:4]
    py = pidx = None
    if pool:
        n, dd, h, w, c = z.shape
        assert not s2d and q8 is None and final is None and dd % 2 == 0 and h % 2 == 0 and w % 2 == 0
        py = torch.empty((n, dd // 2, h // 2, w // 2, c), dtype=z.dtype, device=z.device)
        pidx = torch.empty(py.shape, dtype=torch.uint8, device=z.device)
        d.pool_y, d.ldpy, d.pool_widx = py.data_ptr(), act_ld(py), pidx.data_ptr()
        d.sd, d.sh, d.sw = dd, h, w
    after = _norm_probe("fwd", z, gamma)
    _lib.check(_lib.load().mi355_normact_fwd(C.byref(d), _stream()), "normact_fwd")
    if after is not None:
        after()
    return (out, py, pidx) if pool else out


def normact_bwd(z, da, groups, mean, rstd, gamma, beta, slope, drop_p, seed, batch_stats, want_affine_grads,
                s2d=False, seed_t=None, affine_into=None, accumulate=False, q8=None, implicit=None, pool=None):
    require_cuda(z, da)
    lib = _lib.load()
    n, dd, h, w, c = z.shape
    rows = n * dd * h * w
    d = _normact_desc(z, groups, mean, rstd, gamma, beta, slope, drop_p, seed, seed_t)
    keep_implicit = None
    if implicit is not None:
        gz, gw = implicit
        require_cuda(gz, gw)
        assert da is None and not s2d and z.dtype == torch.bfloat16 and gz.dtype == torch.bfloat16
        assert tuple(gz.shape[:4]) == tuple(z.shape[:4]) and gw.dtype == torch.float32 and gw.is_contiguous()
        gw2 = gw.detach().reshape(gw.shape[0], -1)
        assert gw2.shape[0] <= 8 and gw2.shape[0] <= gz.shape[4] and gw2.shape[1] <= c
        d.gz, d.ldgz, d.gw, d.gw_ld, d.gk = gz.data_ptr(), act_ld(gz), gw2.data_ptr(), gw2.shape[1], gw2.shape[0]
        keep_implicit = (gz, gw2)
    elif pool is not None:
        pidx, pdy = pool
        require_cuda(pidx, pdy)
        assert not s2d and pidx.dtype == torch.uint8 and pidx.is_contiguous() and pdy.dtype == z.dtype
        assert tuple(pidx.shape) == (n, dd // 2, h // 2, w // 2, c) == tuple(pdy.shape) and dd % 2 == 0 and h % 2 == 0 and w % 2 == 0
        d.pool_idx, d.pool_dy, d.ldpdy = pidx.data_ptr(), pdy.data_ptr(), act_ld(pdy)
        d.sd, d.sh, d.sw = dd, h, w
        if da is not None:
            assert tuple(da.shape) == tuple(z.shape) and da.dtype == z.dtype
            d.da, d.ldda = da.data_ptr(), act_ld(da)
    else:
        d.da, d.ldda = da.data_ptr(), act_ld(da)
    dz = torch.empty(z.shape, dtype=z.dtype, device=z.device)
    d.dz, d.lddz = dz.data_ptr(), act_ld(dz)
    d.batch_stats = 1 if batch_stats else 0
    if s2d:
        d.s2d_da = 1
        d.sd, d.sh, d.sw = z.shape[1:4]
    if q8 is not None:
        _set_q8(d, q8)
    dgamma = dbeta = None
    keep = []
    after = _norm_probe("bwd", z, gamma)
    if mean is not None and (batch_stats or want_affine_grads):
        bpg = lib.mi355_channel_stats_blocks(rows // groups)
        part = torch.empty((groups * bpg, 2, c), dtype=torch.float32, device=z.device)
        d.part, d.blocks_per_group = part.data_ptr(), bpg
        _lib.check(lib.mi355_normact_bwd_reduce(C.byref(d), _stream()), "normact_bwd_reduce")
        sums = torch.empty((groups, 2, c), dtype=torch.float32, device=z.device)
        if affine_into is not None:
            g_into, b_into = affine_into
            require_cuda(g_into, b_into)
            assert g_into.dtype == b_into.dtype == torch.float32 and g_into.numel() == b_into.numel() <= c
            _lib.check(lib.mi355_normact_bwd_finalize_into(part.data_ptr(), bpg, groups, c, sums.data_ptr(),
                                                           g_into.data_ptr(), b_into.data_ptr(), g_into.numel(),
                                                           1 if accumulate else 0, _stream()), "normact_bwd_finalize")
        else:
            dgamma = torch.empty((c,), dtype=torch.float32, device=z.device)
            dbeta = torch.empty((c,), dtype=torch.float32, device=z.device)
            _lib.check(lib.mi355_normact_bwd_finalize(part.data_ptr(), bpg, groups, c, sums.data_ptr(),
                                                      dgamma.data_ptr(), dbeta.data_ptr(), _stream()),
                       "normact_bwd_finalize")
        d.sums = sums.data_ptr()
        keep += [part, sums]
    _lib.check(lib.mi355_normact_bwd_apply(C.byref(d), _stream()), "normact_bwd_apply")
    if after is not None:
        after()
    return dz, dgamma, dbeta


SMALL_NORM_ELEMENTS = 1 << 19


SMALL_NORM_ELEMENTS_GROUPED = SMALL_NORM_ELEMENTS


def norm_is_small(n: int, d: int, h: int, w: int, c: int, serial_groups: int = 1) -> bool:
    limit = SMALL_NORM_ELEMENTS if serial_groups <= 1 else SMALL_NORM_ELEMENTS_GROUPED
    return c >= 64 and n * d * h * w * c <= limit


def normact_small_fwd(z, groups, gamma, beta, eps, slope, drop_p=0.0, seed=0, seed_t=None, running_mean=None,
                      running_var=None, momentum=0.0, batches_tracked=None, out=None, s2d=False):
    require_cuda(z, gamma, beta, out, running_mean, running_var)
    n, dd, h, w, c = z.shape
    if out is None:
        out = torch.empty(z.shape, dtype=z.dtype, device=z.device)
    mean = torch.empty((groups, c), dtype=torch.float32, device=z.device)
    rstd = torch.empty_like(mean)
    d = _lib.NormSmallDesc()
    d.base = _normact_desc(z, groups, None, None, gamma, beta, slope, drop_p, seed, seed_t)
    d.base.a, d.base.lda = out.data_ptr(), act_ld(out)
    if s2d:
        d.base.s2d_a = 1
        d.base.sd, d.base.sh, d.base.sw = z.shape[1:4]
    d.eps, d.momentum = eps, momentum
    d.mean_out, d.rstd_out = mean.data_ptr(), rstd.data_ptr()
    d.running_mean, d.running_var, d.batches_tracked = _ptr(running_mean), _ptr(running_var), _ptr(batches_tracked)
    d.n_real = running_mean.numel() if running_mean is not None else 0
    after = _norm_probe("fwd", z, gamma)
    _lib.check(_lib.load().mi355_normact_small_fwd(C.byref(d), _stream()), "normact_small_fwd")
    if after is not None:
        after()
    return out, mean, rstd


def normact_small_bwd(z, da, groups, mean, rstd, gamma, beta, slope, drop_p, seed, batch_stats, s2d=False, seed_t=None,
                      affine_into=None, accumulate=False, want_affine=True, group_scratch=None):
    require_cuda(z, da, mean, rstd)
    n, dd, h, w, c = z.shape
    d = _lib.NormSmallDesc()
    d.base = _normact_desc(z, groups, mean, rstd, gamma, beta, slope, drop_p, seed, seed_t)
    d.base.da, d.base.ldda = da.data_ptr(), act_ld(da)
    dz = torch.empty(z.shape, dtype=z.dtype, device=z.device)
    d.base.dz, d.base.lddz = dz.data_ptr(), act_ld(dz)
    d.base.batch_stats = 1 if batch_stats else 0
    if s2d:
        d.base.s2d_da = 1
        d.base.sd, d.base.sh, d.base.sw = z.shape[1:4]
    dgamma = dbeta = None
    if affine_into is not None:
        g_into, b_into = affine_into
        require_cuda(g_into, b_into)
        assert g_into.dtype == b_into.dtype == torch.float32 and g_into.numel() == b_into.numel() <= c
        d.base.n_affine = g_into.numel()
        d.dgamma, d.dbeta, d.accumulate = g_into.data_ptr(), b_into.data_ptr(), 1 if accumulate else 0
    elif want_affine:
        dgamma = torch.zeros((c,), dtype=torch.float32, device=z.device)
        dbeta = torch.zeros((c,), dtype=torch.float32, device=z.device)
        d.dgamma, d.dbeta, d.accumulate = dgamma.data_ptr(), dbeta.data_ptr(), 0
    gpart = None
    if (groups >= 3) if group_scratch is None else group_scratch:
        gpart = torch.empty((groups, 2, c), dtype=torch.float64, device=z.device)
        d.base.part = gpart.data_ptr()
    after = _norm_probe("bwd", z, gamma)
    _lib.check(_lib.load().mi355_normact_small_bwd(C.byref(d), _stream()), "normact_small_bwd")
# ... 104 lines not shown
```

Baseline: 100.4 volumes/s.

## Fuse generator output unpack and S2D repack into final normact kernel epilogue

Extends the fused final 1x1x1 convolution kernel so its epilogue also writes the NCDHW f32 output and the space-to-depth bf16 layout the discriminator reads. This replaces the separate unpack and s2d_repack passes in GenOutFn for the discriminator's generator forward. When the discriminator reads only the S2D form, the f32 output is skipped entirely and marked unwritten. It adds bookkeeping through a pointer-keyed side table and guards that raise if the unwritten values are later read, and it adds scattered stores plus extra index arithmetic to the kernel.

```diff
diff --git a/include/mi355_unet.h b/include/mi355_unet.h
--- a/include/mi355_unet.h
+++ b/include/mi355_unet.h
@@ -151,6 +151,7 @@
   void* fy; int32_t ldfy; int32_t fcp; const float* fbias; int32_t skip_a;
   const void* pool_idx; const void* pool_dy; int32_t ldpdy;
   void* pool_y; int32_t ldpy; uint8_t* pool_widx;
+  float* fy32; void* fys; int32_t ldfys; int32_t skip_fy;
 } mi355_normact_desc;
 int mi355_normact_fwd(const mi355_normact_desc* d, void* stream);
 int mi355_normact_bwd_reduce(const mi355_normact_desc* d, void* stream);
diff --git a/unet_bssfp_amd/_lib.py b/unet_bssfp_amd/_lib.py
--- a/unet_bssfp_amd/_lib.py
+++ b/unet_bssfp_amd/_lib.py
@@ -61,7 +61,8 @@
                 ("gz", _vp), ("ldgz", _i32), ("gw", _vp), ("gw_ld", _i32), ("gk", _i32),
                 ("fy", _vp), ("ldfy", _i32), ("fcp", _i32), ("fbias", _vp), ("skip_a", _i32),
                 ("pool_idx", _vp), ("pool_dy", _vp), ("ldpdy", _i32),
-                ("pool_y", _vp), ("ldpy", _i32), ("pool_widx", _vp)]
+                ("pool_y", _vp), ("ldpy", _i32), ("pool_widx", _vp),
+                ("fy32", _vp), ("fys", _vp), ("ldfys", _i32), ("skip_fy", _i32)]
 
 
 class QueueLoad(C.Structure):
diff --git a/unet_bssfp_amd/csrc/elementwise.hip b/unet_bssfp_amd/csrc/elementwise.hip
--- a/unet_bssfp_amd/csrc/elementwise.hip
+++ b/unet_bssfp_amd/csrc/elementwise.hip
@@ -398,6 +398,7 @@
   uint8_t* q8; int ld8; const float* q_use; float* q_next;
   const char* gz; int ldgz; const float* gw; int gw_ld; int gk;
   char* fy; int ldfy; int fcp; const float* fbias; int skip_a;
+  float* fy32; char* fys; int ldfys; int skip_fy; S2D seam;
   const uint8_t* pool_idx; const char* pool_dy; int ldpdy; int pd, ph, pw;
   char* pool_y; int ldpy; uint8_t* pool_widx;
 };
@@ -560,7 +561,7 @@
 }
 
 typedef float f32x4v __attribute__((ext_vector_type(4)));
-template <bool DROP>
+template <bool DROP, bool SEAM>
 __global__ __launch_bounds__(256) void normact_fwd_final32_kernel(const NormActArgs q) {
   const int lane = threadIdx.x & 63, wave = threadIdx.x >> 6, n = lane & 15, p = lane >> 4;
   const int g = blockIdx.y, ch0 = 8 * p;
@@ -596,6 +597,17 @@
   bf16_t* yb = reinterpret_cast<bf16_t*>(q.fy) + (long long)g * q.rows_per_group * q.ldfy;
   const long long stride = (long long)gridDim.x * 64;
   const long long first = (long long)blockIdx.x * 64 + wave * 16;
+  unsigned cw = 0, chh = 0, cd = 0, cn = 0, sw_ = 0, sh_ = 0, sd_ = 0, sn_ = 0, lane32 = 0;
+  if constexpr (SEAM) {
+    const unsigned W = q.seam.w, H = q.seam.h, D = q.seam.d;
+    const unsigned b0 = (unsigned)((long long)g * q.rows_per_group) + blockIdx.x * 64u + (unsigned)__builtin_amdgcn_readfirstlane(wave) * 16u;
+    unsigned t = b0 / W;
+    cw = b0 - t * W; cn = t / H; chh = t - cn * H; t = cn; cn = t / D; cd = t - cn * D;
+    const unsigned st = gridDim.x * 64u;
+    t = st / W;
+    sw_ = st - t * W; sn_ = t / H; sh_ = t - sn_ * H; t = sn_; sn_ = t / D; sd_ = t - sn_ * D;
+    lane32 = 4u * p * (D * H * W) + n;
+  }
   uint4 zn = make_uint4(0u, 0u, 0u, 0u);
   if (first < q.rows_per_group) {
     const long long rc = first + n < q.rows_per_group ? first + n : q.rows_per_group - 1;
@@ -630,7 +642,37 @@
     if (ok && 4 * p < q.fcp) {
       const uint2 yv = make_uint2((uint32_t)f32_to_bf16_bits(acc[0] + fb[0]) | ((uint32_t)f32_to_bf16_bits(acc[1] + fb[1]) << 16),
                                   (uint32_t)f32_to_bf16_bits(acc[2] + fb[2]) | ((uint32_t)f32_to_bf16_bits(acc[3] + fb[3]) << 16));
-      *reinterpret_cast<uint2*>(yb + row * q.ldfy + 4 * p) = yv;
+      if (!SEAM || !q.skip_fy) *reinterpret_cast<uint2*>(yb + row * q.ldfy + 4 * p) = yv;
+      if constexpr (SEAM) {
+        const unsigned W = q.seam.w, H = q.seam.h, D = q.seam.d, w_ = cw + n;
+        const unsigned ox = __shfl_down(yv.x, 16), oy = __shfl_down(yv.y, 16);
+        if (p < 2 && q.fy32) {
+          const unsigned dhw = D * H * W;
+          float* o = q.fy32 + (cn * (unsigned)q.gk * dhw + (cd * H + chh) * W + cw) + lane32;
+          const unsigned yw[2] = {yv.x, yv.y};
+#pragma unroll
+          for (int j = 0; j < 4; ++j)
+            if (4 * p + j < q.gk) o[j * dhw] = __uint_as_float(j & 1 ? yw[j >> 1] & 0xffff0000u : yw[j >> 1] << 16);
+        }
+        if (p == 0 && q.fys) {
+          const unsigned srow = ((cn * (D / 2 + 1) + ((cd + 1) >> 1)) * (H / 2 + 1) + ((chh + 1) >> 1)) * (W / 2 + 1) + ((w_ + 1) >> 1);
+          const unsigned blk = ((cd + 1) & 1) * 4 + ((chh + 1) & 1) * 2 + ((w_ + 1) & 1);
+          const unsigned border = ((cd == 0 || cd == D - 1) ? 4 : 0) | ((chh == 0 || chh == H - 1) ? 2 : 0) | ((w_ == 0 || w_ == W - 1) ? 1 : 0);
+          bf16_t* cell = reinterpret_cast<bf16_t*>(q.fys) + srow * (unsigned)q.ldfys;
+          *reinterpret_cast<uint4*>(cell + blk * 8) = make_uint4(yv.x, yv.y, ox, oy);
+          if (border)
+#pragma unroll 1
+            for (unsigned sub = 1; sub < 8; ++sub)
+              if ((sub & ~border) == 0) *reinterpret_cast<uint4*>(cell + (blk ^ sub) * 8) = make_uint4(0u, 0u, 0u, 0u);
+        }
+      }
+    }
+    if constexpr (SEAM) {
+      const unsigned W = q.seam.w, H = q.seam.h, D = q.seam.d;
+      cw += sw_; if (cw >= W) { cw -= W; ++chh; }
+      chh += sh_; if (chh >= H) { chh -= H; ++cd; }
+      cd += sd_; if (cd >= D) { cd -= D; ++cn; }
+      cn += sn_;
     }
   }
 }
@@ -2007,6 +2049,17 @@
                 "%s: the fused 1x1x1 convolution needs bf16, 32 channels, gk <= 8 outputs in rows of fcp (8 .. 32) channels", who);
   MI355_REQUIRE(!d->skip_a || d->fy, "%s: skip_a without the fused convolution", who);
   q->fy = (char*)d->fy; q->ldfy = d->ldfy; q->fcp = d->fcp; q->fbias = d->fbias; q->skip_a = d->skip_a;
+  MI355_REQUIRE(!(d->fy32 || d->fys) || (d->fy && d->sd >= 2 && d->sh >= 2 && d->sw >= 2 && !((d->sd | d->sh | d->sw) & 1) &&
+                                         ((long long)d->rows_per_group * d->groups) % ((long long)d->sd * d->sh * d->sw) == 0 &&
+                                         (long long)d->rows_per_group * d->groups < (1ll << 31) && d->sw % 16 == 0 &&
+                                         (!d->fys || (d->ldfys >= 64 && d->ldfys % 8 == 0 &&
+                                                      (long long)d->rows_per_group * d->groups / ((long long)d->sd * d->sh * d->sw) * (d->sd / 2 + 1) *
+                                                              (d->sh / 2 + 1) * (d->sw / 2 + 1) * d->ldfys < (1ll << 31))) &&
+                                         (!d->fy32 || (long long)d->rows_per_group * d->groups * d->gk < (1ll << 31))),
+                "%s: the fused output layouts need the fused convolution, even extents sd/sh/sw (sw % 16 == 0) that divide the row count, S rows of >= 64 channels and outputs of fewer than 2^31 elements", who);
+  MI355_REQUIRE(!d->skip_fy || d->fy32 || d->fys, "%s: skip_fy without another output layout", who);
+  q->fy32 = d->fy32; q->fys = (char*)d->fys; q->ldfys = d->ldfys; q->skip_fy = d->skip_fy;
+  q->seam = S2D{d->sd, d->sh, d->sw, 8};
   MI355_REQUIRE(!d->pool_idx || (d->pool_dy && !d->gz && !d->s2d_da && !d->s2d_a && d->sd >= 2 && d->sh >= 2 && d->sw >= 2 &&
                                  !((d->sd | d->sh | d->sw) & 1) && d->ldpdy >= d->c && d->ldpdy % (d->dtype == MI355_DT_F32 ? 4 : 8) == 0 &&
                                  ((long long)d->rows_per_group * d->groups) % ((long long)d->sd * d->sh * d->sw) == 0 &&
@@ -2068,8 +2121,11 @@
     MI355_REQUIRE(d->fcp == 16, "normact_fwd: the fused convolution writes 16-channel rows");
     long long b = (d->rows_per_group + 64 * 8 - 1) / (64 * 8);
     const dim3 grid32((unsigned)(b < 1 ? 1 : (b > 2048 ? 2048 : b)), d->groups);
-    if (q.thr16) normact_fwd_final32_kernel<true><<<grid32, dim3(256), 0, (hipStream_t)stream>>>(q);
-    else normact_fwd_final32_kernel<false><<<grid32, dim3(256), 0, (hipStream_t)stream>>>(q);
+    if (q.fy32 || q.fys) {
+      if (q.thr16) normact_fwd_final32_kernel<true, true><<<grid32, dim3(256), 0, (hipStream_t)stream>>>(q);
+      else normact_fwd_final32_kernel<false, true><<<grid32, dim3(256), 0, (hipStream_t)stream>>>(q);
+    } else if (q.thr16) normact_fwd_final32_kernel<true, false><<<grid32, dim3(256), 0, (hipStream_t)stream>>>(q);
+    else normact_fwd_final32_kernel<false, false><<<grid32, dim3(256), 0, (hipStream_t)stream>>>(q);
   } else {
     if (q.thr16) normact_fwd_kernel<bf16_t, true><<<grid, dim3(256), 0, (hipStream_t)stream>>>(q);
     else normact_fwd_kernel<bf16_t, false><<<grid, dim3(256), 0, (hipStream_t)stream>>>(q);
diff --git a/unet_bssfp_amd/functional.py b/unet_bssfp_amd/functional.py
--- a/unet_bssfp_amd/functional.py
+++ b/unet_bssfp_amd/functional.py
@@ -390,6 +390,47 @@
     @classmethod
     def clear(cls):
         cls._by_ptr.clear()
+
+
+class SeamOut:
+    _by_ptr = {}
+    enabled = True
+
+    @classmethod
+    def put(cls, y, y32, s):
+        if len(cls._by_ptr) >= 8:
+            cls._by_ptr.clear()
+        cls._by_ptr[y.data_ptr()] = (y32, s, tuple(y.shape), y)
+
+    @classmethod
+    def take(cls, y):
+        hit = cls._by_ptr.pop(y.data_ptr(), None)
+        if hit is None:
+            return None
+        if hit[2] != tuple(y.shape):
+            raise RuntimeError("SeamOut: the tensor that takes the fused output layouts is not the one they were computed for")
+        return hit[0], hit[1]
+
+    @classmethod
+    def holds(cls, y) -> bool:
+        return y.data_ptr() in cls._by_ptr
+
+    _unwritten = set()
+
+    @classmethod
+    def mark_unwritten(cls, y32):
+        cls._unwritten.add(y32.data_ptr())
+
+    @classmethod
+    def unwritten(cls, y32) -> bool:
+        hit = y32.data_ptr() in cls._unwritten
+        cls._unwritten.discard(y32.data_ptr())
+        return hit
+
+    @classmethod
+    def clear(cls):
+        cls._by_ptr.clear()
+        cls._unwritten.clear()
 
 
 def fp8_operand(x: torch.Tensor, slot: "Fp8Scales.Slot", constant: bool = False) -> torch.Tensor:
@@ -499,6 +540,8 @@
     @staticmethod
     def forward(ctx, act, c):
         ctx.meta = (act.shape[4], act.dtype)
+        if SeamOut.holds(act):
+            raise RuntimeError("UnpackFn: this output was promised to GenOutFn and has not been written (SeamOut)")
         return ops.unpack_ncdhw(act, c, 0)
 
     @staticmethod
@@ -518,6 +561,15 @@
         act = ops.as_act(act)
         ctx.meta = (tuple(act.shape), act.dtype, c)
         ctx.set_materialize_grads(False)
+        pre = SeamOut.take(act)
+        if pre is not None:
+            y32, s = pre
+            if tuple(s.shape) != ops.s2d_shape(act.shape[0], *act.shape[1:4], cblk) or (y32 is not None and y32.shape[1] != c):
+                raise RuntimeError("GenOutFn: the fused output layouts do not match the requested ones")
+            if y32 is None:
+                y32 = torch.empty((act.shape[0], c, *act.shape[1:4]), dtype=torch.float32, device=act.device)
+                SeamOut.mark_unwritten(y32)
+            return y32, s
         return ops.unpack_ncdhw(act, c, 0), ops.s2d_repack(act, cblk)
 
     @staticmethod
@@ -1112,6 +1164,7 @@
         LazyPool.clear()
         PoolSide.clear()
         FusedFinal.clear()
+        SeamOut.clear()
         Fp8Scales.advance(device)
 
     @classmethod
@@ -1193,11 +1246,18 @@
             emit8.touched = True
             Fp8Side.put(a, a8)
         elif final is not None and z.dtype == torch.bfloat16 and c == 32:
-            fw, fb, skip_a = final
+            fw, fb, skip_a = final[:3]
             y = ops.new_act(n, d, h, w, round_up(fw.shape[0], 16), z.dtype, z.device)
+            seam = None
+            if (len(final) > 3 and final[3] is not None and SeamOut.enabled and d % 2 == 0 and h % 2 == 0 and w % 16 == 0
+                    and rows < 2 ** 31):
+                y32 = torch.empty((n, fw.shape[0], d, h, w), dtype=torch.float32, device=z.device) if final[3] else None
+                seam = (y32, _new_s2d(ops.s2d_shape(n, d, h, w, 8), z.dtype, z.device), True)
             a = ops.normact_fwd(z, groups, mean, rstd, gp, bp, cfg.slope, p, seed, seed_t=seed_t,
-                                final=(fw.detach(), fb.detach() if fb is not None else None, y), skip_a=skip_a)
+                                final=(fw.detach(), fb.detach() if fb is not None else None, y), skip_a=skip_a, seam=seam)
             FusedFinal.put(a, y, fw)
+            if seam is not None:
+                SeamOut.put(y, seam[0], seam[1])
         elif (pool_after and PoolSide.enabled and not s2d_out and emit8 is None and d % 2 == 0 and h % 2 == 0 and w % 2 == 0
               and (rows // groups) % (d * h * w) == 0):
             a, py, pidx = ops.normact_fwd(z, groups, mean, rstd, gp, bp, cfg.slope, p, seed, seed_t=seed_t, pool=True)
diff --git a/unet_bssfp_amd/gan.py b/unet_bssfp_amd/gan.py
--- a/unet_bssfp_amd/gan.py
+++ b/unet_bssfp_amd/gan.py
@@ -93,13 +93,15 @@
         return (self.fused_loss_heads and self.l1_fn is None and not self.extra_recon_terms
                 and all(t.is_cuda and t.dtype == torch.float32 for t in tensors))
 
-    def _gen_for_discr(self, x):
+    def _gen_for_discr(self, x, s2d_only=False):
         if hasattr(self.gen, "emit_s2d") and next(self.gen.parameters()).is_cuda:
             self.gen.emit_s2d = True
+            self.gen.emit_s2d_only = bool(s2d_only)
             try:
                 return self.gen(x)
             finally:
                 self.gen.emit_s2d = False
+                self.gen.emit_s2d_only = False
         return self.gen(x)
 
     @staticmethod
@@ -108,6 +110,8 @@
         s = getattr(y, "_mi355_s2d", None)
         if s is not None:
             out._mi355_s2d = s.detach()
+        if getattr(y, "_mi355_unwritten", False):
+            out._mi355_unwritten = True
         return out
 
     def _gen_step(self, x, y, logs, step_name="train"):
@@ -136,7 +140,8 @@
         return 2
 
     def _discr_step(self, x, y):
-        y_hat = self._detach(self._gen_for_discr(x))
+        only = self._discr_pair() and hasattr(self.discr, "reads_s2d_only") and self.discr.reads_s2d_only(x, y)
+        y_hat = self._detach(self._gen_for_discr(x, s2d_only=only))
         if self._discr_pair():
             both = self.discr.forward_pair(x, y_hat, y, stacked=self._fused_losses(x, y))
             if isinstance(both, torch.Tensor):
diff --git a/unet_bssfp_amd/nn.py b/unet_bssfp_amd/nn.py
--- a/unet_bssfp_amd/nn.py
+++ b/unet_bssfp_amd/nn.py
@@ -204,7 +204,7 @@
                 h = self._packed_x(x, split[2])
                 h1 = self._s2d_of(y, split[3])
             else:
-                h = Fn.PackFn.apply(-cp, self.compute_dtype, x, y)
+                h = Fn.PackFn.apply(-cp, self.compute_dtype, x, self._values(y))
             for i, blk in enumerate(blocks):
                 if i == 0 and split:
                     h = blk.forward_act(h, h1, s2d_out=True, split=split[:2])
@@ -214,7 +214,7 @@
                 if i == 1 and blk.conv.weight.requires_grad:
                     Fn.StageBoundary.mark(h)
         else:
-            h = Fn.PackFn.apply(cp, self.compute_dtype, x, y)
+            h = Fn.PackFn.apply(cp, self.compute_dtype, x, self._values(y))
             for i, blk in enumerate(blocks):
                 h = blk.forward_act(h)
                 if i == 1 and blk.conv.weight.requires_grad:
@@ -241,7 +241,19 @@
         s = getattr(y, "_mi355_s2d", None)
         if s is not None and s.dtype == self.compute_dtype and s.shape[4] == 8 * cpy and s.shape[0] == y.shape[0]:
             return s
-        return Fn.PackFn.apply(-cpy, self.compute_dtype, y)
+        return Fn.PackFn.apply(-cpy, self.compute_dtype, self._values(y))
+
+    @staticmethod
+    def _values(y):
+        if getattr(y, "_mi355_unwritten", False):
+            raise RuntimeError("Discriminator: this generator output was produced as S(output) only (emit_s2d_only) and the route "
+                               "taken reads its values; ask the generator for the f32 tensor")
+        return y
+
+    def reads_s2d_only(self, x, y) -> bool:
+        if not (self.pair_single_pass(x, y, y) and round_up(y.shape[1], 8) == 8 and self.compute_dtype == torch.bfloat16):
+            return False
+        return self._split_first_block(x, y, 2 * x.shape[0]) is not None
 
     def _packed_x(self, x, cpx):
         hit = Fn.PackMemo.get(x, -cpx, self.compute_dtype)
@@ -274,12 +286,12 @@
                 if s is not None and s.dtype == self.compute_dtype and tuple(s.shape) == tuple(h1[half * n:(half + 1) * n].shape):
                     h1[half * n:(half + 1) * n].copy_(s.detach())
                 else:
-                    ops.pack_ncdhw_s2d(y.detach().to(torch.float32).contiguous(), h1[half * n:(half + 1) * n], split[3], 0, split[3])
+                    ops.pack_ncdhw_s2d(self._values(y).detach().to(torch.float32).contiguous(), h1[half * n:(half + 1) * n], split[3], 0, split[3])
         else:
             h = Fn._new_s2d(ops.s2d_shape(2 * n, d, hh, w, cp), self.compute_dtype, x.device)
             x32 = x.detach().to(torch.float32).contiguous()
             for half, y in enumerate((y_a, y_b)):
-                ops.pack2(x32, y.detach().to(torch.float32).contiguous(), h[half * n:(half + 1) * n], 0, cp, s2d_cblk=cp)
+                ops.pack2(x32, self._values(y).detach().to(torch.float32).contiguous(), h[half * n:(half + 1) * n], 0, cp, s2d_cblk=cp)
         for i, blk in enumerate(blocks):
             if i == 0 and split:
                 h = blk.forward_act(h, h1, s2d_out=True, bn_groups=2, split=split[:2])
@@ -308,7 +320,7 @@
         self.cfg = Fn.NormCfg("instance", cout, eps=eps, slope=slope, p=float(dropout or 0.0))
 
     def forward_act(self, x0, x1=None, feeds: Optional[Conv3d] = None, up_from=None, final: Optional[Conv3d] = None,
-                    pool_after: bool = False):
+                    pool_after: bool = False, seam: Optional[bool] = None):
         n, d, h, w = x0.shape[:4]
         cp = round_up(self.conv.out_channels, 16)
         small = ops.norm_is_small(n, d, h, w, cp)
@@ -331,7 +343,7 @@
         fin = None
         if (final is not None and not small and z.dtype == torch.bfloat16 and cp == 32 and emit8 is None and final.out_channels <= 8
                 and final.in_channels <= cp and Fn.LazyDx.enabled):
-            fin = (final.weight, final.bias, not torch.is_grad_enabled())
+            fin = (final.weight, final.bias, not torch.is_grad_enabled(), seam)
         return Fn.NormActFn.apply(z, part if not small else None, self.adn.N.weight, self.adn.N.bias, shift, self.cfg,
                                   self.training, None, None, False, None, small, 1, emit8, emit8_bwd, fin, pool_after)
 
@@ -342,9 +354,9 @@
         self.conv_0 = Convolution(cin, cout, dropout)
         self.conv_1 = Convolution(cout, cout, dropout)
 
-    def forward_act(self, x0, x1=None, up_from=None, final=None, pool_after=False):
+    def forward_act(self, x0, x1=None, up_from=None, final=None, pool_after=False, seam=None):
         return self.conv_1.forward_act(self.conv_0.forward_act(x0, x1, feeds=self.conv_1.conv, up_from=up_from), final=final,
-                                       pool_after=pool_after)
+                                       pool_after=pool_after, seam=seam)
 
 
 class Down(_Mi355Module):
@@ -384,11 +396,11 @@
                 and x_e.shape[4] + deconv.out_channels == conv.in_channels and deconv.bias is not None
                 and x.shape[3] >= 32 and not ops.norm_is_small(x_e.shape[0], *x_e.shape[1:4], co))
 
-    def forward_act(self, x, x_e, final=None):
+    def forward_act(self, x, x_e, final=None, seam=None):
         if self._fused(x, x_e):
             if not hasattr(self, "upcat_tables"):
                 self.upcat_tables = Fn.UpCatTables()
-            return self.convs.forward_act(x_e, None, up_from=(x, self.upsample.deconv, self.upcat_tables), final=final)
+            return self.convs.forward_act(x_e, None, up_from=(x, self.upsample.deconv, self.upcat_tables), final=final, seam=seam)
         x_0 = self.upsample.deconv.forward_act(x)
         if x_0.shape[1:4] != x_e.shape[1:4]:
             for ax in (1, 2, 3):
@@ -396,7 +408,7 @@
                     x_0 = torch.cat([x_0, x_0.narrow(ax, x_0.shape[ax] - 1, 1)], ax)
             if x_0.shape[1:4] != x_e.shape[1:4]:
                 raise ValueError(f"skip {tuple(x_e.shape[1:4])} and up-sampled map {tuple(x_0.shape[1:4])} differ by more than one")
-        return self.convs.forward_act(x_e, x_0, final=final)
+        return self.convs.forward_act(x_e, x_0, final=final, seam=seam)
 
 
 class BasicUNet(_Mi355Module):
@@ -469,7 +481,7 @@
         y3 = torch.func.functional_call(self, self._embedded_parameters(), (x3,), {"_embedded": True})
         return y3.mean(2)
 
-    def forward_act(self, x):
+    def forward_act(self, x, seam: Optional[bool] = None):
         d, h, w = x.shape[1:4]
         if min(d, h, w) < 16 or (d >> 4) * (h >> 4) * (w >> 4) < 2:
             raise ValueError(f"four 2x poolings need extents >= 16, and InstanceNorm more than one element at the bottom "
@@ -486,7 +498,7 @@
         u3 = self.upcat_3.forward_act(u4, s2)
         u2 = self.upcat_2.forward_act(u3, s1)
         lazy = self.lazy_final_dx and u2.dtype == torch.bfloat16
-        u1 = self.upcat_1.forward_act(u2, s0, final=self.final_conv if lazy else None)
+        u1 = self.upcat_1.forward_act(u2, s0, final=self.final_conv if lazy else None, seam=seam if lazy else None)
         z, _ = self.final_conv.forward_act(u1, lazy_dx=lazy and not ops.norm_is_small(*u1.shape))
         return z
 
@@ -524,13 +536,16 @@
                                      "bssfp": bssfp_input, "t1w": dwi_tensor_input, "unet": unet})
 
     emit_s2d = False
+    emit_s2d_only = False
 
     def forward(self, x):
         head = self.blocks[self.input_modality]
         a = head.forward_act(head._to_act(x))
-        z = self.blocks["unet"].forward_act(a)
-        if self.emit_s2d and z.dtype == torch.bfloat16 and all(e % 2 == 0 for e in z.shape[1:4]):
+        if self.emit_s2d and a.dtype == torch.bfloat16 and all(e % 2 == 0 for e in a.shape[1:4]):
+            z = self.blocks["unet"].forward_act(a, seam=not self.emit_s2d_only)
             y, s = Fn.GenOutFn.apply(z, 6, 8)
             y._mi355_s2d = s
+            if Fn.SeamOut.unwritten(y):
+                y._mi355_unwritten = True
             return y
-        return Fn.UnpackFn.apply(z, 6)
+        return Fn.UnpackFn.apply(self.blocks["unet"].forward_act(a), 6)
diff --git a/unet_bssfp_amd/ops.py b/unet_bssfp_amd/ops.py
--- a/unet_bssfp_amd/ops.py
+++ b/unet_bssfp_amd/ops.py
@@ -549,7 +549,7 @@
 
 
 def normact_fwd(z, groups, mean, rstd, gamma, beta, slope, drop_p=0.0, seed=0, out=None, s2d=False, seed_t=None, q8=None,
-                final=None, skip_a=False, pool=False):
+                final=None, skip_a=False, pool=False, seam=None):
     require_cuda(z, mean, rstd, gamma, beta, out)
     if out is None:
         out = torch.empty(z.shape, dtype=z.dtype, device=z.device)
@@ -567,8 +567,19 @@
         d.fy, d.ldfy, d.fcp, d.fbias = fy.data_ptr(), act_ld(fy), fy.shape[4], _ptr(fb.detach() if fb is not None else None)
         d.skip_a = 1 if skip_a else 0
         keep_final = (fw2, fb, fy)
+        if seam is not None:
+            y32, ys, skip_fy = seam
+            require_cuda(y32, ys)
+            n, dd, h, w, _ = z.shape
+            assert (y32 is not None or ys is not None) and dd % 2 == 0 and h % 2 == 0 and w % 16 == 0
+            assert y32 is None or (y32.dtype == torch.float32 and y32.is_contiguous()
+                                   and tuple(y32.shape) == (n, fw2.shape[0], dd, h, w))
+            assert ys is None or (ys.dtype == torch.bfloat16 and is_act(ys) and tuple(ys.shape) == s2d_shape(n, dd, h, w, 8))
+            d.fy32, d.fys, d.ldfys = _ptr(y32), _ptr(ys), act_ld(ys) if ys is not None else 0
+            d.skip_fy = 1 if skip_fy else 0
+            d.sd, d.sh, d.sw = dd, h, w
     else:
-        assert not skip_a
+        assert not skip_a and seam is None
     if q8 is not None:
         _set_q8(d, q8)
     if s2d:
```

Measured after the change: 101.0 volumes/s, median of 6. Within noise of the previous version (+0.6%).
